# HKPolyU-UAV/FLVIS

Hardware: AMD Instinct MI355X
Metric: frames/sec/node (640×480 stereo+IMU) + ATE vs CPU ref, EuRoC MH_05 (higher is better)
Workload: dtype u8/f32 LK+GFTT, f64 geometry+BA

## Files before the change

### flvis_amd/csrc/frame_schedule.cpp

```cpp
#include <algorithm>
#include <chrono>
#include <cstring>
#include <thread>
#include <vector>

#include "pipeline_host.hpp"

using namespace flvis;

static void fill_pyr(Pipeline* pl, PyrSel& ps, uint8_t* const* l0, uint8_t* const* l1, const int* cur, int flip, int levels) {
  ps.levels = levels;
  for (int l = 0; l <= levels; l++) {
    ps.lvl[l] = ImgSel{{l0[l], l1 ? l1[l] : l0[l]}, cur, flip, nullptr};
    ps.w[l] = pl->lw[l];
    ps.h[l] = pl->lh[l];
    ps.pitch[l] = pl->lpitch[l];
    ps.stride[l] = pl->lstride[l];
    ps.bx[l] = pl->lbx;
    ps.by[l] = pl->lby;
  }
}

unsigned flvis::pyramid_levels(hipStream_t ds, bool bordered, ImgSel src0, int spitch0, size_t sstride0, bool ingest, bool level0_is_buffer,
                               const PyrSel& pyr, int S, const int* active) {
// ... 35 lines not shown
      if (f) border_left &= ~(1u << d);
    }
    l = d;
  }
  return border_left;
}

static void join_signal(Pipeline* pl, Lane* L, JoinId id, hipStream_t s) {
  Join& j = L->join[id];
  ++j.seq;
  if (pl->flag_joins) launch_store_flag(s, j.word, j.seq);
  else hipEventRecord(j.ev, s);
}
static void join_wait(Pipeline* pl, Lane* L, hipStream_t s, JoinId id) {
  const Join& j = L->join[id];
  if (pl->flag_joins) launch_wait_flag(s, j.word, 1, j.seq, L->d_progress + 2);
  else hipStreamWaitEvent(s, j.ev, 0);
}

namespace flvis {
struct LaunchJoins {
  Pipeline* pl;
  Lane* L;
  hipStream_t s;
  KJoin& kj;
  int n_wait = 0, sig_later = -1, post_later = -1;
  LaunchJoins(Pipeline* pl_, Lane* L_, hipStream_t s_, KJoin& kj_) : pl(pl_), L(L_), s(s_), kj(kj_) {}
  LaunchJoins(const LaunchJoins&) = delete;
  ~LaunchJoins() { end(); }
  bool fold_signal(JoinId id) {
    if (!pl->fold_joins) return false;
    Join& j = L->join[id];
    kj.sig = j.word;
    kj.sig_seq = ++j.seq;
    kj.sig_cnt = j.cnt;
    return true;
  }
  bool fold_wait(JoinId id) {
    if (!pl->fold_joins || n_wait == (int)(sizeof(kj.wait) / sizeof(kj.wait[0]))) return false;
    kj.wait[n_wait] = L->join[id].word;
    kj.wait_seq[n_wait++] = L->join[id].seq;
    kj.err = L->d_progress + 2;
    return true;
  }
  bool fold_post(JoinId id) {
    if (!pl->fold_joins) return false;
    kj.post = L->join[id].word;
    kj.post_seq = L->join[id].seq;
    kj.err = L->d_progress + 2;
    return true;
  }
  void signal(JoinId id) {
    if (!fold_signal(id)) sig_later = id;
  }
  void wait(JoinId id) {
    if (!fold_wait(id)) join_wait(pl, L, s, id);
  }
  void post(JoinId id) {
    if (!fold_post(id)) post_later = id;
  }
  void end() {
    kj = KJoin{};
    if (sig_later >= 0) join_signal(pl, L, (JoinId)sig_later, s);
    if (post_later >= 0) join_wait(pl, L, s, (JoinId)post_later);
    n_wait = 0, sig_later = post_later = -1;
  }
};
}

LmCloudRec flvis::lane_lmc(const Pipeline* pl, const Lane* L) {
  LmCloudRec r = pl->lmc;
  r.hdr += (size_t)L->s0 * LMC_HDR;
  r.ids += (size_t)L->s0 * r.cap;
  r.pts += (size_t)L->s0 * r.cap * 3;
  return r;
}
void flvis::local_map_work(Pipeline* pl, Lane* L, hipStream_t bs, int pairs, hipEvent_t prof_end) {
  if (pl->lmc.cap <= 0) {
    launch_ba_worker(bs, L->pipe);
    if (prof_end) hipEventRecord(prof_end, bs);
    return;
  }
  Pipe one = L->pipe;
  one.ba_drain = 1;
  const LmCloudRec r = lane_lmc(pl, L);
  for (int k = 0; k < pairs; k++) {
    launch_ba_worker(bs, one);
    if (prof_end && k == 0) hipEventRecord(prof_end, bs);
    launch_lm_cloud_append(bs, one, r);
  }
}

void flvis::launch_local_map(Pipeline* pl, Lane* L, JoinId at, bool signal, hipEvent_t* prof_begin_end) {
  const int bi = (L->idx * pl->nba_lane + (int)(L->ba_launches % pl->nba_lane)) % pl->nba;
  hipStream_t bs = pl->ba_stream[bi];
  if (prof_begin_end) {
    unsigned char& rec = L->prof18_rec[(size_t)pl->prof_step];
    if (rec) prof_begin_end = nullptr;
    else rec = 1;
  }
  if (signal) join_signal(pl, L, at, L->st);
  join_wait(pl, L, bs, at);
  const bool rec_on = pl->lmc.cap > 0;
  if (rec_on && L->ba_launches > 0) join_wait(pl, L, bs, J_BA(L->ba_launches - 1));
  if (prof_begin_end) hipEventRecord(prof_begin_end[0], bs);
  local_map_work(pl, L, bs, pl->ba_every + std::min(L->lmc_cmds, pl->ba_every), prof_begin_end ? prof_begin_end[1] : nullptr);
  L->lmc_cmds = 0;
  join_signal(pl, L, J_BA(L->ba_launches), bs);
  L->ba_launches++;
  L->ba_pending = false;
}

static void sync_streams(flvis_ctx* ctx) {
  hipStreamSynchronize(ctx->stream);
  Pipeline* pl = ctx->pipe;
  if (!pl) return;
  for (Lane* L : pl->lanes) {
    hipStreamSynchronize(L->st);
    hipStreamSynchronize(L->det_stream);
  }
  for (int k = 0; k < Pipeline::NBA; k++)
    if (pl->ba_stream[k]) hipStreamSynchronize(pl->ba_stream[k]);
}
void flvis::sync_all(flvis_ctx* ctx) {
  if (ctx->pipe)
    for (Lane* L : ctx->pipe->lanes)
      if (L->ba_pending) launch_local_map(ctx->pipe, L, J_FE, true, nullptr);
  sync_streams(ctx);
  Pipeline* pl = ctx->pipe;
  if (!pl) return;
  for (Lane* L : pl->lanes) {
    std::vector<unsigned> hd(L->S), tl(L->S);
    for (int guard = 0; guard < 64; guard++) {
      hipMemcpy(hd.data(), L->pipe.kfq_head, sizeof(unsigned) * L->S, hipMemcpyDeviceToHost);
      hipMemcpy(tl.data(), L->pipe.kfq_tail, sizeof(unsigned) * L->S, hipMemcpyDeviceToHost);
      bool pending = false;
      for (int i = 0; i < L->S; i++) pending = pending || hd[i] != tl[i];
      if (!pending) break;
      local_map_work(pl, L, pl->ba_stream[0], 1, nullptr);
      hipStreamSynchronize(pl->ba_stream[0]);
    }
  }
}

static long long lane_backpressure_depth(Pipeline* pl, Lane* L) {
  long long D = std::max(0, KFQ / 2 / pl->ba_every - 3);
  if (L->cmd_steps.empty()) return D;
  const long long window = (D + pl->nba_lane + 2) * pl->ba_every;
  std::vector<long long>& c = L->cmd_steps;
  c.erase(std::remove_if(c.begin(), c.end(), [&](long long f) { return L->frames_uploaded - f > window; }), c.end());
  return std::max(0LL, D - (long long)c.size());
}

void flvis::lane_backpressure_wait(Pipeline* pl, Lane* L, LaunchJoins* folded) {
  const long long D = lane_backpressure_depth(pl, L);
  for (int k = 0; k < pl->nba_lane; k++) {
    const long long j = L->ba_launches - 1 - D - k;
    if (j < 0 || L->ba_launches - j > BAQ) continue;
    if (folded) folded->wait(J_BA(j));
    else join_wait(pl, L, L->st, J_BA(j));
  }
}

namespace {

struct Frame {
  Pipeline* pl;
  Lane* L;
  Pipe& p;
  hipStream_t st, ds;
  int S, w, h;
  int with_local_map;
  long long frame_no;
  bool zerocopy;
  bool prof;
  hipEvent_t* pev;
  hipEvent_t* prof18;
  bool skipped, idle_step;
  bool eq, aligned, depth_cam, r_in_place;
  ImgSel in0, in1, l0cur;
  bool cmd_pending;
  bool first_processed;
  bool head_prepare;
  bool head_posts;
  bool merge_collect;
  void mark(int i, int end, hipStream_t s) const {
    if (prof && ((pl->prof_mask >> i) & 1ull)) hipEventRecord(pev[2 * i + end], s);
  }
  void pb(int i, hipStream_t s) const { mark(i, 0, s); }
  void pe(int i, hipStream_t s) const { mark(i, 1, s); }
  void stage_host_inputs(const uint8_t* d_img0, const uint8_t* d_img1, const double* h_times, const uint8_t* present);
  void stage_ingest_left(), stage_head(), stage_idle_tail(), stage_temporal_lk(), stage_collect_ransac_f(), stage_detection_fork();
  void stage_pnp_pose(), stage_new_landmarks(), stage_stereo_depth(), stage_frame_end();
  void local_map_tail(hipEvent_t* p18, bool timed), frame_end(bool backpressure);
  LKParams lk_params(int stats_at, int tc_mode, int order) const;
};

void Frame::stage_host_inputs(const uint8_t* d_img0, const uint8_t* d_img1, const double* h_times, const uint8_t* present) {
  frame_no = ++L->frames_uploaded;
  const int pslot = (int)((frame_no - 1) % Lane::PIN_RING);
  uint8_t* pin = (uint8_t*)L->pinned[pslot];
  if (pl->sync_each_frame) hipStreamSynchronize(st);
  const long long lead = std::min(std::min(pl->host_lead, pl->host_lead_cap), (int)Lane::PIN_RING - 1);
  if (frame_no > lead && *L->h_progress < frame_no - lead) {
    const auto tw = std::chrono::steady_clock::now();
    int polls = 0;
    while (*L->h_progress < frame_no - lead) {
      if ((++polls & 255) == 0 && hipStreamQuery(st) == hipSuccess && *L->h_progress < frame_no - lead) break;
      std::this_thread::sleep_for(std::chrono::microseconds(30));
    }
    pl->host_ms_wait += std::chrono::duration<double, std::milli>(std::chrono::steady_clock::now() - tw).count();
  }
  double* pt = (double*)pin;
  double* pi = pt + S;
  const uint8_t** ptab = (const uint8_t**)(pi + (size_t)S * IMU_MAX * 7);
  int* pn = (int*)(ptab + 2);
  int* ppres = (int*)((uint8_t*)pin + L->in_off_pres);
  int n_present = S;
  if (present) {
    n_present = 0;
    for (int s = 0; s < S; s++) n_present += (ppres[s] = present[s] ? 1 : 0);
  }
  const bool all_present = n_present == S, none_present = n_present == 0;
  memcpy(pt, h_times, sizeof(double) * S);
  for (int s = 0; s < S; s++)
    memcpy(pi + (size_t)s * IMU_MAX * 7, &L->h_imu[(size_t)s * IMU_MAX * 7], sizeof(double) * 7 * L->h_nimu[s]);
  ptab[0] = d_img0;
  ptab[1] = d_img1;
  memcpy(pn, L->h_nimu.data(), sizeof(int) * S);
  std::fill(L->h_nimu.begin(), L->h_nimu.end(), 0);
  cmd_pending = L->cmd_since_frame;
  L->cmd_since_frame = false;
  zerocopy = L->pinned_dev[pslot] != nullptr;
  L->h_tab[0] = d_img0, L->h_tab[1] = d_img1;
  p.in_img1 = d_img1;
  {
    uint8_t* din = zerocopy ? L->pinned_dev[pslot] : L->d_inputs;
    L->d_time = reinterpret_cast<double*>(din);
    p.imu_in = reinterpret_cast<double*>(din + L->in_off_imu);
    p.n_imu = reinterpret_cast<int*>(din + L->in_off_n);
    p.present = all_present ? nullptr : reinterpret_cast<const int*>(din + L->in_off_pres);
  }
  if (!zerocopy) hipMemcpyAsync(L->d_inputs, pin, L->input_bytes, hipMemcpyHostToDevice, st);
  prof = pl->prof_cap > 0 && pl->prof_step < pl->prof_cap;
  pev = prof ? &L->prof_ev[(size_t)pl->prof_step * (2 * PROF_STAGES)] : nullptr;
  prof18 = (prof && ((pl->prof_mask >> 18) & 1ull)) ? &pev[2 * 18] : nullptr;
  skipped = pl->frames_fed < (long long)pl->cfg.skip_first_n_imgs;
  idle_step = skipped || none_present;
  first_processed = pl->frames_fed == (long long)pl->cfg.skip_first_n_imgs;
  depth_cam = pl->cfg.cam_type == CAM_DEPTH;
  eq = pl->cfg.need_equal_hist != 0;
  aligned = (w & 15) == 0 && !(((uintptr_t)d_img0 | (depth_cam ? (uintptr_t)0 : (uintptr_t)d_img1)) & 15);
  r_in_place = !eq && aligned;
  in0 = img_plain(d_img0), in1 = img_plain(d_img1);
  l0cur = ImgSel{{L->pyr0[0][0], L->pyr0[1][0]}, p.img_slot, 0, nullptr};
  head_prepare = pl->head_prepare && !pl->feedback_used && !idle_step;
  merge_collect = (pl->chain_merge & 2) != 0;
}

void Frame::stage_ingest_left() {
  ImgSel l0in{{L->pyr0[0][0], L->pyr0[1][0]}, p.img_slot_in, 0, nullptr};
  if (pl->fold_joins && zerocopy && L->endf_valid && pl->chain_continuous) {
    join_wait(pl, L, ds, J_ENDF);
  } else {
    join_signal(pl, L, J_LM, st);
    join_wait(pl, L, ds, J_LM);
  }
  if (pl->up_event) hipStreamWaitEvent(ds, pl->up_event, 0);
  if (pl->up_flag) launch_wait_flag(ds, pl->up_flag, Pipeline::HostFeed::FLAG_WORDS, pl->up_seq, L->d_progress + 2);
  pb(1, ds);
  const int* pg = p.present;
  if (eq) launch_equalize_hist(ds, in0, l0in, w, h, w, pl->lpitch[0], (size_t)w * h, pl->lstride[0], S, L->eq_hist, L->eq_lut, pg);
  else if (!aligned) launch_copy_image_any(ds, in0, l0in, w, h, w, pl->lpitch[0], (size_t)w * h, pl->lstride[0], S, pg);
  pe(1, ds);
  pb(2, ds);
  PyrSel pyl;
  fill_pyr(pl, pyl, L->pyr0[0], L->pyr0[1], p.img_slot_in, 0, pl->levels);
  unsigned border_left = pyramid_levels(ds, pl->lbx != 0, in0, w, (size_t)w * h, !eq && aligned, true, pyl, S, pg);
  if (pl->levels == 0 && !eq && aligned) launch_copy_image(ds, in0, l0in, w, h, w, pl->lpitch[0], (size_t)w * h, pl->lstride[0], S, pg);
  if (border_left) launch_pyr_border(ds, pyl, S, pg, border_left);
  pe(2, ds);
  join_signal(pl, L, J_IMG, ds);
}

void Frame::stage_head() {
  pb(0, st);
  bool head_signals;
  {
    LaunchJoins j(pl, L, st, p.kj);
    head_signals = !pl->feedback_used && j.fold_signal(J_HEAD);
    head_posts = !idle_step && j.fold_post(J_IMG);
    if (head_prepare) launch_frame_head_prepare(st, p, L->d_time, L->d_progress, frame_no);
    else launch_frame_head(st, p, L->d_time, L->d_progress, frame_no);
  }
  if (pl->feedback_used) launch_apply_correction(st, p);
  pe(0, st);
  if (!head_signals) join_signal(pl, L, J_HEAD, st);
}

void Frame::local_map_tail(hipEvent_t* p18, bool timed) {
  if (with_local_map && (pl->frames_fed % pl->ba_every) == 0) {
    if (L->ba_pending) launch_local_map(pl, L, J_FE, true, nullptr);
    if (pl->defer_ba) L->ba_pending = true;
    else if (L->endf_valid) launch_local_map(pl, L, J_ENDF, false, p18);
    else launch_local_map(pl, L, J_FE, true, p18);
  } else if (!with_local_map) {
    if (cmd_pending) {
      if (L->ba_launches > 0) join_wait(pl, L, st, J_BA(L->ba_launches - 1));
      launch_kfq_drop(st, p);
    } else hipMemcpyAsync(p.kfq_head, p.kfq_tail, sizeof(unsigned) * S, hipMemcpyDeviceToDevice, st);
    if (timed) {
      pb(18, st);
      pe(18, st);
      L->prof18_rec[(size_t)pl->prof_step] = 1;
    }
  }
}

void Frame::frame_end(bool backpressure) {
  LaunchJoins j(pl, L, st, p.kj);
  if (backpressure) lane_backpressure_wait(pl, L, &j);
  pb(17, st);
  L->endf_valid = j.fold_signal(J_ENDF);
  launch_frame_end(st, p);
  j.end();
  pe(17, st);
  pe(19, st);
}

void Frame::stage_idle_tail() {
  frame_end(false);
  if (prof)
    for (int i = 1; i < PROF_STAGES; i++)
      if (i != 17 && i != 19) {
        pb(i, st);
        pe(i, st);
      }
  if (!skipped) local_map_tail(nullptr, false);
}

LKParams Frame::lk_params(int stats_at, int tc_mode, int order) const {
  LKParams prm{30, 1e-3 * 1e-3, 1e-4f, 1};
  if (pl->lk_stats) prm.stats = reinterpret_cast<unsigned long long*>(p.counters) + stats_at;
  if (pl->lk_stats) prm.stats_tc = reinterpret_cast<unsigned long long*>(p.counters) + 61;
  if (L->tc) {
    prm.tc = L->tc;
    prm.tc_mode = tc_mode;
    prm.tc_cap = p.tc_cap;
    prm.tc_stride = L->tc_stride;
    prm.tc_slot = p.lk_slot;
    prm.tc_tag = p.lk_tag;
  }
  prm.dbg_slot = (int)(pl->frames_fed & 7);
  prm.order = order;
  return prm;
}

void Frame::stage_temporal_lk() {
  if (first_processed && L->idx > 0) hipStreamWaitEvent(st, pl->lanes[L->idx - 1]->ev_stagger, 0);
  pb(3, st);
  if (!head_prepare) launch_track_prepare(st, p);
  pe(3, st);
  if (!head_posts) join_wait(pl, L, st, J_IMG);
  pb(4, st);
  PyrSel prev, next;
  fill_pyr(pl, prev, L->pyr0[0], L->pyr0[1], p.img_slot, 1, pl->levels_t);
  fill_pyr(pl, next, L->pyr0[0], L->pyr0[1], p.img_slot, 0, pl->levels_t);
  launch_lk_track(st, prev, next, p.prev_pts, p.next_pts, p.lk_status, p.lk_count, NMAX, S, lk_params(36, 2, 0), p.act_track, pl->max_pts, 1);
  pe(4, st);
}

void Frame::stage_collect_ransac_f() {
  pb(5, st);
  if (!merge_collect) launch_track_collect(st, p);
  pe(5, st);
  if (first_processed && pl->lanes.size() > 1) hipEventRecord(L->ev_stagger, st);
  pb(6, st);
  {
    LaunchJoins j(pl, L, st, p.kj);
    j.signal(J_LM);
    launch_ransac_f(st, p, merge_collect);
    pe(6, st);
  }
}

void Frame::stage_detection_fork() {
  join_wait(pl, L, ds, J_LM);
  join_wait(pl, L, ds, J_HEAD);
  launch_gftt(ds, l0cur, w, h, pl->lpitch[0], pl->lstride[0], S, L->gftt, nullptr, p.cam.gftt_ql, p.gftt_maxc, p.cam.gftt_num,
              (double)p.cam.gftt_dis, L->gftt_xy, L->gftt_n, 2 * p.cam.gftt_num, p.gftt_act,
              (prof && ((pl->prof_mask >> 10) & 7ull) == 7ull) ? &pev[2 * 10] : nullptr, false);
  {
    KJoin prep_kj{};
    LaunchJoins j(pl, L, ds, prep_kj);
    j.signal(J_GFTT);
    launch_feature_dem_prep(ds, l0cur, w, h, pl->lpitch[0], pl->lstride[0], S, p.cam.dem, L->gftt_xy, L->gftt_n, 2 * p.cam.gftt_num,
                            p.gftt_act, L->dem_sorted, L->dem_roff, &prep_kj);
  }
  join_wait(pl, L, ds, J_HEAD);
  if (!depth_cam) {
    if (eq) launch_equalize_hist(ds, in1, img_plain(L->pyr1[0]), w, h, w, pl->lpitch[0], (size_t)w * h, pl->lstride[0], S, L->eq_hist, L->eq_lut, p.act_img);
    else if (!aligned) launch_copy_image_any(ds, in1, img_plain(L->pyr1[0]), w, h, w, pl->lpitch[0], (size_t)w * h, pl->lstride[0], S, p.act_img);
    PyrSel pyr_r;
    fill_pyr(pl, pyr_r, L->pyr1, nullptr, nullptr, 0, pl->levels);
    unsigned border_left = pyramid_levels(ds, pl->lbx != 0, in1, w, (size_t)w * h, false, !r_in_place, pyr_r, S, p.act_img);
    if (border_left) launch_pyr_border(ds, pyr_r, S, p.act_img, border_left);
  }
  join_signal(pl, L, J_DET, ds);
}

void Frame::stage_pnp_pose() {
  pb(7, st);
  const bool ba_here = L->ba_pending;
  bool pnp_signals;
  {
    LaunchJoins j(pl, L, st, p.kj);
    pnp_signals = ba_here && j.fold_signal(J_FE);
    launch_ransac_pnp(st, p);
  }
  if (p.pnp_tail_cv) launch_pnp_tail_cv(st, p);
  pe(7, st);
  if (ba_here) launch_local_map(pl, L, J_FE, !pnp_signals, prof18);
  pb(8, st);
  launch_pose_lm(st, p);
  pe(8, st);
  pb(9, st);
  {
    LaunchJoins j(pl, L, st, p.kj);
    j.signal(J_LM);
    launch_reproj_filter(st, p);
    pe(9, st);
  }
  join_wait(pl, L, ds, J_LM);
  launch_vi_correction(ds, p);
}

void Frame::stage_new_landmarks() {
  {
    KJoin dem_kj{};
    LaunchJoins j(pl, L, st, dem_kj);
    j.wait(J_GFTT);
    pb(13, st);
    launch_feature_dem(st, w, h, S, p.cam.dem, L->dem_sorted, L->dem_roff, 2 * p.cam.gftt_num, p.det_mode, p.exist_xy, p.n_exist, NMAX,
                       p.new_xy, p.n_new, NEW_MAX, &dem_kj);
  }
  const bool merge_seeds = (pl->chain_merge & 1) != 0;
  bool an_signals, seeds_post;
  {
    LaunchJoins j(pl, L, st, p.kj);
    an_signals = j.fold_signal(J_LM);
    if (!merge_seeds) {
      launch_add_new(st, p);
      j.end();
    }
    pe(13, st);
    pb(14, st);
    seeds_post = j.fold_post(J_DET);
    if (merge_seeds) launch_add_new_seeds(st, p);
    else launch_depth_seeds(st, p);
  }
  pe(14, st);
  if (!an_signals) join_signal(pl, L, J_LM, st);
  join_wait(pl, L, ds, J_LM);
  launch_depth_triangulate(ds, p);
  join_signal(pl, L, J_TRI, ds);
  if (!seeds_post) join_wait(pl, L, st, J_DET);
}

void Frame::stage_stereo_depth() {
  pb(15, st);
  if (!depth_cam) {
    PyrSel prev, next;
    fill_pyr(pl, prev, L->pyr0[0], L->pyr0[1], p.img_slot, 0, pl->levels_s);
    fill_pyr(pl, next, L->pyr1, nullptr, nullptr, 0, pl->levels_s);
    next.lvl[0] = r_in_place ? in1 : img_plain(L->pyr1[0]);
    next.pitch[0] = r_in_place ? w : pl->lpitch[0];
    next.stride[0] = r_in_place ? (size_t)w * h : pl->lstride[0];
    if (r_in_place) next.bx[0] = next.by[0] = 0;
    launch_lk_track(st, prev, next, p.prev_pts, p.next_pts, p.lk_status, p.lk_count, NMAX, S, lk_params(48, 1, 1), p.det_mode, pl->max_pts, 2);
  }
  pe(15, st);
  LaunchJoins j(pl, L, st, p.kj);
  j.wait(J_TRI);
  pb(16, st);
  launch_depth_innovate(st, p);
  j.end();
  pe(16, st);
}

void Frame::stage_frame_end() {
  frame_end(with_local_map != 0);
  if (pl->kfl.cap > 0) kf_log_frame(pl, L, st, in1.b[0], depth_cam || r_in_place);
  local_map_tail(prof18, prof);
}

}

static void lane_frame(Pipeline* pl, Lane* L, const uint8_t* d_img0, const uint8_t* d_img1, const double* h_times, const uint8_t* present,
                       int with_local_map) {
  Frame f{pl, L, L->pipe, L->st, L->det_stream, L->S, pl->cfg.image_width, pl->cfg.image_height, with_local_map};
  f.stage_host_inputs(d_img0, d_img1, h_times, present);
  f.pb(19, f.st);
  if (!f.idle_step) f.stage_ingest_left();
  f.stage_head();
  if (f.idle_step) return f.stage_idle_tail();
  f.stage_temporal_lk();
  f.stage_collect_ransac_f();
  f.stage_detection_fork();
  f.stage_pnp_pose();
  f.stage_new_landmarks();
  f.stage_stereo_depth();
  f.stage_frame_end();
}

extern "C" {

int flvis_image_feed(flvis_ctx* ctx, const uint8_t* d_img0, const uint8_t* d_img1, const double* h_times,
                     flvis_frame_out* h_out, int with_local_map) {
  return flvis_image_feed_present(ctx, d_img0, d_img1, h_times, nullptr, h_out, with_local_map);
}

int flvis_image_feed_present(flvis_ctx* ctx, const uint8_t* d_img0, const uint8_t* d_img1, const double* h_times, const uint8_t* h_present,
                             flvis_frame_out* h_out, int with_local_map) {
  if (!ctx || !ctx->pipe || !d_img0 || !d_img1 || !h_times) return FLVIS_ERR_INVALID_ARG;
  Pipeline* pl = ctx->pipe;
  if (h_present) {
    bool all = true;
    for (int s = 0; s < pl->S && all; s++) all = h_present[s] != 0;
    if (all) h_present = nullptr;
  }
  hipSetDevice(ctx->device);
  const size_t img_px = (size_t)pl->cfg.image_width * pl->cfg.image_height;
  const size_t img1_bytes = img_px * (pl->cfg.cam_type == CAM_DEPTH ? 2 : 1);
  const bool multi = pl->lanes.size() > 1;
  const auto t_host0 = std::chrono::steady_clock::now();
  if (multi) hipEventRecord(pl->ev_in, ctx->stream);
  for (Lane* L : pl->lanes) {
    if (multi) hipStreamWaitEvent(L->st, pl->ev_in, 0);
    lane_frame(pl, L, d_img0 + (size_t)L->s0 * img_px, d_img1 + (size_t)L->s0 * img1_bytes, h_times + L->s0,
               h_present ? h_present + L->s0 : nullptr, with_local_map);
    if (multi) {
      hipEventRecord(L->ev_end[pl->frames_fed % Lane::HOLD_RING], L->st);
      const long long rel = pl->frames_fed - pl->input_hold;
      if (rel >= 0) hipStreamWaitEvent(ctx->stream, L->ev_end[rel % Lane::HOLD_RING], 0);
    }
  }
  pl->host_ms_total += std::chrono::duration<double, std::milli>(std::chrono::steady_clock::now() - t_host0).count();
  const bool prof = pl->prof_cap > 0 && pl->prof_step < pl->prof_cap;
  if (prof) pl->prof_step++;
  pl->frames_fed++;
  if (h_present) {
    for (int s = 0; s < pl->S; s++) pl->stream_frames += h_present[s] != 0;
  } else {
    pl->stream_frames += pl->S;
  }
  hipError_t e = hipGetLastError();
  if (e != hipSuccess) return ctx->hip_fail(e, "image_feed launch");
  if (h_out) {
    static_assert(sizeof(flvis_frame_out) == sizeof(FrameOut), "FrameOut layout");
    for (Lane* L : pl->lanes) {
      e = hipMemcpyAsync(h_out + L->s0, L->pipe.out, sizeof(FrameOut) * L->S, hipMemcpyDeviceToHost, L->st);
      if (e != hipSuccess) return ctx->hip_fail(e, "image_feed readback");
    }
    for (Lane* L : pl->lanes) {
      e = hipStreamSynchronize(L->st);
      if (e != hipSuccess) return ctx->hip_fail(e, "image_feed readback");
    }
  }
  return FLVIS_OK;
}


int flvis_imu_feed_all(flvis_ctx* ctx, const int* h_counts, const double* h_samples, int samples_per_stream) {
  if (!ctx || !ctx->pipe || !h_counts || !h_samples || samples_per_stream <= 0) return FLVIS_ERR_INVALID_ARG;
  Pipeline* pl = ctx->pipe;
  for (int s = 0; s < pl->S; s++) {
    int n = h_counts[s];
    if (n < 0 || n > samples_per_stream) return ctx->fail(FLVIS_ERR_INVALID_ARG, "imu_feed_all: bad count");
    int rc = flvis_imu_feed_flvis_frame(ctx, s, n, h_samples + (size_t)s * samples_per_stream * 7);
    if (rc) return rc;
  }
  return FLVIS_OK;
}

int flvis_run_steps(flvis_ctx* ctx, int n_steps, const flvis_step* steps, int with_local_map, double* h_call_ms) {
  return flvis_run_steps_present(ctx, n_steps, steps, nullptr, with_local_map, h_call_ms);
}

int flvis_run_steps_present(flvis_ctx* ctx, int n_steps, const flvis_step* steps, const uint8_t* h_present, int with_local_map,
                            double* h_call_ms) {
  if (!ctx || !ctx->pipe || n_steps < 0 || (n_steps > 0 && !steps)) return FLVIS_ERR_INVALID_ARG;
  for (int k = 0; k < n_steps; k++) {
    const flvis_step& f = steps[k];
    const auto t0 = std::chrono::steady_clock::now();
    if (f.h_imu_counts) {
      const int rc = flvis_imu_feed_all(ctx, f.h_imu_counts, f.h_imu_samples, f.imu_samples_per_stream);
      if (rc != FLVIS_OK) return rc;
    }
    ctx->pipe->defer_ba = k + 1 < n_steps;
    ctx->pipe->chain_continuous = k > 0;
    const int rc = flvis_image_feed_present(ctx, f.d_img0, f.d_img1, f.h_times, h_present ? h_present + (size_t)k * ctx->pipe->S : nullptr,
                                            nullptr, with_local_map);
    ctx->pipe->defer_ba = false;
    ctx->pipe->chain_continuous = false;
    if (rc != FLVIS_OK) return rc;
    if (h_call_ms) h_call_ms[k] = std::chrono::duration<double, std::milli>(std::chrono::steady_clock::now() - t0).count();
  }
  return FLVIS_OK;
}

}
```

### flvis_amd/csrc/img_kernels.hip

```cpp
#include <cstdlib>

#include "dev_common.hpp"
#include "dem_sort.hpp"
#include "eig_strip.hpp"
#include "img_kernels.hpp"

namespace flvis {

template <int TH, int TW, int TS>
__device__ __forceinline__ void load_tile_u8(const uint8_t* __restrict__ img, int w, int h, int pitch, int x0, int y0,
                                             uint8_t* tile, int bx = 0, int by = 0) {
  static_assert(TW % 4 == 0, "tile width must be a multiple of 4");
  constexpr int DW = TW / 4;
  if (x0 >= -bx && y0 >= -by && x0 + TW <= w + bx && y0 + TH <= h + by && blockDim.x == 256) {
    constexpr int N = TH * DW, T = (N + 255) / 256;
    const __attribute__((address_space(1))) uint8_t* const base =
        (const __attribute__((address_space(1))) uint8_t*)(img + (ptrdiff_t)y0 * pitch + x0);
    uint32_t v[T];
#pragma unroll
    for (int t = 0; t < T; t++) {
      const int i = (int)threadIdx.x + 256 * t;
      const int r = i / DW, c = i - r * DW;
      const bool on = 256 * (t + 1) <= N || i < N;
      v[t] = *(const __attribute__((address_space(1))) uint32_t*)(base + (on ? (size_t)r * pitch + 4 * c : 0));
    }
#pragma unroll
    for (int t = 0; t < T; t++) asm volatile("" : "+v"(v[t]));
#pragma unroll
    for (int t = 0; t < T; t++) {
      const int i = (int)threadIdx.x + 256 * t;
      const int r = i / DW, c = i - r * DW;
      if (256 * (t + 1) <= N || i < N) *reinterpret_cast<uint32_t*>(tile + r * TS + 4 * c) = v[t];
    }
    return;
  }
  for (int i = threadIdx.x; i < TH * DW; i += blockDim.x) {
    int r = i / DW, c = i - r * DW;
    int gy = reflect101c(y0 + r, h);
    int gx = x0 + 4 * c;
    const uint8_t* row = img + (size_t)gy * pitch;
    uint32_t v;
    if (gx >= 0 && gx + 3 < w) {
      v = *reinterpret_cast<const uint32_t*>(row + gx);
    } else {
      uint32_t b0 = row[reflect101c(gx, w)], b1 = row[reflect101c(gx + 1, w)], b2 = row[reflect101c(gx + 2, w)],
               b3 = row[reflect101c(gx + 3, w)];
      v = b0 | (b1 << 8) | (b2 << 16) | (b3 << 24);
    }
    *reinterpret_cast<uint32_t*>(tile + r * TS + 4 * c) = v;
  }
}

__global__ __launch_bounds__(256) void k_hist256(ImgSel src, int w, int h, int pitch, size_t sstride,
                                                 unsigned* __restrict__ hist, const int* __restrict__ active) {
  const int s = blockIdx.y;
  if (active && !active[s]) return;
  __shared__ unsigned lh[4][256];
  for (int i = threadIdx.x; i < 1024; i += 256) (&lh[0][0])[i] = 0;
  __syncthreads();
  const uint8_t* img = src.ptr(s, sstride);
  const int wv = threadIdx.x >> 6;
  const int dwords_per_row = w >> 2;
  const int total = dwords_per_row * h;
  for (int i = blockIdx.x * 256 + threadIdx.x; i < total; i += gridDim.x * 256) {
    const int y = i / dwords_per_row, x4 = i - y * dwords_per_row;
    uint32_t v = *reinterpret_cast<const uint32_t*>(img + (size_t)y * pitch + 4 * x4);
    atomicAdd(&lh[wv][v & 255], 1u);
    atomicAdd(&lh[wv][(v >> 8) & 255], 1u);
    atomicAdd(&lh[wv][(v >> 16) & 255], 1u);
    atomicAdd(&lh[wv][v >> 24], 1u);
  }
  __syncthreads();
  unsigned t = lh[0][threadIdx.x] + lh[1][threadIdx.x] + lh[2][threadIdx.x] + lh[3][threadIdx.x];
  if (t) atomicAdd(&hist[s * 256 + threadIdx.x], t);
}

__global__ __launch_bounds__(256) void k_equalize_lut(unsigned* __restrict__ hist, uint8_t* __restrict__ lut, int total,
                                                      const int* __restrict__ active) {
  const int s = blockIdx.x;
  if (active && !active[s]) return;
  __shared__ unsigned hs[256];
  __shared__ unsigned cs[256];
  __shared__ int first;
  const int t = threadIdx.x;
  hs[t] = hist[s * 256 + t];
  hist[s * 256 + t] = 0;
  if (t == 0) first = 256;
  __syncthreads();
  if (hs[t]) atomicMin(&first, t);
  cs[t] = hs[t];
  __syncthreads();
  for (int o = 1; o < 256; o <<= 1) {
    unsigned v = (t >= o) ? cs[t - o] : 0;
    __syncthreads();
    cs[t] += v;
    __syncthreads();
  }
  const int i0 = first;
  uint8_t out;
  if ((int)hs[i0] == total) {
    out = (uint8_t)i0;
  } else if (t <= i0) {
    out = 0;
  } else {
    float scale = (256 - 1.f) / (float)(total - (int)hs[i0]);
    int sum = (int)(cs[t] - cs[i0]);
    int v = __float2int_rn((float)sum * scale);
    out = (uint8_t)(v < 0 ? 0 : v > 255 ? 255 : v);
  }
  lut[s * 256 + t] = out;
}

__global__ __launch_bounds__(256) void k_lut_apply(ImgSel src, ImgSel dst, int w, int h, int spitch, int dpitch,
                                                   size_t sstride, size_t dstride, const uint8_t* __restrict__ lut,
                                                   const int* __restrict__ active) {
  const int s = blockIdx.y;
  if (active && !active[s]) return;
  __shared__ uint8_t l[256];
  l[threadIdx.x] = lut ? lut[s * 256 + threadIdx.x] : (uint8_t)threadIdx.x;
  __syncthreads();
  const uint8_t* in = src.ptr(s, sstride);
  uint8_t* out = const_cast<uint8_t*>(dst.ptr(s, dstride));
  const int dpr = w >> 2;
  const int total = dpr * h;
  for (int i = blockIdx.x * 256 + threadIdx.x; i < total; i += gridDim.x * 256) {
    const int y = i / dpr, x4 = i - y * dpr;
    uint32_t v = *reinterpret_cast<const uint32_t*>(in + (size_t)y * spitch + 4 * x4);
    uint32_t o = (uint32_t)l[v & 255] | ((uint32_t)l[(v >> 8) & 255] << 8) | ((uint32_t)l[(v >> 16) & 255] << 16) |
                 ((uint32_t)l[v >> 24] << 24);
    *reinterpret_cast<uint32_t*>(out + (size_t)y * dpitch + 4 * x4) = o;
  }
}

template <int CH>
__global__ __launch_bounds__(256) void k_bgr_to_gray(const uint8_t* __restrict__ src, uint8_t* __restrict__ dst, int quads) {
  const int i = blockIdx.x * 256 + threadIdx.x;
  if (i >= quads) return;
  const uint32_t* in = reinterpret_cast<const uint32_t*>(src) + (size_t)i * CH;
  uint32_t o = 0;
  if (CH == 4) {
#pragma unroll
    for (int k = 0; k < 4; k++) {
      const uint32_t v = in[k];
      const uint32_t y = ((v & 255u) * 1868u + ((v >> 8) & 255u) * 9617u + ((v >> 16) & 255u) * 4899u + (1u << 13)) >> 14;
      o |= y << (8 * k);
    }
  } else {
    const uint32_t a = in[0], b = in[1], c = in[2];
    const uint32_t px[4][3] = {{a & 255u, (a >> 8) & 255u, (a >> 16) & 255u},
                               {a >> 24, b & 255u, (b >> 8) & 255u},
                               {(b >> 16) & 255u, b >> 24, c & 255u},
                               {(c >> 8) & 255u, (c >> 16) & 255u, c >> 24}};
#pragma unroll
    for (int k = 0; k < 4; k++) o |= ((px[k][0] * 1868u + px[k][1] * 9617u + px[k][2] * 4899u + (1u << 13)) >> 14) << (8 * k);
  }
  reinterpret_cast<uint32_t*>(dst)[i] = o;
}
// ... 498 lines not shown
      out[2 * pos] = (float)x;
      out[2 * pos + 1] = (float)y;
      atomicOr(&bitmap[y * wpr + (x >> 5)], 1u << (x & 31));
    }
    accepted += __popcll(accmask);
    __builtin_amdgcn_wave_barrier();
    asm volatile("" ::: "memory");
  }
  ps.accepted = accepted;
}

__global__ __launch_bounds__(SORT_T) void k_gftt_pick(unsigned long long* __restrict__ keys, int* __restrict__ nkeys, int cap,
                                                      int w, int h, const int* __restrict__ max_corners_s, int max_corners,
                                                      double min_distance, float* __restrict__ out_xy,
                                                      int* __restrict__ out_n, int out_cap, const int* __restrict__ active,
                                                      unsigned* __restrict__ maxenc, const double* __restrict__ qual_s,
                                                      double quality) {
  const int s = blockIdx.x;
  if (active && !active[s]) return;
  extern __shared__ __attribute__((aligned(16))) unsigned char pick_smem[];
  unsigned long long* sk = reinterpret_cast<unsigned long long*>(pick_smem);
  int* hist = reinterpret_cast<int*>(sk + SORT_LDS);
  unsigned* bitmap = reinterpret_cast<unsigned*>(hist + PICK_BINS + 8);
  __shared__ PickState ps;
  __shared__ int s_lo, s_hi, s_m, s_full, s_fill;
  const int tid = threadIdx.x;
  const unsigned thr_ord = f32_ordered((float)((double)f32_unordered(maxenc[s]) * (qual_s ? qual_s[s] : quality)));
  __syncthreads();
  if (tid == 0) maxenc[s] = 0;
  int n = nkeys[s];
  if (n > cap) n = cap;
  const int maxc = max_corners_s ? max_corners_s[s] : max_corners;
  unsigned long long* K = keys + (size_t)s * cap;
  float* out = out_xy + (size_t)s * out_cap * 2;
  const bool use_dist = min_distance >= 1.0;
  const float md2 = (float)(min_distance * min_distance);
  int R = use_dist ? (int)__double2int_rn(min_distance) : 0;
  if (R > PICK_MAXR) R = PICK_MAXR;
  const int wpr = (w + 31) >> 5;
  for (int i = tid; i < wpr * h; i += SORT_T) bitmap[i] = 0;
  for (int i = tid; i <= PICK_BINS; i += SORT_T) hist[i] = 0;
  if (tid <= PICK_MAXR) {
    int cw = -1;
    if (tid <= R)
      for (int dx = 0; dx <= R; dx++) {
        float fdx = (float)dx, fdy = (float)tid;
        if (fdx * fdx + fdy * fdy < md2) cw = dx;
      }
    ps.chord[tid] = cw;
  }
  if (tid == 0) {
    ps.accepted = 0;
    s_full = 0;
  }
  __syncthreads();
  for (int i = tid; i < n; i += SORT_T) {
    const unsigned long long nk = ~K[i];
    if ((unsigned)(nk >> 32) > thr_ord) atomicAdd(&hist[(unsigned)(nk >> 52)], 1);
  }
  __syncthreads();
  {
    const int b0 = PICK_BINS - 4 * (tid + 1);
    const int c3 = hist[b0 + 3], c2 = hist[b0 + 2], c1 = hist[b0 + 1], c0 = hist[b0];
    int mysum = c0 + c1 + c2 + c3, inc = mysum;
    const int lane = tid & 63, wv = tid >> 6;
#pragma unroll
    for (int o = 1; o < 64; o <<= 1) {
      const int v = __shfl_up(inc, o, 64);
      if (lane >= o) inc += v;
    }
    __shared__ int wtot[SORT_T / 64];
    if (lane == 63) wtot[wv] = inc;
    __syncthreads();
    int before = inc - mysum;
    for (int k = 0; k < wv; k++) before += wtot[k];
    hist[b0 + 3] = before + c3;
    hist[b0 + 2] = before + c3 + c2;
    hist[b0 + 1] = before + c3 + c2 + c1;
    hist[b0] = before + mysum;
  }
  __syncthreads();
  int hi = PICK_BINS;
  bool sorted_all = false;
  while (true) {
    if (tid == 0) {
      int lo = hi, m = 0;
      if (!s_full && hi > 0) {
        int tier = SORT_LDS;
        if (hi == PICK_BINS && maxc > 0 && 3 * maxc < SORT_LDS) tier = 3 * maxc > 1024 ? 3 * maxc : 1024;
        const int basec = hist[hi];
        int a = 0, b = hi - 1;
        if (hist[hi - 1] - basec > SORT_LDS) {
          s_full = 1;
        } else {
          if (hist[hi - 1] - basec > tier) tier = SORT_LDS;
          while (a < b) {
            const int mid = (a + b) >> 1;
            if (hist[mid] - basec <= tier) b = mid;
            else a = mid + 1;
          }
          lo = a;
          m = hist[lo] - basec;
        }
      }
      s_lo = lo;
      s_hi = hi;
      s_m = m;
    }
    __syncthreads();
    if (s_full) break;
    const int lo = s_lo, m = s_m;
    if (lo == hi) break;
    if (tid == 0) s_fill = 0;
    __syncthreads();
    for (int i = tid; i < n; i += SORT_T) {
      const unsigned long long k = K[i];
      const int bin = (int)((~k) >> 52);
      if (bin >= lo && bin < hi && (unsigned)((~k) >> 32) > thr_ord) sk[atomicAdd(&s_fill, 1)] = k;
    }
    __syncthreads();
    sort_keys_lds(sk, m);
    if (tid < 64) pick_walk(sk, m, w, h, wpr, bitmap, maxc, md2, R, use_dist, out, out_cap, ps);
    __syncthreads();
    hi = lo;
    if ((maxc > 0 && ps.accepted >= maxc) || hi == 0) {
      sorted_all = true;
      break;
    }
  }
  if (!sorted_all && s_full) {
    for (int i = tid; i < wpr * h; i += SORT_T) bitmap[i] = 0;
    if (tid == 0) ps.accepted = 0;
    __syncthreads();
    sort_keys_global(K, n, cap, sk);
    __syncthreads();
    const int nv = hist[0];
    if (tid < 64) {
      for (int base = 0; base < nv && (maxc <= 0 || ps.accepted < maxc); base += SORT_LDS) {
        const int m = (nv - base) < SORT_LDS ? (nv - base) : SORT_LDS;
        pick_walk(K + base, m, w, h, wpr, bitmap, maxc, md2, R, use_dist, out, out_cap, ps);
      }
    }
    __syncthreads();
  }
  if (tid == 0) {
    int accepted = ps.accepted;
    if (maxc > 0 && accepted > maxc) accepted = maxc;
    if (accepted > out_cap) accepted = out_cap;
    out_n[s] = accepted;
    nkeys[s] = 0;
  }
}

constexpr int DEM_MAXC = 4096;
constexpr int DEM_MAXR = 192;
int dem_max_region_features() { return DEM_MAXR; }

__device__ __forceinline__ float dem_harris(const uint8_t* __restrict__ img, int pitch, float ptx, float pty) {
  int xx = (int)ptx, yy = (int)pty;
  const uint8_t* p = img + (size_t)yy * pitch + xx;
  int p0 = p[-pitch - 1], p1 = p[-pitch], p2 = p[-pitch + 1];
  int p3 = p[-1];
  int p5 = p[pitch + 1];
  int p6 = p[pitch - 1], p7 = p[pitch], p8 = p[pitch + 1];
  float IX = (float)((p0 + p3 + p6 - (p2 + p5 + p8)) / 3);
  float IY = (float)((p0 + p1 + p2 - (p6 + p7 + p8)) / 3);
  float X2 = IX * IX, Y2 = IY * IX, XY = IX * IX;
  return (X2 * Y2) - (XY * XY) - 0.05f * (X2 + Y2) * (X2 + Y2);
}

constexpr int DEM_T = 256;
constexpr int DEMP_T = 1024;
struct PackedArray {
  typedef int value_type;
  int* v;
  __device__ __forceinline__ int get(int i) const { return v[i]; }
  __device__ __forceinline__ void set(int i, int x) const { v[i] = x; }
  __device__ __forceinline__ bool before(int a, int b) const { return (a >> 16) < (b >> 16); }
};

__device__ __forceinline__ void k_feature_dem_prep_body(ImgSel src, int w, int h, int pitch, size_t sstride, DemParams prm,
                                                            const float* __restrict__ corners, const int* __restrict__ ncorners,
                                                            int corner_cap, const int* __restrict__ active, float* __restrict__ sorted_xy,
                                                            int* __restrict__ region_off) {
  const int s = blockIdx.x;
  if (active && !active[s]) return;
  const int tid = threadIdx.x, lane = tid & 63, wv = tid >> 6;
  extern __shared__ __attribute__((aligned(16))) unsigned char dem_smem[];
  const int cmax = ((corner_cap < DEM_MAXC ? corner_cap : DEM_MAXC) + 1) & ~1;
  float* cx = reinterpret_cast<float*>(dem_smem);
  float* cy = cx + cmax;
  float* cscore = cy + cmax;
  short* creg = reinterpret_cast<short*>(cscore + cmax);
  short* bucket = creg + cmax;
  __shared__ int rcount[16], roff[17];
  const uint8_t* img = src.ptr(s, sstride);
  int nc = ncorners[s];
  if (nc > corner_cap) nc = corner_cap;
  if (nc > DEM_MAXC) nc = DEM_MAXC;
  const float* C = corners + (size_t)s * corner_cap * 2;
  if (tid < 16) rcount[tid] = 0;
  __syncthreads();
  for (int i = tid; i < nc; i += DEMP_T) {
    float px = C[2 * i], py = C[2 * i + 1];
    int r = -1;
    float sc = 0.f;
    if (px >= 3 && px < (w - 3) && py >= 3 && py < (h - 3)) {
      r = (int)(4.f * floorf(py / (float)prm.regionHeight) + px / (float)prm.regionWidth);
      sc = dem_harris(img, pitch, px, py);
      atomicAdd(&rcount[r], 1);
    }
    cx[i] = px;
    cy[i] = py;
    cscore[i] = sc;
    creg[i] = (short)r;
  }
  __syncthreads();
  if (tid == 0) {
    int o = 0;
    for (int r = 0; r < 16; r++) {
      roff[r] = o;
      o += rcount[r];
    }
    roff[16] = o;
  }
  __syncthreads();
  for (int r = wv; r < 16; r += DEMP_T / 64) {
    int o = roff[r];
    for (int base = 0; base < nc; base += 64) {
      const int i = base + lane;
      const bool in = i < nc && creg[i] == r;
      const unsigned long long bq = __ballot(in);
      if (in) bucket[o + lane_prefix(bq)] = (short)i;
      o += __popcll(bq);
    }
  }
  __syncthreads();
  float* const SX = sorted_xy + (size_t)s * corner_cap * 2;
  __shared__ int rtie[16];
  __shared__ int sstack[16][3 * demsort::STACK];
  int* const ccls = reinterpret_cast<int*>(cx + 3 * cmax) + cmax;
  if (tid < 16) rtie[tid] = 0;
  __syncthreads();
  for (int j = tid; j < roff[16]; j += DEMP_T) {
    const int i = bucket[j];
    const int r = creg[i];
    const float sc = cscore[i];
    int greater = 0, earlier = 0;
    bool tie = false;
    for (int q = roff[r]; q < roff[r + 1]; q++) {
      const float sj = cscore[bucket[q]];
      greater += sj > sc;
      earlier += sj == sc && q < j;
      tie = tie || (sj == sc && q != j);
    }
    if (tie) rtie[r] = 1;
    ccls[j] = (greater << 16) | (j - roff[r]);
    const int pos = greater + earlier;
    SX[2 * (roff[r] + pos)] = cx[i];
    SX[2 * (roff[r] + pos) + 1] = cy[i];
  }
  __syncthreads();
  if (wv < 16 && rtie[wv] && roff[wv + 1] - roff[wv] > demsort::THRESHOLD) {
    const int r0 = roff[wv], n = roff[wv + 1] - r0;
    if (lane == 0) demsort::quicksort_phase(PackedArray{ccls + r0}, n, sstack[wv]);
    __builtin_amdgcn_wave_barrier();
    asm volatile("s_waitcnt lgkmcnt(0)" ::: "memory");
    for (int e = lane; e < n; e += 64) {
      const int key = ccls[r0 + e], cls = key >> 16;
      int earlier = 0;
      for (int q = 0; q < e; q++) earlier += (ccls[r0 + q] >> 16) == cls;
      const int i = bucket[r0 + (key & 0xffff)];
      SX[2 * (r0 + cls + earlier)] = cx[i];
      SX[2 * (r0 + cls + earlier) + 1] = cy[i];
    }
  }
  if (tid < 17) region_off[(size_t)s * 17 + tid] = roff[tid];
}
__global__ __launch_bounds__(DEMP_T) void k_feature_dem_prep(ImgSel src, int w, int h, int pitch, size_t sstride, DemParams prm,
                                                            const float* __restrict__ corners, const int* __restrict__ ncorners,
                                                            int corner_cap, const int* __restrict__ active, float* __restrict__ sorted_xy,
                                                            int* __restrict__ region_off, KJoin kj) {
  kj_wait(kj);
  k_feature_dem_prep_body(src, w, h, pitch, sstride, prm, corners, ncorners, corner_cap, active, sorted_xy, region_off);
  kj_signal(kj);
}

__device__ __forceinline__ void k_feature_dem_body(int w, int h, DemParams prm, const float* __restrict__ sorted_xy,
                                                       const int* __restrict__ region_off, int corner_cap, const int* __restrict__ mode,
                                                       const double* __restrict__ exist_xy, const int* __restrict__ nexist,
                                                       int exist_cap, float* __restrict__ out_xy, int* __restrict__ out_n,
                                                       int out_cap) {
  const int s = blockIdx.x;
  const int md = mode ? mode[s] : 1;
  if (md == 0) return;
  const int tid = threadIdx.x, lane = tid & 63, wv = tid >> 6;
  extern __shared__ __attribute__((aligned(16))) unsigned char dem_smem[];
  const int cmax = ((corner_cap < DEM_MAXC ? corner_cap : DEM_MAXC) + 1) & ~1;
  float* cx = reinterpret_cast<float*>(dem_smem);
  float* cy = cx + cmax;
  __shared__ int roff[17];
  __shared__ float kx[16][DEM_MAXR], ky[16][DEM_MAXR];
  __shared__ int kcount[16], knew0[16], ooff[17], kover[16];
  __shared__ int wcnt[DEM_T / 64][16];
  if (tid < 17) roff[tid] = region_off[(size_t)s * 17 + tid];
  if (tid < 16) kcount[tid] = 0, kover[tid] = 0;
  __syncthreads();
  {
    const float* const SX = sorted_xy + (size_t)s * corner_cap * 2;
    const int tot = roff[16] < cmax ? roff[16] : cmax;
    for (int j = tid; j < tot; j += DEM_T) {
      cx[j] = SX[2 * j];
      cy[j] = SX[2 * j + 1];
    }
  }
  if (md == 2) {
    int ne = nexist[s];
    if (ne > exist_cap) ne = exist_cap;
    const double* E = exist_xy + (size_t)s * exist_cap * 2;
    for (int base = 0; base < ne; base += DEM_T) {
      const int i = base + tid;
      int r = -1;
      float px = 0.f, py = 0.f;
      if (i < ne) {
        px = (float)E[2 * i];
        py = (float)E[2 * i + 1];
        if (px >= 3 && px < (w - 3) && py >= 3 && py < (h - 3))
          r = (int)(4.f * floorf(py / (float)prm.regionHeight) + px / (float)prm.regionWidth);
      }
      int myrank = 0;
#pragma unroll
      for (int q = 0; q < 16; q++) {
        const unsigned long long bq = __ballot(r == q);
        if (lane == 0) wcnt[wv][q] = __popcll(bq);
        if (r == q) myrank = lane_prefix(bq);
      }
      __syncthreads();
      if (r >= 0) {
        int k = kcount[r] + myrank;
        for (int v = 0; v < wv; v++) k += wcnt[v][r];
        if (k < DEM_MAXR) {
          kx[r][k] = px;
          ky[r][k] = py;
        }
      }
      __syncthreads();
      if (tid < 16) {
        int k = kcount[tid];
        for (int v = 0; v < DEM_T / 64; v++) k += wcnt[v][tid];
        kcount[tid] = k < DEM_MAXR ? k : DEM_MAXR;
        if (k >= DEM_MAXR) kover[tid] = 1;
      }
      __syncthreads();
    }
  }
  __syncthreads();
  if (tid < 16) knew0[tid] = kcount[tid];
  __syncthreads();
  {
    const int r = tid >> 4, sub = tid & 15;
    const int bd = prm.boundary_dis;
    int kept = kcount[r];
    unsigned count = 0;
    const int j0 = roff[r], j1 = roff[r + 1];
    if (md == 2 && kover[r]) {
      int ne = nexist[s];
      if (ne > exist_cap) ne = exist_cap;
      const double* E = exist_xy + (size_t)s * exist_cap * 2;
      int found = 0;
      for (int j = j0; j < j1 && !found; j++) {
        const float px = (float)__float2int_rn(cx[j]), py = (float)__float2int_rn(cy[j]);
        int bad = 0;
        for (int i = sub; i < ne; i += 16) {
          const float ex = (float)E[2 * i], ey = (float)E[2 * i + 1];
          if (!(ex >= 3 && ex < (w - 3) && ey >= 3 && ey < (h - 3))) continue;
          if ((int)(4.f * floorf(ey / (float)prm.regionHeight) + ex / (float)prm.regionWidth) != r) continue;
          if (fabsf(px - ex) <= (float)bd || fabsf(py - ey) <= (float)bd) bad = 1;
        }
        bad = (int)((__ballot(bad != 0) >> (lane & 48)) & 0xFFFFull);
        if (!bad) {
          if (sub == 0) {
            kx[r][0] = px;
            ky[r][0] = py;
          }
          found = 1;
        }
      }
      if (sub == 0) {
        knew0[r] = 0;
        kcount[r] = found;
      }
    } else {
    for (int j = j0; j < j1; j++) {
      float px = cx[j], py = cy[j];
      if (md == 2) {
        px = (float)__float2int_rn(px);
        py = (float)__float2int_rn(py);
      }
      int bad = 0;
      for (int k = sub; k < kept; k += 16) {
        float dis_x = fabsf(px - kx[r][k]);
        float dis_y = fabsf(py - ky[r][k]);
        if (dis_x <= (float)bd || dis_y <= (float)bd) bad = 1;
      }
      bad = (int)((__ballot(bad != 0) >> (lane & 48)) & 0xFFFFull);
      if (!bad) {
        if (kept < DEM_MAXR && sub == 0) {
          kx[r][kept] = px;
          ky[r][kept] = py;
        }
        kept++;
        count++;
        __builtin_amdgcn_wave_barrier();
        asm volatile("" ::: "memory");
        if (md == 1) {
          if (count >= prm.max_region_feature_num) break;
        } else {
          if ((unsigned)kept >= prm.max_region_feature_num) break;
        }
      }
    }
    if (sub == 0) kcount[r] = kept < DEM_MAXR ? kept : DEM_MAXR;
    }
  }
  __syncthreads();
  if (tid == 0) {
    int o = 0;
    for (int r = 0; r < 16; r++) {
      ooff[r] = o;
      o += kcount[r] - knew0[r];
    }
    ooff[16] = o;
    out_n[s] = o < out_cap ? o : out_cap;
  }
  __syncthreads();
  {
    float* O = out_xy + (size_t)s * out_cap * 2;
    const int r = tid >> 4, sub = tid & 15;
    for (int k = knew0[r] + sub; k < kcount[r]; k += 16) {
      const int o = ooff[r] + (k - knew0[r]);
      if (o < out_cap) {
        O[2 * o] = kx[r][k];
        O[2 * o + 1] = ky[r][k];
      }
    }
  }
}
__global__ __launch_bounds__(DEM_T) void k_feature_dem(int w, int h, DemParams prm, const float* __restrict__ sorted_xy,
                                                       const int* __restrict__ region_off, int corner_cap, const int* __restrict__ mode,
                                                       const double* __restrict__ exist_xy, const int* __restrict__ nexist,
                                                       int exist_cap, float* __restrict__ out_xy, int* __restrict__ out_n,
                                                       int out_cap, KJoin kj) {
  kj_wait(kj);
  k_feature_dem_body(w, h, prm, sorted_xy, region_off, corner_cap, mode, exist_xy, nexist, exist_cap, out_xy, out_n, out_cap);
  kj_signal(kj);
}

static inline int div_up(int a, int b) { return (a + b - 1) / b; }

void launch_equalize_hist(hipStream_t st, ImgSel src, ImgSel dst, int w, int h, int spitch, int dpitch, size_t sstride,
                          size_t dstride, int S, unsigned* hist, uint8_t* lut, const int* active) {
  int blocks = div_up((w / 4) * h, 256 * 8);
  if (blocks > 64) blocks = 64;
  hipLaunchKernelGGL(k_hist256, dim3(blocks, S), dim3(256), 0, st, src, w, h, spitch, sstride, hist, active);
  hipLaunchKernelGGL(k_equalize_lut, dim3(S), dim3(256), 0, st, hist, lut, w * h, active);
  int ablocks = div_up((w / 4) * h, 256 * 4);
  hipLaunchKernelGGL(k_lut_apply, dim3(ablocks, S), dim3(256), 0, st, src, dst, w, h, spitch, dpitch, sstride, dstride,
                     (const uint8_t*)lut, active);
}

void launch_bgr_to_gray(hipStream_t st, const uint8_t* src, int channels, uint8_t* dst, size_t npixels) {
  const int quads = (int)(npixels / 4);
  if (channels == 4)
    hipLaunchKernelGGL(k_bgr_to_gray<4>, dim3(div_up(quads, 256)), dim3(256), 0, st, src, dst, quads);
  else
    hipLaunchKernelGGL(k_bgr_to_gray<3>, dim3(div_up(quads, 256)), dim3(256), 0, st, src, dst, quads);
}

void launch_copy_image(hipStream_t st, ImgSel src, ImgSel dst, int w, int h, int spitch, int dpitch, size_t sstride,
                       size_t dstride, int S, const int* active) {
  const bool a16 = !src.ind && (w % 16) == 0 && (spitch % 16) == 0 && (dpitch % 16) == 0 && (sstride % 16) == 0 && (dstride % 16) == 0 &&
                   ((uintptr_t)src.b[0] % 16) == 0 && ((uintptr_t)src.b[1] % 16) == 0 && ((uintptr_t)dst.b[0] % 16) == 0 &&
                   ((uintptr_t)dst.b[1] % 16) == 0;
  if (a16) {
    hipLaunchKernelGGL(k_copy_image16, dim3(div_up((w / 16) * h, 256 * 2), S), dim3(256), 0, st, src, dst, w / 16, h, spitch,
                       dpitch, sstride, dstride, active);
    return;
  }
  int ablocks = div_up((w / 4) * h, 256 * 4);
  hipLaunchKernelGGL(k_lut_apply, dim3(ablocks, S), dim3(256), 0, st, src, dst, w, h, spitch, dpitch, sstride, dstride,
                     (const uint8_t*)nullptr, active);
}

void launch_copy_image_any(hipStream_t st, ImgSel src, ImgSel dst, int w, int h, int spitch, int dpitch, size_t sstride,
                           size_t dstride, int S, const int* active) {
  hipLaunchKernelGGL(k_copy_image_any, dim3(div_up((dpitch / 4) * h, 256 * 4), S), dim3(256), 0, st, src, dst, w, h, spitch, dpitch,
                     sstride, dstride, active);
}

bool pyr_border_fusable(int w, int h, int bx, int by) { return bx < w && by < h; }

void launch_pyr_down(hipStream_t st, ImgSel src, int sw, int sh, int spitch, size_t sstride, ImgSel dst, int dpitch,
                     size_t dstride, int S, const int* active, int bx, int by, int sbx, int sby) {
  int dw = (sw + 1) / 2, dh = (sh + 1) / 2;
  hipLaunchKernelGGL(k_pyr_down, dim3(div_up(dw, PD_TW), div_up(dh, PD_TH), S), dim3(256), 0, st, src, sw, sh, spitch,
                     sstride, dst, dpitch, dstride, active, bx, by, sbx, sby);
}

void launch_pyr_down_ingest(hipStream_t st, ImgSel src, int sw, int sh, int spitch, size_t sstride, ImgSel dst0, int d0pitch,
                            size_t d0stride, ImgSel dst, int dpitch, size_t dstride, int S, const int* active, int bx, int by) {
  int dw = (sw + 1) / 2, dh = (sh + 1) / 2;
  hipLaunchKernelGGL(k_pyr_down_ingest, dim3(div_up(dw, PD_TW), div_up(dh, PD_TH), S), dim3(256), 0, st, src, sw, sh, spitch,
                     sstride, dst0, d0pitch, d0stride, dst, dpitch, dstride, active, bx, by);
}

void launch_pyr_border(hipStream_t st, const PyrSel& pyr, int S, const int* active, unsigned level_mask) {
  bool any = false;
  for (int l = 0; l <= pyr.levels; l++) any = any || (((level_mask >> l) & 1u) && (pyr.bx[l] > 0 || pyr.by[l] > 0));
  if (!any) return;
  hipLaunchKernelGGL(k_pyr_border, dim3(8, pyr.levels + 1, S), dim3(256), 0, st, pyr, active, level_mask);
}
void launch_corner_response(hipStream_t st, int variant, int rows, ImgSel src, int w, int h, int pitch, size_t sstride, int S, unsigned* maxenc,
                            unsigned long long* keys, int* nkeys, int cap, const int* active) {
  dim3 grid(div_up(w, EG_TW), div_up(h, EG_TH), S);
  if (variant == 2)
    launch_eig_walk(st, src, w, h, pitch, sstride, S, maxenc, keys, nkeys, cap, active, rows);
  else if (variant == 1)
    hipLaunchKernelGGL(k_eig_cand_strip, grid, dim3(256), 0, st, src, w, h, pitch, sstride, maxenc, keys, nkeys, cap, active);
  else
    hipLaunchKernelGGL(k_eig_cand, grid, dim3(256), 0, st, src, w, h, pitch, sstride, maxenc, keys, nkeys, cap, active);
}

void launch_gftt(hipStream_t st, ImgSel src, int w, int h, int pitch, size_t sstride, int S, GfttScratch sc,
                 const double* qual_s, double quality, const int* maxc_s, int max_corners, double min_distance,
                 float* out_xy, int* out_n, int out_cap, const int* active, hipEvent_t* ev, bool reset_counters) {
  if (reset_counters) {
    hipMemsetAsync(sc.maxenc, 0, sizeof(unsigned) * S, st);
    hipMemsetAsync(sc.nkeys, 0, sizeof(int) * S, st);
  }
  if (ev) hipEventRecord(ev[0], st);
  static const int variant_rows = [] {
    const char* e = getenv("FLVIS_EIG_WALK");
    if (!e) return 60;
    if (atoi(e) > 0) return atoi(e);
    e = getenv("FLVIS_EIG_STRIP");
    return (e && atoi(e) != 0) ? -2 : -1;
  }();
  launch_corner_response(st, variant_rows > 0 ? 2 : (variant_rows == -2 ? 1 : 0), variant_rows, src, w, h, pitch, sstride, S, sc.maxenc, sc.keys,
                         sc.nkeys, sc.cap, active);
  if (ev) hipEventRecord(ev[1], st), hipEventRecord(ev[2], st), hipEventRecord(ev[3], st), hipEventRecord(ev[4], st);
  const size_t lds = sizeof(unsigned long long) * SORT_LDS + sizeof(int) * (PICK_BINS + 8) +
                     (size_t)((w + 31) / 32) * h * sizeof(unsigned);
  hipLaunchKernelGGL(k_gftt_pick, dim3(S), dim3(SORT_T), lds, st, sc.keys, sc.nkeys, sc.cap, w, h, maxc_s, max_corners,
                     min_distance, out_xy, out_n, out_cap, active, sc.maxenc, qual_s, quality);
  if (ev) hipEventRecord(ev[5], st);
}

void launch_feature_dem_prep(hipStream_t st, ImgSel src, int w, int h, int pitch, size_t sstride, int S, DemParams prm,
                             const float* corners, const int* ncorners, int corner_cap, const int* active, float* sorted_xy,
                             int* region_off, const KJoin* kj) {
  const int cmax = ((corner_cap < DEM_MAXC ? corner_cap : DEM_MAXC) + 1) & ~1;
  hipLaunchKernelGGL(k_feature_dem_prep, dim3(S), dim3(DEMP_T), (size_t)cmax * 20, st, src, w, h, pitch, sstride, prm, corners, ncorners,
                     corner_cap, active, sorted_xy, region_off, kj ? *kj : KJoin{});
}
void launch_feature_dem(hipStream_t st, int w, int h, int S, DemParams prm, const float* sorted_xy, const int* region_off,
                        int corner_cap, const int* mode, const double* exist_xy, const int* nexist, int exist_cap, float* out_xy,
                        int* out_n, int out_cap, const KJoin* kj) {
  const int cmax = ((corner_cap < DEM_MAXC ? corner_cap : DEM_MAXC) + 1) & ~1;
  hipLaunchKernelGGL(k_feature_dem, dim3(S), dim3(DEM_T), (size_t)cmax * 8, st, w, h, prm, sorted_xy, region_off, corner_cap, mode,
                     exist_xy, nexist, exist_cap, out_xy, out_n, out_cap, kj ? *kj : KJoin{});
}

hipError_t img_kernels_init() {
  hipError_t e = hipFuncSetAttribute((const void*)k_feature_dem_prep, hipFuncAttributeMaxDynamicSharedMemorySize, DEM_MAXC * 20);
  if (e != hipSuccess) return e;
  return hipFuncSetAttribute((const void*)k_gftt_pick, hipFuncAttributeMaxDynamicSharedMemorySize, 150 * 1024);
}

}
```

### flvis_amd/csrc/pipeline.cpp

```cpp
#include <algorithm>
#include <chrono>
#include <cmath>
#include <cstddef>
#include <cstdio>
#include <cstdlib>
#include <cstring>
#include <thread>
#include <limits>
#include <vector>

#include "pipeline_host.hpp"

using namespace flvis;

static const char* kStageNames[PROF_STAGES] = {
    "imu_feed+frame_begin", "ingest(equalize)", "pyr_down(left)", "track_prepare", "lk_track(temporal)", "track_collect",
    "ransac_f", "ransac_pnp", "track_post+pose_lm", "reproj_filter", "gftt:eig_cand", "gftt:(merged)", "gftt:pick",
    "feature_dem+add_new", "depth_prepare", "lk_track(stereo)", "depth_innovate", "frame_end",
    "ba_worker(launch)", "frame(chain)"};

namespace {

int lk_levels(int w, int h, int win, int max_level) {
  int level = 0;
// ... 311 lines not shown
  p.tc_cap = 0;
  p.tc = nullptr;
  p.tc_stride = 0;
  L->tc = nullptr;
  {
    const bool on = pl->lk_tcache && pl->cfg.cam_type != CAM_DEPTH && pl->levels_s == pl->levels_t;
    if (ok && on) {
      const int cap = std::min(NMAX, (pl->max_pts + 63) / 64 * 64);
      L->tc_stride = lk_tc_slot_dwords(pl->levels_t);
      const size_t n = (size_t)S * cap * L->tc_stride;
      L->tc = dalloc<uint32_t>(L->allocs, n, false);
      if (L->tc) {
        hipMemset(L->tc, 0xff, n * sizeof(uint32_t));
        p.tc_cap = cap;
        p.tc = L->tc;
        p.tc_stride = L->tc_stride;
      } else {
        (void)hipGetLastError();
      }
    }
  }
  const int cap = gftt_key_cap(w, h);
  L->gftt.cap = cap;
  ok = ok && ((L->gftt.maxenc = dalloc<unsigned>(L->allocs, S)) != nullptr);
  ok = ok && ((L->gftt.nkeys = dalloc<int>(L->allocs, S)) != nullptr);
  ok = ok && ((L->gftt.keys = dalloc<unsigned long long>(L->allocs, (size_t)cap * S, false)) != nullptr);
  ok = ok && ((L->gftt_xy = dalloc<float>(L->allocs, (size_t)S * 2 * c.gftt_num * 2)) != nullptr);
  ok = ok && ((L->gftt_n = dalloc<int>(L->allocs, S)) != nullptr);
  ok = ok && ((L->dem_sorted = dalloc<float>(L->allocs, (size_t)S * 2 * c.gftt_num * 2)) != nullptr);
  ok = ok && ((L->dem_roff = dalloc<int>(L->allocs, (size_t)S * 17)) != nullptr);
  ok = ok && ((L->eq_hist = dalloc<unsigned>(L->allocs, (size_t)S * 256)) != nullptr);
  ok = ok && ((L->eq_lut = dalloc<uint8_t>(L->allocs, (size_t)S * 256)) != nullptr);
  ok = ok && ((L->d_join = dalloc<long long>(L->allocs, (size_t)JOIN_IDS * 8)) != nullptr);
  ok = ok && ((L->d_join_cnt = dalloc<unsigned>(L->allocs, (size_t)JOIN_IDS)) != nullptr);
  if (!ok) return false;
  for (int id = 0; id < JOIN_IDS; id++) L->join[id].word = L->d_join + 8 * id, L->join[id].cnt = L->d_join_cnt + id;
  for (int b = 0; b < S; b += RESET_LIST) {
    ResetList rl{};
    rl.n = std::min(RESET_LIST, S - b);
    for (int i = 0; i < rl.n; i++) rl.s[i] = b + i, rl.mode[i] = RS_TRACKER | RS_CREATE;
    launch_stream_reset(nullptr, p, rl, nullptr);
  }
  std::vector<unsigned long long> hseed(S);
  for (int s = 0; s < S; s++) hseed[s] = seed_base + (unsigned long long)(s0 + s);
  hipMemcpy(seeds, hseed.data(), sizeof(unsigned long long) * S, hipMemcpyHostToDevice);
  hipMemcpy(rig, pl->rigs.data() + s0, sizeof(RigParams) * S, hipMemcpyHostToDevice);
  L->cmd_frame.assign(S, -1);
  L->h_imu.assign((size_t)S * IMU_MAX * 7, 0.0);
  L->h_nimu.assign(S, 0);
  L->imu_read.assign(S, 0);
  for (int k = 0; k < Lane::PIN_RING; k++)
    if (hipHostMalloc(&L->pinned[k], L->input_bytes, hipHostMallocMapped) != hipSuccess) return false;
  for (int k = 0; k < Lane::PIN_RING; k++) {
    void* dv = nullptr;
    if (hipHostGetDevicePointer(&dv, L->pinned[k], 0) != hipSuccess) {
      (void)hipGetLastError();
      dv = nullptr;
    }
    L->pinned_dev[k] = (uint8_t*)dv;
  }
  {
    void* hp = nullptr;
    void* dp = nullptr;
    if (hipHostMalloc(&hp, 64, hipHostMallocMapped | hipHostMallocCoherent) != hipSuccess || hipHostGetDevicePointer(&dp, hp, 0) != hipSuccess) return false;
    L->h_progress = (volatile long long*)hp;
    L->d_progress = (long long*)dp;
    for (int k = 0; k < 8; k++) L->h_progress[k] = 0;
    L->pipe.ba_ovf_word = L->d_progress + 4;
  }
  if (own_stream) {
    if (hipStreamCreateWithFlags(&L->st, hipStreamNonBlocking) != hipSuccess) return false;
    L->own_st = true;
  } else {
    L->st = ctx->stream;
  }
  bool evok = hipStreamCreateWithFlags(&L->det_stream, hipStreamNonBlocking) == hipSuccess;
  for (int id = 0; id < JOIN_IDS && evok; id++) evok = hipEventCreateWithFlags(&L->join[id].ev, pl->ev_flags) == hipSuccess;
  evok = evok && hipEventCreateWithFlags(&L->ev_stagger, pl->ev_flags) == hipSuccess;
  for (hipEvent_t& e : L->ev_end) evok = evok && hipEventCreateWithFlags(&e, pl->ev_flags) == hipSuccess;
  return evok;
}

extern "C" {

}

static int check_cfg(flvis_ctx* ctx, const flvis_cfg* cfg, const std::string& pre) {
  const int w = cfg->image_width, h = cfg->image_height;
  if (w < 64 || h < 64) return ctx->fail(FLVIS_ERR_CONFIG, pre + "image must be at least 64 x 64");
  if (cfg->need_equal_hist && (w & 15)) return ctx->fail(FLVIS_ERR_CONFIG, pre + "equalizeHist rigs need an image width that is a multiple of 16");
  if (cfg->feature_para[5] > 64.0) return ctx->fail(FLVIS_ERR_CAPACITY, pre + "feature_para6 (GFTT minDistance) > 64 is not supported");
  if (cfg->window_size > BA_WMAX) return ctx->fail(FLVIS_ERR_CAPACITY, pre + "window_size exceeds the LDS-resident solver (16)");
  if (!ba_lds_admits(ba_lds_bytes_env(), cfg->window_size)) {
    char msg[192];
    snprintf(msg, sizeof msg, "FLVIS_BA_LDS_KB=%d is below the %d KB the local-map solver needs for window_size %d", ba_lds_bytes_env() / 1024,
             ba_lds_min_bytes(cfg->window_size) / 1024, cfg->window_size);
    return ctx->fail(FLVIS_ERR_CONFIG, pre + msg);
  }
  if (16 * (int)cfg->feature_para[0] > 512) return ctx->fail(FLVIS_ERR_CAPACITY, pre + "feature_para1 (landmarks per region) must be <= 32: the pose LM holds 512 edges");
  if ((int)cfg->feature_para[3] * 2 > 4096) return ctx->fail(FLVIS_ERR_CAPACITY, pre + "feature_para4 (gftt_num) must be <= 2048");
  if ((size_t)((w + 31) / 32) * h * 4 > 96 * 1024) return ctx->fail(FLVIS_ERR_CAPACITY, pre + "image too large for the GFTT LDS bitmap");
  if (cfg->cam_type == CAM_DEPTH && !(cfg->depth_factor > 0)) return ctx->fail(FLVIS_ERR_CONFIG, pre + "depth mode needs depth_factor > 0");
  return FLVIS_OK;
}

static const char* batch_field_mismatch(const flvis_cfg& ref, const flvis_cfg& c) {
  if (c.type_of_vi != ref.type_of_vi) return "type_of_vi";
  if (c.cam_type != ref.cam_type) return "cam_type";
  if (c.imu_type != ref.imu_type) return "imu_type";
  if (c.image_width != ref.image_width) return "image_width";
  if (c.image_height != ref.image_height) return "image_height";
  static const char* const fp[6] = {"feature_para[0]", "feature_para[1]", "feature_para[2]", "feature_para[3]", "feature_para[4]", "feature_para[5]"};
  for (int i = 0; i < 6; i++)
    if (memcmp(&c.feature_para[i], &ref.feature_para[i], sizeof(double))) return fp[i];
  if (c.window_size != ref.window_size) return "window_size";
  if (c.skip_first_n_imgs != ref.skip_first_n_imgs) return "skip_first_n_imgs";
  if (c.need_equal_hist != ref.need_equal_hist) return "need_equal_hist";
  return nullptr;
}

static int check_stream_cfgs(flvis_ctx* ctx, const flvis_cfg& ref, int n, const flvis_cfg* cfgs, const int* streams, const char* what) {
  for (int i = 0; i < n; i++) {
    const int s = streams ? streams[i] : i;
    const std::string pre = std::string(what) + ": stream " + std::to_string(s) + ": ";
    const int rc = check_cfg(ctx, &cfgs[i], pre);
    if (rc != FLVIS_OK) return rc;
    if (const char* f = batch_field_mismatch(ref, cfgs[i]))
      return ctx->fail(FLVIS_ERR_CONFIG, pre + "batch-wide field " + f + " differs from the tracker's (stream 0)");
  }
  return FLVIS_OK;
}

static bool env_is(const char* name, int v) {
  const char* e = getenv(name);
  return e && atoi(e) == v;
}
static void read_knobs(Pipeline* pl) {
  const char* j = getenv("FLVIS_JOIN");
  pl->flag_joins = !(j && !strcmp(j, "event"));
  if (!j) {
    const char* cc = getenv("ROCPROF_COUNTER_COLLECTION");
    if (cc && cc[0] && strcmp(cc, "0") && strcmp(cc, "False") && strcmp(cc, "false")) pl->flag_joins = false;
  }
  pl->fold_joins = pl->flag_joins && !env_is("FLVIS_JOIN_FOLD", 0);
  if (const char* e = getenv("FLVIS_LANES")) {
    const int v = atoi(e);
    if (v >= 1 && v <= 16) pl->n_lanes_req = v;
  }
  pl->lk_border = !env_is("FLVIS_LK_BORDER", 0);
  pl->lk_tcache = !env_is("FLVIS_LK_TCACHE", 0);
  pl->head_prepare = !env_is("FLVIS_HEAD_PREPARE", 0);
  if (const char* e = getenv("FLVIS_HOST_LEAD")) pl->host_lead = std::max(1, std::min(atoi(e), (int)Lane::PIN_RING));
  if (const char* e = getenv("FLVIS_SYNC_EACH_FRAME")) pl->sync_each_frame = atoi(e) != 0;
  if (const char* e = getenv("FLVIS_CHAIN_MERGE")) pl->chain_merge = atoi(e) & 3;
  if (const char* e = getenv("FLVIS_BA_EVERY")) {
    const int v = atoi(e);
    if (v >= 1 && v <= KFQ / 4) pl->ba_every = v;
  }
  pl->kf_check = env_is("FLVIS_KF_CHECK", 1);
  if (const char* e = getenv("FLVIS_PNP_TAIL")) pl->pnp_tail_cv = !strcmp(e, "cv");
  if (const char* e = getenv("FLVIS_H2D_MODE")) pl->hf.mode = atoi(e) == 1 ? 1 : 2;
  if (const char* e = getenv("FLVIS_PROF_EVENT_SCOPE")) pl->prof_scope = !strcmp(e, "agent") ? hipEventReleaseToDevice : 0u;
}

static int tracker_create_impl(flvis_ctx* ctx, const flvis_cfg* cfgs, int n_cfgs, int n_streams, uint64_t seed_base, int traj_capacity) {
  const flvis_cfg* cfg = &cfgs[0];
  const int w = cfg->image_width, h = cfg->image_height;
  hipSetDevice(ctx->device);
  Pipeline* pl = new Pipeline();
  ctx->pipe = pl;
  read_knobs(pl);
  const int S = n_streams;
  pl->S = S;
  pl->cfg = *cfg;
  pl->cfgs.resize(S);
  pl->rigs.resize(S);
  for (int k = 0; k < S; k++) {
    pl->cfgs[k] = cfgs[n_cfgs == 1 ? 0 : k];
    if (k > 0 && n_cfgs == 1) pl->rigs[k] = pl->rigs[0];
    else rig_from_cfg(pl->cfgs[k], pl->rigs[k]);
  }
  pl->max_pts = std::min(NMAX, 16 * (int)cfg->feature_para[0]);
  pl->levels_t = lk_levels(w, h, 31, 10);
  pl->levels_s = lk_levels(w, h, 31, 5);
  pl->levels = std::max(pl->levels_t, pl->levels_s);
  if (pl->levels >= LK_MAX_LEVELS) pl->levels = LK_MAX_LEVELS - 1;
  pl->lbx = pl->lk_border ? LK_BORDER_X : 0;
  pl->lby = pl->lk_border ? LK_BORDER_Y : 0;
  int lw = w, lh = h;
  for (int l = 0; l <= pl->levels; l++) {
    pl->lw[l] = lw;
    pl->lh[l] = lh;
    pl->lpitch[l] = align_up(lw, 16) + 2 * pl->lbx;
    pl->lstride[l] = (size_t)pl->lpitch[l] * (lh + 2 * pl->lby) + 64;
    pl->lstride[l] = (pl->lstride[l] + 63) / 64 * 64;
    lw = (lw + 1) / 2;
    lh = (lh + 1) / 2;
  }
  int n_lanes = std::min(pl->n_lanes_req, S);
  pl->lane_size = (S + n_lanes - 1) / n_lanes;
  n_lanes = (S + pl->lane_size - 1) / pl->lane_size;
  pl->nba_lane = std::max(1, std::min(pl->nba_lane, Pipeline::NBA / n_lanes));
  pl->nba = std::min(Pipeline::NBA, pl->nba_lane * n_lanes);
  bool ok = true;
  for (int k = 0; k < n_lanes && ok; k++) {
    Lane* L = new Lane();
    L->idx = k;
    pl->lanes.push_back(L);
    const int s0 = k * pl->lane_size;
    ok = lane_create(ctx, pl, L, s0, std::min(pl->lane_size, S - s0), seed_base, traj_capacity, n_lanes > 1);
  }
  int prio_least = 0, prio_greatest = 0;
  hipDeviceGetStreamPriorityRange(&prio_least, &prio_greatest);
  for (int k = 0; k < pl->nba && ok; k++)
    ok = hipStreamCreateWithPriority(&pl->ba_stream[k], hipStreamNonBlocking, prio_least) == hipSuccess;
  ok = ok && hipEventCreateWithFlags(&pl->ev_in, pl->ev_flags) == hipSuccess;
  if (!ok) {
    flvis_pipeline_destroy_internal(ctx);
    (void)hipGetLastError();
    return ctx->fail(FLVIS_ERR_HIP, "tracker_create: device / pinned allocation or stream creation failed");
  }
  if (ba_kernels_init() != hipSuccess || track_kernels_init() != hipSuccess) {
    (void)hipGetLastError();
    flvis_pipeline_destroy_internal(ctx);
    return ctx->fail(FLVIS_ERR_HIP, "tracker_create: cannot reserve LDS for the BA kernel");
  }
  hipDeviceSynchronize();
  return FLVIS_OK;
}

extern "C" {

int flvis_tracker_create(flvis_ctx* ctx, const flvis_cfg* cfg, int n_streams, uint64_t seed_base, int traj_capacity) {
  if (!ctx || !cfg || n_streams <= 0) return FLVIS_ERR_INVALID_ARG;
  if (ctx->pipe) flvis_pipeline_destroy_internal(ctx);
  const int rc = check_cfg(ctx, cfg, "");
  if (rc != FLVIS_OK) return rc;
  return tracker_create_impl(ctx, cfg, 1, n_streams, seed_base, traj_capacity);
}

int flvis_tracker_create_rigs(flvis_ctx* ctx, const flvis_cfg* cfgs, int n_streams, uint64_t seed_base, int traj_capacity) {
  if (!ctx || !cfgs || n_streams <= 0) return FLVIS_ERR_INVALID_ARG;
  const int rc = check_stream_cfgs(ctx, cfgs[0], n_streams, cfgs, nullptr, "tracker_create_rigs");
  if (rc != FLVIS_OK) return rc;
  if (ctx->pipe) flvis_pipeline_destroy_internal(ctx);
  return tracker_create_impl(ctx, cfgs, n_streams, n_streams, seed_base, traj_capacity);
}

int flvis_get_stream_cfg(flvis_ctx* ctx, int stream, flvis_cfg* out) {
  if (!ctx || !out) return FLVIS_ERR_INVALID_ARG;
  Pipeline* pl = ctx->pipe;
  if (!pl) return ctx->fail(FLVIS_ERR_INVALID_ARG, "get_stream_cfg: no tracker (flvis_tracker_create)");
  if (stream < 0 || stream >= pl->S) return ctx->fail(FLVIS_ERR_INVALID_ARG, "get_stream_cfg: stream out of range");
  *out = pl->cfgs[stream];
  return FLVIS_OK;
}

static int lane_flush_imu(flvis_ctx* ctx, Lane& L) {
  hipError_t e = hipStreamSynchronize(L.st);
  L.pipe.imu_in = reinterpret_cast<double*>(L.d_inputs + L.in_off_imu);
  L.pipe.n_imu = reinterpret_cast<int*>(L.d_inputs + L.in_off_n);
  if (e == hipSuccess) e = hipMemcpy(L.pipe.imu_in, L.h_imu.data(), sizeof(double) * L.h_imu.size(), hipMemcpyHostToDevice);
  if (e == hipSuccess) e = hipMemcpy(L.pipe.n_imu, L.h_nimu.data(), sizeof(int) * L.S, hipMemcpyHostToDevice);
  if (e != hipSuccess) return ctx->hip_fail(e, "imu_feed (flush)");
  launch_imu_feed(L.st, L.pipe);
  e = hipStreamSynchronize(L.st);
  if (e != hipSuccess) return ctx->hip_fail(e, "imu_feed (flush)");
  std::fill(L.h_nimu.begin(), L.h_nimu.end(), 0);
  return FLVIS_OK;
}

int flvis_imu_feed_flvis_frame(flvis_ctx* ctx, int stream, int n, const double* samples7) {
  if (!ctx || !ctx->pipe || !samples7) return FLVIS_ERR_INVALID_ARG;
  Pipeline* pl = ctx->pipe;
  if (stream < 0 || stream >= pl->S || n < 0) return ctx->fail(FLVIS_ERR_INVALID_ARG, "imu_feed: bad stream");
  int ls;
  Lane& L = pl->lane_of(stream, ls);
  while (n > 0) {
    int& cnt = L.h_nimu[ls];
    if (cnt == IMU_MAX) {
      hipSetDevice(ctx->device);
      const int rc = lane_flush_imu(ctx, L);
      if (rc != FLVIS_OK) return rc;
    }
    const int m = std::min(n, IMU_MAX - L.h_nimu[ls]);
    memcpy(&L.h_imu[((size_t)ls * IMU_MAX + L.h_nimu[ls]) * 7], samples7, sizeof(double) * 7 * m);
    L.h_nimu[ls] += m;
    samples7 += 7 * (size_t)m;
    n -= m;
  }
  return FLVIS_OK;
}

int flvis_imu_feed(flvis_ctx* ctx, int stream, double t, const double* a, const double* g) {
  if (!ctx || !ctx->pipe || !a || !g) return FLVIS_ERR_INVALID_ARG;
  double s[7];
  s[0] = t;
  if (ctx->pipe->cfg.imu_type == 3) return ctx->fail(FLVIS_ERR_CONFIG, "imu_feed: this rig has no IMU (type_of_vi 4: imu_type NONE)");
  switch (ctx->pipe->cfg.imu_type) {
    case 0:
      s[1] = -a[2]; s[2] = a[0]; s[3] = a[1];
      s[4] = g[2]; s[5] = -g[0]; s[6] = -g[1];
      break;
    case 1:
      s[1] = -a[2]; s[2] = a[1]; s[3] = -a[0];
      s[4] = g[2]; s[5] = -g[1]; s[6] = g[0];
      break;
// ... 859 lines not shown
```

### flvis_amd/csrc/pipeline_host.hpp

```cpp
#pragma once
#include <vector>

#include "../../include/flvis_hip.h"
#include "ctx.hpp"
#include "kf_log.hpp"
#include "lm_cloud.hpp"
#include "track_kernels.hpp"

namespace flvis {

constexpr int PROF_STAGES = 20;

constexpr int BAQ = 64;
enum JoinId {
  J_IMG,
  J_DET,
  J_GFTT,
  J_FE,
  J_LM,
  J_TRI,
  J_HEAD,
  J_ENDF,
  J_BA0,
  JOIN_IDS = J_BA0 + BAQ
};
inline JoinId J_BA(long long launch) { return (JoinId)(J_BA0 + (int)(launch % BAQ)); }
struct Join {
  hipEvent_t ev = nullptr;
  long long* word = nullptr;
  unsigned* cnt = nullptr;
  long long seq = 0;
};

struct Lane {
  int s0 = 0, S = 0;
  Pipe pipe;
  hipStream_t st = nullptr;
  bool own_st = false;
  uint8_t* pyr0[2][LK_MAX_LEVELS] = {};
  uint8_t* pyr1[LK_MAX_LEVELS] = {};
  uint32_t* tc = nullptr;
  int tc_stride = 0;
  GfttScratch gftt;
  float* gftt_xy = nullptr;
  float* dem_sorted = nullptr;
  int* dem_roff = nullptr;
  int* gftt_n = nullptr;
  unsigned* eq_hist = nullptr;
  uint8_t* eq_lut = nullptr;
  uint8_t* d_inputs = nullptr;
  double* d_time = nullptr;
  const uint8_t** d_tab = nullptr;
  size_t input_bytes = 0;
  std::vector<double> h_imu;
  std::vector<int> h_nimu;
  std::vector<long long> imu_read;
  static constexpr int PIN_RING = 4;
  void* pinned[PIN_RING] = {};
  uint8_t* pinned_dev[PIN_RING] = {};
  const uint8_t* h_tab[2] = {nullptr, nullptr};
  size_t in_off_imu = 0, in_off_tab = 0, in_off_n = 0, in_off_pres = 0;
  volatile long long* h_progress = nullptr;
  long long* d_progress = nullptr;
  long long frames_uploaded = 0;
  std::vector<void*> allocs;
  std::vector<hipEvent_t> prof_ev;
  std::vector<unsigned char> prof18_rec;
  hipStream_t det_stream = nullptr;
  Join join[JOIN_IDS];
  long long* d_join = nullptr;
  unsigned* d_join_cnt = nullptr;
  bool endf_valid = false;
  int idx = 0;
  static constexpr int HOLD_RING = 8;
  hipEvent_t ev_end[HOLD_RING] = {};
  hipEvent_t ev_stagger = nullptr;
  long long ba_launches = 0;
  bool ba_pending = false;
  std::vector<long long> cmd_frame;
  std::vector<long long> cmd_steps;
  int lmc_cmds = 0;
  bool cmd_since_frame = false;
  long long kfl_seq = 0;
};

struct Pipeline {
  int S = 0;
  flvis_cfg cfg;
  std::vector<flvis_cfg> cfgs;
  std::vector<RigParams> rigs;
  int lane_size = 0;
  std::vector<Lane*> lanes;
  int levels_t = 0, levels_s = 0, levels = 0;
  int lw[LK_MAX_LEVELS], lh[LK_MAX_LEVELS], lpitch[LK_MAX_LEVELS];
  size_t lstride[LK_MAX_LEVELS];
  int lbx = 0, lby = 0;
  int max_pts = 0;
  int n_lanes_req = 1;
  bool lk_border = true;
  bool lk_tcache = true;
  int chain_merge = 3;
  bool head_prepare = true;
  bool kf_check = false;
  bool pnp_tail_cv = false;
  unsigned prof_scope = 0;
  long long frames_fed = 0;
  long long stream_frames = 0;
  std::vector<void*> allocs;
  int prof_cap = 0, prof_step = 0;
  unsigned long long prof_mask = ~0ull;
  static constexpr int NBA = 8;
  int nba = 2;
  int nba_lane = 2;
  int host_lead = 3;
  int host_lead_cap = 4;
  int input_hold = 0;
  double host_ms_total = 0, host_ms_wait = 0;
  bool sync_each_frame = false;
  int ba_every = 1;
  bool lk_stats = false;
  hipStream_t ba_stream[NBA] = {};
  long long ba_rr = 0;
  hipEvent_t ev_in = nullptr;
  bool defer_ba = false;
  bool feedback_used = false;
  struct HostFeed {
    hipStream_t strm = nullptr;
    static constexpr int SLOTS = 3;
    uint8_t* raw[SLOTS][2] = {};
    uint8_t* gray[SLOTS][2] = {};
    int mode = 2;
    static constexpr int FLAG_WORDS = 4096, FLAG_RING = 4;
    long long* h_flag[FLAG_RING] = {};
    long long* d_flag = nullptr;
    long long slot_frame[SLOTS] = {0, 0, 0};
    long long last_call_frame = -1;
    size_t raw_bytes[2] = {}, gray_bytes = 0;
    hipEvent_t ev_done[2] = {}, ev_free[2] = {};
    long long n = 0;
    volatile long long* h_up = nullptr;
    long long* d_up = nullptr;
    std::vector<double> times;
    double ms_wait_uploads = 0, ms_issue = 0, ms_feed = 0;
    bool timing = false;
    hipEvent_t ev_t0[2] = {}, ev_t1[2] = {};
    bool timed[2] = {false, false};
    size_t timed_bytes[2] = {0, 0};
    double up_ms = 0, up_bytes = 0, up_calls = 0;
  } hf;
  hipEvent_t up_event = nullptr;
  const long long* up_flag = nullptr;
  long long up_seq = 0;
  static constexpr unsigned ev_flags = hipEventDisableTiming;
  bool flag_joins = false;
  bool fold_joins = false;
  bool chain_continuous = false;
  LmCloudRec lmc{};
  hipEvent_t lmc_ev = nullptr;
  KfLogRec kfl{};
  Lane& lane_of(int stream, int& local) {
    const int k = stream / lane_size;
    local = stream - k * lane_size;
    return *lanes[k];
  }
};

template <typename T>
T* dalloc(std::vector<void*>& allocs, size_t n, bool zero = true) {
  void* p = nullptr;
  if (hipMalloc(&p, n * sizeof(T)) != hipSuccess) return nullptr;
  if (zero) hipMemset(p, 0, n * sizeof(T));
  allocs.push_back(p);
  return (T*)p;
}

unsigned pyramid_levels(hipStream_t ds, bool bordered, ImgSel src0, int spitch0, size_t sstride0, bool ingest, bool level0_is_buffer,
                        const PyrSel& pyr, int S, const int* active);
void sync_all(flvis_ctx* ctx);
LmCloudRec lane_lmc(const Pipeline* pl, const Lane* L);
void local_map_work(Pipeline* pl, Lane* L, hipStream_t bs, int pairs, hipEvent_t prof_end);
void launch_local_map(Pipeline* pl, Lane* L, JoinId at, bool signal, hipEvent_t* prof_begin_end);
KfLogRec lane_kfl(const Pipeline* pl, const Lane* L);
void kf_log_frame(Pipeline* pl, Lane* L, hipStream_t st, const uint8_t* in1, bool in_place);
void kf_log_reset_stream(Pipeline* pl, Lane* L, int ls);
void kf_log_free(Pipeline* pl);
struct LaunchJoins;
void lane_backpressure_wait(Pipeline* pl, Lane* L, LaunchJoins* folded);

}
```

### flvis_amd/csrc/track_kernels.hip

```cpp
#include <vector>

#include "dev_common.hpp"
#include "dev_geom.hpp"
#include "epnp_core.hpp"
#include "track_kernels.hpp"
#include "cv_solvers.hpp"
#include "vi_motion.hpp"

namespace flvis {

FD Landmark* lm_ptr(const Pipe& p, int slot, int s) { return p.lm + ((size_t)slot * p.S + s) * NMAX; }

extern __shared__ __attribute__((aligned(16))) unsigned char pl_smem[];

FD int glibc_rand_next(StreamState& st) {
  int pos = st.rnd_pos;
  int a = st.rnd_r[(pos + 34 - 31) % 34], b = st.rnd_r[(pos + 34 - 3) % 34];
  int n = (int)((unsigned)a + (unsigned)b);
  st.rnd_r[pos] = n;
  st.rnd_pos = (pos + 1) % 34;
  return (int)(((unsigned)n) >> 1);
}

FD void track_fail(StreamState& st) {
  st.cont_fail++;
  st.cur ^= 1;
  if (st.cont_fail >= 2) {
    st.state = ST_TRACKFAIL;
    st.cont_fail = 0;
  }
  st.phase = PH_IDLE;
  st.ok = 0;
}

__device__ inline void imu_feed_dev(const Pipe& p, int s, const double* in) {
  StreamState& st = p.st[s];
  ViRing ring{p.vi + (size_t)s * VI_QUEUE, &st};
  int n = p.n_imu[s];
  if (n > IMU_MAX) n = IMU_MAX;
  double* const out = p.imu_out + (size_t)s * IMU_OUT_CAP * IMU_ROW;
  long long seen = st.imu_seen;
  const ViGain gain{{rig_of(p, s).vi_para[0]}};
  int i = 0;
  for (; i < n && !st.vi_initialized; i++, seen++)
    vi_imu_feed(gain, st, ring, in[7 * i], V3{in[7 * i + 1], in[7 * i + 2], in[7 * i + 3]},
                V3{in[7 * i + 4], in[7 * i + 5], in[7 * i + 6]}, out + (size_t)(seen % IMU_OUT_CAP) * IMU_ROW);
  if (i < n) {
    const V3 acc_bias = ld3(st.acc_bias), gyro_bias = ld3(st.gyro_bias);
    int head = st.vi_head, count = st.vi_count;
    MotionState prev = ring.back();
    Q4 kdq{st.kf_dq[0], st.kf_dq[1], st.kf_dq[2], st.kf_dq[3]};
    double kdt = st.kf_dt;
    V3 kdp = ld3(st.kf_dp), kdv = ld3(st.kf_dv);
    for (; i < n; i++, seen++) {
      MotionState cur;
      vi_propagate(gain, prev, in[7 * i], V3{in[7 * i + 1], in[7 * i + 2], in[7 * i + 3]},
                   V3{in[7 * i + 4], in[7 * i + 5], in[7 * i + 6]}, acc_bias, gyro_bias, cur, kdq, kdt, kdp, kdv);
      imu_row_store(out + (size_t)(seen % IMU_OUT_CAP) * IMU_ROW, cur.t, ms_q(cur), ld3(cur.pos), ld3(cur.vel));
      ring.base[(head + count) % VI_QUEUE] = cur;
      count++;
      if (count >= VI_QUEUE) {
        head = (head + 1) % VI_QUEUE;
        count--;
      }
      prev = cur;
    }
    st.vi_head = head;
    st.vi_count = count;
    st.kf_dq[0] = kdq.w, st.kf_dq[1] = kdq.x, st.kf_dq[2] = kdq.y, st.kf_dq[3] = kdq.z;
    st.kf_dt = kdt;
    st3(st.kf_dp, kdp);
    st3(st.kf_dv, kdv);
  }
  st.imu_seen = seen;
  p.n_imu[s] = 0;
}
__global__ __launch_bounds__(64) void k_imu_feed(Pipe p) {
  int s = blockIdx.x * blockDim.x + threadIdx.x;
  if (s >= p.S) return;
  imu_feed_dev(p, s, p.imu_in + (size_t)s * IMU_MAX * 7);
}

__device__ inline void pose_record_push(const Pipe& p, int s, StreamState& st, int frame_id, const double* T7, bool pop) {
  if (st.rec_count == POSE_REC) {
    st.rec_head = (st.rec_head + 1) % POSE_REC;
    st.rec_count--;
  }
  const int k = (st.rec_head + st.rec_count) % POSE_REC;
  p.rec_id[(size_t)s * POSE_REC + k] = frame_id;
  for (int j = 0; j < 7; j++) p.rec_T[((size_t)s * POSE_REC + k) * 7 + j] = T7[j];
  st.rec_count++;
  if (pop && st.rec_count >= 1000) {
    st.rec_head = (st.rec_head + 1) % POSE_REC;
    st.rec_count--;
  }
}

constexpr int AC_T = 256;
__global__ __launch_bounds__(AC_T) void k_apply_correction(Pipe p) {
  const int s = blockIdx.x;
  StreamState& st = p.st[s];
  CorrectionDev& c = p.corr_in[s];
  if (!c.valid || st.phase != PH_TRACK) return;
  __shared__ double s_old_inv[7], s_upd[7];
  __shared__ int s_idx;
  __shared__ long long s_ids[1024];
  const int tid = threadIdx.x;
  const int last = st.cur ^ 1;
  if (tid == 0) {
    const int corr_id = (int)c.frame_id;
    int idx = 0;
    for (int i = st.rec_count - 1; i >= 0; i--)
      if (p.rec_id[(size_t)s * POSE_REC + (st.rec_head + i) % POSE_REC] == corr_id) {
        idx = i;
        break;
      }
    s_idx = idx;
    const SE3d old = load_pose7(p.rec_T + ((size_t)s * POSE_REC + (st.rec_head + idx) % POSE_REC) * 7);
    store_pose7(s_old_inv, se3_inverse(old));
    for (int j = 0; j < 7; j++) s_upd[j] = c.T_c_w[j];
  }
  __syncthreads();
  const SE3d old_inv = load_pose7(s_old_inv), upd = load_pose7(s_upd);
  for (int i = s_idx + tid; i < st.rec_count; i += AC_T) {
    double* T = p.rec_T + ((size_t)s * POSE_REC + (st.rec_head + i) % POSE_REC) * 7;
    store_pose7(T, se3_mul(se3_mul(load_pose7(T), old_inv), upd));
  }
  if (tid == 0) store_pose7(st.T_c_w[last], se3_mul(se3_mul(load_pose7(st.T_c_w[last]), old_inv), upd));
  Landmark* lms = lm_ptr(p, last, s);
  const int n = st.n_lm[last];
  const int nc = min(c.lm_count, BA_LMAX);
  for (int c0 = 0; c0 < nc; c0 += 1024) {
    const int m = min(1024, nc - c0);
    __syncthreads();
    for (int i = tid; i < m; i += AC_T) s_ids[i] = (long long)(int)c.lm_id[c0 + i];
    __syncthreads();
    for (int j = tid; j < n; j += AC_T) {
      const long long id = lms[j].id;
      int hit = -1;
      for (int i = 0; i < m; i++)
        if (s_ids[i] == id) hit = i;
      if (hit >= 0)
        for (int k = 0; k < 3; k++) lms[j].p3w[k] = c.lm_3d[c0 + hit][k];
    }
  }
  const int no = min(c.lm_outlier_count, BA_EMAX);
  for (int c0 = 0; c0 < no; c0 += 1024) {
    const int m = min(1024, no - c0);
    __syncthreads();
    for (int i = tid; i < m; i += AC_T) s_ids[i] = (long long)(int)c.lm_outlier_id[c0 + i];
    __syncthreads();
    for (int j = tid; j < n; j += AC_T) {
      const long long id = lms[j].id;
      bool hit = false;
      for (int i = 0; i < m; i++) hit = hit || (s_ids[i] == id);
      if (hit) lms[j].inlier = 0;
    }
// ... 1374 lines not shown
}
__global__ void k_track_post(Pipe p) {
  int s = blockIdx.x * blockDim.x + threadIdx.x;
  if (s >= p.S) return;
  if (p.st[s].phase != PH_TRACK) return;
  track_post_dev(p, s);
}

constexpr int PL_T = 256;
constexpr int PL_ROW = 29;
constexpr int PL_NS = 28;
constexpr int PL_CH = 32;
constexpr int PL_EMAX = 512;
struct PoseLMShared {
  double pw[3][PL_EMAX];
  double zu[PL_EMAX], zv[PL_EMAX];
  unsigned char alive[PL_EMAX];
  short src[PL_EMAX];
  double terms[PL_T * PL_ROW];
  double tot[PL_NS];
  double part[PL_T / PL_CH][PL_NS];
  int n;
};
static_assert(sizeof(double) * PL_T * PL_ROW >= sizeof(long long) * PL_EMAX, "the id scratch must fit the terms buffer");

__device__ inline void pose_pass(const SE3d& T, PoseLMShared& sh, int n, bool want_H, double fx, double fy, double cx, double cy) {
  const int tid = threadIdx.x;
  double sum = 0;
  for (int c0 = 0; c0 < n; c0 += PL_T) {
    const int e = c0 + tid;
    double* row = sh.terms + tid * PL_ROW;
    const bool on = e < n && sh.alive[e];
    if (on) {
      double er[2], J[2][6];
      proj_edge(T, V3{sh.pw[0][e], sh.pw[1][e], sh.pw[2][e]}, sh.zu[e], sh.zv[e], fx, fy, cx, cy, er, want_H ? J : nullptr);
      const double c2 = er[0] * er[0] + er[1] * er[1];
      row[27] = huber_rho(c2);
      if (want_H) {
        const double w = huber_w(c2);
        const double o0 = -er[0] * w, o1 = -er[1] * w;
        int q = 0;
#pragma unroll
        for (int r = 0; r < 6; r++) {
          row[21 + r] = J[0][r] * o0 + J[1][r] * o1;
#pragma unroll
          for (int cc = r; cc < 6; cc++) row[q++] = (J[0][r] * w) * J[0][cc] + (J[1][r] * w) * J[1][cc];
        }
      }
    } else if (e < n) {
#pragma unroll
      for (int k = 0; k < PL_NS; k++) row[k] = 0.0;
    }
    __syncthreads();
    const int m = (n - c0 < PL_T) ? n - c0 : PL_T;
    const int nch = (m + PL_CH - 1) / PL_CH;
    {
      const int c = tid / PL_NS, col = tid - c * PL_NS;
      if (c < nch && (want_H || col == 27)) {
        const double* colp = sh.terms + col;
        const int k0 = c * PL_CH, k1 = k0 + PL_CH < m ? k0 + PL_CH : m;
        double ps = 0;
        int k = k0;
        for (; k + 8 <= k1; k += 8) {
          double v[8];
#pragma unroll
          for (int u = 0; u < 8; u++) v[u] = colp[(k + u) * PL_ROW];
#pragma unroll
          for (int u = 0; u < 8; u++) ps += v[u];
        }
        for (; k < k1; k++) ps += colp[k * PL_ROW];
        sh.part[c][col] = ps;
      }
    }
    __syncthreads();
    if (tid < PL_NS && (want_H || tid == 27))
      for (int c = 0; c < nch; c++) sum += sh.part[c][tid];
  }
  if (tid < PL_NS) sh.tot[tid] = sum;
  __syncthreads();
}

__device__ inline void pose_lm_optimize(SE3d& T, PoseLMShared& sh, int n, int iterations, double fx, double fy, double cx, double cy) {
  double lambda = -1, ni = 2;
  for (int iteration = 0; iteration < iterations; iteration++) {
    pose_pass(T, sh, n, true, fx, fy, cx, cy);
    double currentChi = sh.tot[27];
    double H[36], b[6];
    int q = 0;
#pragma unroll
    for (int r = 0; r < 6; r++) {
      b[r] = sh.tot[21 + r];
#pragma unroll
      for (int c = r; c < 6; c++) {
        H[6 * r + c] = sh.tot[q];
        H[6 * c + r] = sh.tot[q];
        q++;
      }
    }
    if (iteration == 0) {
      double maxDiag = 0;
#pragma unroll
      for (int j = 0; j < 6; j++) maxDiag = fmax(fabs(H[7 * j]), maxDiag);
      lambda = 1e-5 * maxDiag;
      ni = 2;
    }
    double rho = 0;
    int qmax = 0;
    bool lambda_bad = false;
    do {
      SE3d backup = T;
      double Hl[36], x[6];
#pragma unroll
      for (int k = 0; k < 36; k++) Hl[k] = H[k];
#pragma unroll
      for (int j = 0; j < 6; j++) {
        Hl[7 * j] += lambda;
        x[j] = 0;
      }
      bool ok2 = solve_spd6(Hl, b, x);
      if (ok2) T = g2o_mul(g2o_exp(x), T);
      __syncthreads();
      pose_pass(T, sh, n, false, fx, fy, cx, cy);
      double tempChi = sh.tot[27];
      if (!ok2) tempChi = 1.7976931348623157e308;
      rho = currentChi - tempChi;
      double scale = 0;
#pragma unroll
      for (int j = 0; j < 6; j++) scale += x[j] * (lambda * x[j] + b[j]);
      scale += 1e-3;
      rho /= scale;
      if (rho > 0 && isfinite(tempChi)) {
        double alpha = 1. - detm::det_powi((2 * rho - 1), 3);
        alpha = fmin(alpha, 2. / 3.);
        double scaleFactor = fmax(1. / 3., alpha);
        lambda *= scaleFactor;
        ni = 2;
        currentChi = tempChi;
      } else {
        lambda *= ni;
        ni *= 2;
        T = backup;
        if (!isfinite(lambda)) {
          lambda_bad = true;
          break;
        }
      }
      qmax++;
    } while (rho < 0 && qmax < 10);
    __syncthreads();
    if (qmax == 10 || rho == 0 || lambda_bad) break;
  }
}

__global__ __launch_bounds__(PL_T) void k_pose_lm(Pipe p) {
  const int s = blockIdx.x;
  CRig& rg = rig_of(p, s);
  StreamState& st = p.st[s];
  if (st.phase != PH_TRACK) return;
  const int tid = threadIdx.x, lane = tid & 63;
  const int cur = st.cur;
  Landmark* lms = lm_ptr(p, cur, s);
  const int nl = st.n_lm[cur];
  PoseLMShared& sh = *reinterpret_cast<PoseLMShared*>(pl_smem);
  long long* ids = reinterpret_cast<long long*>(sh.terms);
#ifdef FLVIS_RANSAC_PROF
  long long tlast_ = (long long)wall_clock64();
#endif
  __shared__ int s_go;
  __syncthreads();
  if (tid == 64) s_go = track_post_dev(p, s) ? 1 : 0;
  if (tid < 64) {
    int n = 0;
    for (int base = 0; base < nl; base += 64) {
      const int i = base + lane;
      const bool sel = i < nl && lms[i].has3d && lms[i].inlier;
      const unsigned long long bm = __ballot(sel);
      if (sel) {
        const int k = n + lane_prefix(bm);
        if (k < PL_EMAX) {
          ids[k] = lms[i].id;
          sh.src[k] = (short)i;
        }
      }
      n += __popcll(bm);
    }
    if (lane == 0) sh.n = n < PL_EMAX ? n : PL_EMAX;
  }
  __syncthreads();
  RPROF(48, 0);
  if (!s_go) return;
  const int n = sh.n;
  bool ok = n >= 10;
  if (ok) {
    for (int k = tid; k < n; k += PL_T) {
      const long long id = ids[k];
      int rank = 0;
      for (int j = 0; j < n; j++) rank += ids[j] < id;
      const Landmark& lm = lms[sh.src[k]];
      sh.pw[0][rank] = lm.p3w[0];
      sh.pw[1][rank] = lm.p3w[1];
      sh.pw[2][rank] = lm.p3w[2];
      sh.zu[rank] = lm.p2u[0];
      sh.zv[rank] = lm.p2u[1];
      sh.alive[rank] = 1;
    }
    __syncthreads();
    const double fx = rg.fx, fy = rg.fy, cx = rg.cx, cy = rg.cy;
    SE3d T0 = load_pose7(st.T_c_w[cur]);
    if (tid == 0) store_pose7(st.dbg_T_pre, T0);
    SE3d T = g2o_from_mat(q_to_mat(T0.q), T0.t);
    RPROF(48, 1);
    pose_lm_optimize(T, sh, n, 2, fx, fy, cx, cy);
    RPROF(48, 2);
    __shared__ int s_alive[PL_T / 64];
    int alive = 0;
    for (int base = 0; base < n; base += PL_T) {
      const int e = base + tid;
      bool keep = false;
      if (e < n) {
        double er[2];
        proj_edge(T, V3{sh.pw[0][e], sh.pw[1][e], sh.pw[2][e]}, sh.zu[e], sh.zv[e], fx, fy, cx, cy, er, nullptr);
        keep = !(er[0] * er[0] + er[1] * er[1] > 3.0);
        if (!keep) sh.alive[e] = 0;
      }
      int tot;
      block_rank<PL_T / 64>(keep, s_alive, tot);
      alive += tot;
    }
    __syncthreads();
    RPROF(48, 3);
    if (alive < 10) {
      ok = false;
    } else {
      pose_lm_optimize(T, sh, n, 2, fx, fy, cx, cy);
      RPROF(48, 4);
      if (tid == 0) {
        store_pose7(st.T_c_w[cur], se3_from_mat(q_to_mat(T.q), T.t));
        store_pose7(st.dbg_T_lm, load_pose7(st.T_c_w[cur]));
      }
    }
  }
  if (!ok && tid == 0) track_fail(st);
#ifdef FLVIS_RANSAC_PROF
  if (tid == 0 && p.counters) atomicAdd((unsigned long long*)&p.counters[48 + 7], 1ull);
#endif
}

__global__ __launch_bounds__(PL_T) void k_pose_lm_sets(const double* __restrict__ lm3d, const double* __restrict__ lm2d,
                                                       const long long* __restrict__ lm_id, const int* __restrict__ count, int cap,
                                                       const double* __restrict__ K4, int k_stride, double* __restrict__ pose7,
                                                       unsigned char* __restrict__ okflag) {
  const int b = blockIdx.x, tid = threadIdx.x;
  PoseLMShared& sh = *reinterpret_cast<PoseLMShared*>(pl_smem);
  long long* ids = reinterpret_cast<long long*>(sh.terms);
  int n = count[b];
  n = n < 0 ? 0 : (n > cap ? cap : n);
  bool ok = n >= 10;
  if (ok) {
    const long long* const gid = lm_id + (size_t)b * cap;
    const double* const P = lm3d + (size_t)b * cap * 3;
    const double* const Z = lm2d + (size_t)b * cap * 2;
    for (int k = tid; k < n; k += PL_T) ids[k] = gid[k];
    __syncthreads();
    for (int k = tid; k < n; k += PL_T) {
      const long long id = ids[k];
      int rank = 0;
      for (int j = 0; j < n; j++) rank += (ids[j] < id) || (ids[j] == id && j < k);
      sh.pw[0][rank] = P[3 * k];
      sh.pw[1][rank] = P[3 * k + 1];
      sh.pw[2][rank] = P[3 * k + 2];
      sh.zu[rank] = Z[2 * k];
      sh.zv[rank] = Z[2 * k + 1];
      sh.alive[rank] = 1;
    }
    __syncthreads();
    const double* const k4 = K4 + (size_t)k_stride * b;
    const double fx = k4[0], fy = k4[1], cx = k4[2], cy = k4[3];
    const SE3d T0 = load_pose7(pose7 + 7 * b);
    SE3d T = g2o_from_mat(q_to_mat(T0.q), T0.t);
    pose_lm_optimize(T, sh, n, 2, fx, fy, cx, cy);
    __shared__ int s_alive[PL_T / 64];
    int alive = 0;
    for (int base = 0; base < n; base += PL_T) {
      const int e = base + tid;
      bool keep = false;
      if (e < n) {
        double er[2];
        proj_edge(T, V3{sh.pw[0][e], sh.pw[1][e], sh.pw[2][e]}, sh.zu[e], sh.zv[e], fx, fy, cx, cy, er, nullptr);
        keep = !(er[0] * er[0] + er[1] * er[1] > 3.0);
        if (!keep) sh.alive[e] = 0;
      }
      int tot;
      block_rank<PL_T / 64>(keep, s_alive, tot);
      alive += tot;
    }
    __syncthreads();
    if (alive < 10) {
      ok = false;
    } else {
      pose_lm_optimize(T, sh, n, 2, fx, fy, cx, cy);
      if (tid == 0) store_pose7(pose7 + 7 * b, se3_from_mat(q_to_mat(T.q), T.t));
    }
  }
  if (tid == 0) okflag[b] = ok ? 1 : 0;
}

__device__ __forceinline__ void k_reproj_filter_body(const Pipe& p) {
  const int s = blockIdx.x;
  CRig& rg = rig_of(p, s);
  StreamState& st = p.st[s];
  if (st.phase != PH_TRACK) return;
  const int i = threadIdx.x;
  const int cur = st.cur;
  Landmark* lms = lm_ptr(p, cur, s);
  const int n = st.n_lm[cur];
  __shared__ double valid[NMAX];
  __shared__ double sh_thr;
  __shared__ int s_cnt[NMAX / 64];
  const SE3d T = load_pose7(st.T_c_w[cur]);
  Landmark lm;
  double d = 0;
  bool v = false;
  if (i < n) {
    lm = lms[i];
    V3 pc = se3_act(T, V3{lm.p3w[0], lm.p3w[1], lm.p3w[2]});
    double u = rg.fx * pc.x / pc.z + rg.cx, vv = rg.fy * pc.y / pc.z + rg.cy;
    double ex = lm.p2u[0] - u, ey = lm.p2u[1] - vv;
    d = sqrt(ex * ex + ey * ey);
    v = d < 3.0;
  }
  int nv;
  const int vr = block_rank<NMAX / 64>(v, s_cnt, nv);
  if (v) valid[vr] = d;
  if (i == 0 && nv == 0) sh_thr = 3.0;
  __syncthreads();
  if (i == 0) {
    double sum = 0;
    for (int k = 0; k < nv; k++) sum += valid[k];
    st.reproj_err = sum / (double)nv;
  }
  if (i < nv) {
    const int target = nv / 2;
    const double vi = valid[i];
    int less = 0, eq = 0;
    for (int j = 0; j < nv; j++) {
      const double vj = valid[j];
      less += vj < vi;
      eq += vj == vi;
    }
    if (less <= target && target < less + eq) sh_thr = 1.5 * vi;
  }
  __syncthreads();
  double sh = sh_thr;
  if (sh >= 3.0) sh = 3.0;
  const bool keep = i < n && !(d > sh);
  int kept;
  const int k = block_rank<NMAX / 64>(keep, s_cnt, kept);
  if (keep) {
    lm.inlier = 1;
    lms[k] = lm;
    double* ex = p.exist_xy + ((size_t)s * NMAX + k) * 2;
    ex[0] = lm.p2d[0];
    ex[1] = lm.p2d[1];
  }
  if (i == 0) {
    st.n_lm[cur] = kept;
    st.orig_size = kept;
    p.n_exist[s] = kept;
    p.det_mode[s] = 2;
    p.det_maxc[s] = p.cam.gftt_num;
    st.vi_corr_due = st.has_imu ? 1 : 0;
  }
}
__global__ __launch_bounds__(NMAX) void k_reproj_filter(Pipe p) {
  kj_wait(p.kj);
  k_reproj_filter_body(p);
  kj_signal(p.kj);
}
__global__ void k_vi_correction(Pipe p) {
  const int s = blockIdx.x * blockDim.x + threadIdx.x;
  if (s >= p.S) return;
  StreamState& st = p.st[s];
  if (!st.vi_corr_due) return;
  st.vi_corr_due = 0;
  const int cur = st.cur;
  ViRing ring{p.vi + (size_t)s * VI_QUEUE, &st};
  vi_correction_from_vision(rig_of(p, s), st, ring, st.frame_time[cur], load_pose7(st.T_c_w[cur]), st.frame_time[cur ^ 1],
                            load_pose7(st.T_c_w[cur ^ 1]));
}

template <int T>
__device__ __forceinline__ void k_add_new_body(const Pipe& p) {
  const int s = blockIdx.x;
  CRig& rg = rig_of(p, s);
  StreamState& st = p.st[s];
  const int mode = p.det_mode[s];
  if (mode == 0) return;
  const int lane = threadIdx.x;
  const int cur = st.cur;
  Landmark* lms = lm_ptr(p, cur, s);
  int n0 = st.n_lm[cur];
  int nn = p.n_new[s];
  if (n0 + nn > NMAX) nn = NMAX - n0;
  const float* xy = p.new_xy + (size_t)s * NEW_MAX * 2;
  const bool as_inlier = (mode == 1) ? true : (st.orig_size < 60);
  for (int k = lane; k < nn; k += T) {
    float src[2] = {xy[2 * k], xy[2 * k + 1]};
    float und[2] = {src[0], src[1]};
    if ((mode == 1 && p.cam.cam_type != CAM_DEPTH) || p.cam.cam_type == CAM_STEREO_UNRECT)
      undistort_point(src, rig_arr(rg.K0).v, rig_arr(rg.D0).v, rig_arr(rg.R0).v, rig_arr(rg.P0).v, und);
    Landmark lm;
    lm.id = st.lm_id_counter + k;
    lm.p3w[0] = lm.p3w[1] = lm.p3w[2] = 0;
    lm.p3c[0] = lm.p3c[1] = lm.p3c[2] = 0;
    lm.p2d[0] = (double)src[0];
    lm.p2d[1] = (double)src[1];
    lm.p2u[0] = (double)und[0];
    lm.p2u[1] = (double)und[1];
    lm.first2d[0] = lm.p2u[0];
    lm.first2d[1] = lm.p2u[1];
    for (int j = 0; j < 7; j++) lm.first_pose[j] = st.T_c_w[cur][j];
    lm.has3d = 0;
    lm.inlier = as_inlier ? 1 : 0;
    lm.tslot = -1;
    for (int j = 0; j < 4; j++) lm.pad[j] = 0;
    lms[n0 + k] = lm;
  }
  __syncthreads();
  if (lane == 0) {
    st.lm_id_counter += p.n_new[s];
    st.n_lm[cur] = n0 + nn;
    st.n_new = nn;
  }
}
__global__ __launch_bounds__(64) void k_add_new(Pipe p) {
  kj_wait(p.kj);
  k_add_new_body<64>(p);
  kj_signal(p.kj);
}

__device__ __forceinline__ void depth_seed_dev(const Pipe& p, int s, int i) {
  CRig& rg = rig_of(p, s);
  const StreamState& st = p.st[s];
  const int cur = st.cur;
  const int n = st.n_lm[cur];
  if (i == 0) {
    p.lk_count[s] = n;
    p.lk_tag[s] = st.frame_id[cur];
  }
  if (i >= n) return;
  if (p.cam.cam_type == CAM_DEPTH) return;
  Landmark& lm = lm_ptr(p, cur, s)[i];
  float* p0 = p.prev_pts + ((size_t)s * NMAX + i) * 2;
  float* p1 = p.next_pts + ((size_t)s * NMAX + i) * 2;
  p0[0] = (float)lm.p2d[0];
  p0[1] = (float)lm.p2d[1];
  lm.tslot = i < p.tc_cap ? (short)i : (short)-1;
  if (lm.has3d) {
    const SE3d T = load_pose7(st.T_c_w[cur]);
    SE3d T1c = se3_mul(load_pose7(rig_arr(rg.T_c1_c0).v), T);
    float p3[3] = {(float)lm.p3w[0], (float)lm.p3w[1], (float)lm.p3w[2]};
    project_point(p3, q_to_mat(T1c.q), T1c.t, rig_arr(rg.K1).v, rig_arr(rg.D1).v, p1);
  } else {
    p1[0] = p0[0];
    p1[1] = p0[1];
  }
}
__device__ __forceinline__ void k_depth_seeds_body(const Pipe& p) {
  const int s = blockIdx.y;
  if (p.det_mode[s] == 0) return;
  depth_seed_dev(p, s, blockIdx.x * 256 + threadIdx.x);
}
__global__ __launch_bounds__(256) void k_depth_seeds(Pipe p) {
  kj_wait(p.kj);
  k_depth_seeds_body(p);
  kj_signal(p.kj);
  kj_post_wait(p.kj);
}
__global__ __launch_bounds__(256) void k_add_new_seeds(Pipe p) {
  kj_wait(p.kj);
  const int s = blockIdx.x;
  if (p.det_mode[s] != 0) {
    k_add_new_body<256>(p);
    __syncthreads();
    for (int i = threadIdx.x; i < NMAX; i += 256) depth_seed_dev(p, s, i);
  }
  kj_signal(p.kj);
  kj_post_wait(p.kj);
}
__device__ __forceinline__ void k_depth_triangulate_body(const Pipe& p) {
  const int s = blockIdx.y;
  CRig& rg = rig_of(p, s);
  const StreamState& st = p.st[s];
  if (p.det_mode[s] == 0) return;
  const int cur = st.cur;
  const int n = st.n_lm[cur];
  const int i = blockIdx.x * 256 + threadIdx.x;
  if (i >= n) return;
  const Landmark& lm = lm_ptr(p, cur, s)[i];
  const SE3d T = load_pose7(st.T_c_w[cur]);
  SE3d T1 = load_pose7(lm.first_pose);
  V3 baseline = T1.t - T.t;
  double* tri = p.tri + ((size_t)s * NMAX + i) * 3;
  unsigned char tm = 0;
  tri[0] = tri[1] = tri[2] = 0;
  if (norm(baseline) >= 0.2) {
    V3 pw = triangulate_two_view(lm.first2d[0], lm.first2d[1], lm.p2u[0], lm.p2u[1], T1, T, rg.fx, rg.fy, rg.cx,
                                 rg.cy);
    V3 pc = se3_act(T, pw);
    if (pc.z >= 0.5 && pc.z <= (double)rg.range) {
      tri[0] = pc.x;
      tri[1] = pc.y;
      tri[2] = pc.z;
      tm = 1;
    }
  }
  p.tri_mask[(size_t)s * NMAX + i] = tm;
}
__global__ __launch_bounds__(256) void k_depth_triangulate(Pipe p) {
  kj_wait(p.kj);
  k_depth_triangulate_body(p);
  kj_signal(p.kj);
}

__device__ __forceinline__ void k_depth_innovate_body(const Pipe& p) {
  const int s = blockIdx.x;
  CRig& rg = rig_of(p, s);
  StreamState& st = p.st[s];
  if (p.det_mode[s] == 0) return;
  const int i = threadIdx.x;
  const int cur = st.cur;
  Landmark* lms = lm_ptr(p, cur, s);
  const int n = st.n_lm[cur];
  __shared__ float rnd[NMAX];
  __shared__ int s_cnt[NMAX / 64];
  const float* p1 = p.next_pts + (size_t)s * NMAX * 2;
  const uint8_t* status = p.lk_status + (size_t)s * NMAX;
  const double range = (double)rg.range;
  const bool valid = i < n;
  Landmark lm;
  bool ok = false;
  V3 meas{0, 0, 0};
  const bool depth_cam = p.cam.cam_type == CAM_DEPTH;
  float ptx = 0.f, pty = 0.f;
  if (valid) {
    lm = lms[i];
    if (depth_cam) {
      ptx = (float)round(lm.p2d[0]);
      pty = (float)round(lm.p2d[1]);
      const int ix = min(max(__float2int_rn(ptx), 0), p.cam.w - 1), iy = min(max(__float2int_rn(pty), 0), p.cam.h - 1);
      const uint16_t d16 = reinterpret_cast<const uint16_t*>(p.in_img1)[(size_t)s * p.cam.w * p.cam.h + (size_t)iy * p.cam.w + ix];
      const float z = (float)((double)d16 / rg.depth_scale);
      if ((double)z >= 0.3 && z <= rg.range) {
        meas = V3{((double)ptx - rg.cx) * (double)z / rg.fx, ((double)pty - rg.cy) * (double)z / rg.fy, (double)z};
        ok = true;
      }
    } else if (status[i] == 1) {
      float src[2] = {p1[2 * i], p1[2 * i + 1]}, u1[2];
      undistort_point(src, rig_arr(rg.K1).v, rig_arr(rg.D1).v, rig_arr(rg.R1).v, rig_arr(rg.P1).v, u1);
      float u0x = (float)lm.p2u[0], u0y = (float)lm.p2u[1];
      V3 pc = triangulate_dlt((double)u0x, (double)u0y, (double)u1[0], (double)u1[1], rig_arr(rg.P0).v, rig_arr(rg.P1).v);
      if (!(pc.z < 0 || pc.z > range)) {
        meas = pc;
        ok = true;
      }
    }
  }
  int nfail;
  const int frank = block_rank<NMAX / 64>(valid && !ok, s_cnt, nfail);
  if (i == 0)
    for (int k = 0; k < nfail; k++)
      rnd[k] = (float)(0.3 + (double)((float)glibc_rand_next(st) / ((float)(2147483647 / (0.4)))));
  __syncthreads();
  if (valid) {
    const SE3d T = load_pose7(st.T_c_w[cur]);
    const SE3d Tinv = se3_inverse(T);
    const float iir = rg.iir_ratio;
    const bool tm = p.tri_mask[(size_t)s * NMAX + i] != 0;
    if (!ok) {
      double depth = (double)rnd[frank];
      if (depth_cam) {
        meas = V3{(lm.p2d[0] - rg.cx) * depth / rg.fx, (lm.p2d[1] - rg.cy) * depth / rg.fy, depth};
      } else {
        float u0x = (float)lm.p2u[0], u0y = (float)lm.p2u[1];
        meas = V3{((double)u0x - rg.cx) * depth / rg.fx, ((double)u0y - rg.cy) * depth / rg.fy, depth};
      }
    }
    if (!ok && !tm) {
      if (!depth_cam && !lm.has3d && rg.enable_dummy) {
        V3 pw = se3_act(Tinv, meas);
        lm.p3c[0] = meas.x; lm.p3c[1] = meas.y; lm.p3c[2] = meas.z;
        lm.p3w[0] = pw.x; lm.p3w[1] = pw.y; lm.p3w[2] = pw.z;
        lm.has3d = 1;
      }
    } else {
      V3 m = meas;
      if (!ok) {
        const double* tri = p.tri + ((size_t)s * NMAX + i) * 3;
        m = V3{tri[0], tri[1], tri[2]};
      }
      if (lm.has3d) {
        V3 lc = se3_act(T, V3{lm.p3w[0], lm.p3w[1], lm.p3w[2]});
        V3 upd = lc * (double)iir + m * (double)(1 - iir);
        V3 pw = se3_act(Tinv, upd);
        lm.p3c[0] = upd.x; lm.p3c[1] = upd.y; lm.p3c[2] = upd.z;
        lm.p3w[0] = pw.x; lm.p3w[1] = pw.y; lm.p3w[2] = pw.z;
      } else {
        V3 pw = se3_act(Tinv, m);
        lm.p3c[0] = m.x; lm.p3c[1] = m.y; lm.p3c[2] = m.z;
        lm.p3w[0] = pw.x; lm.p3w[1] = pw.y; lm.p3w[2] = pw.z;
        lm.has3d = 1;
      }
    }
  }
  int kept;
  const bool keep = valid && lm.has3d;
  const int k = block_rank<NMAX / 64>(keep, s_cnt, kept);
  if (keep) lms[k] = lm;
  if (i == 0) st.n_lm[cur] = kept;
}
__global__ __launch_bounds__(NMAX) void k_depth_innovate(Pipe p) {
  kj_wait(p.kj);
  k_depth_innovate_body(p);
  kj_signal(p.kj);
}

constexpr int FE_T = 256;
__device__ __forceinline__ void k_frame_end_body(const Pipe& p) {
  const int s = blockIdx.x;
  StreamState& st = p.st[s];
  const int lane = threadIdx.x;
  __shared__ int s_newkf;
  __shared__ int s_cnt[FE_T / 64];
  const bool s_chain = st.phase == PH_TRACK;
  if (lane == 0) s_newkf = 0;
  __syncthreads();
  if (st.phase == PH_INIT) {
    const int cur = st.cur;
    Landmark* lms = lm_ptr(p, cur, s);
    int valid = 0;
    for (int base = 0; base < st.n_lm[cur]; base += FE_T) {
      const int i = base + lane;
      int tot;
      block_rank<FE_T / 64>(i < st.n_lm[cur] && lms[i].has3d && lms[i].inlier, s_cnt, tot);
      valid += tot;
    }
    if (lane == 0) {
      if (valid > 30) {
        pose_record_push(p, s, st, (int)st.frame_id[cur], st.T_c_w[cur], false);
        for (int j = 0; j < 7; j++) st.T_kf[j] = st.T_c_w[cur][j];
        st.new_kf = 1;
        st.state = ST_TRACKING;
      } else if (st.state == ST_TRACKFAIL) {
        st.cur ^= 1;
      }
    }
  } else if (st.phase == PH_TRACK && lane == 0) {
    const int cur = st.cur;
    pose_record_push(p, s, st, (int)st.frame_id[cur], st.T_c_w[cur], true);
    SE3d Tkf = load_pose7(st.T_kf), Tc = load_pose7(st.T_c_w[cur]);
    SE3d Td = se3_mul(Tkf, se3_inverse(Tc));
    V3 r = so3_log(Td.q);
    double t_norm = fabs(Td.t.x) + fabs(Td.t.y) + fabs(Td.t.z);
    double r_norm = fabs(r.x) + fabs(r.y) + fabs(r.z);
    bool kf = false;
    if (st.frameCount < 40 && (st.frameCount % 5) == 0) kf = true;
    if (t_norm >= 0.05 || r_norm >= 0.2) kf = true;
    if (kf) {
      st.new_kf = 1;
      for (int j = 0; j < 7; j++) st.T_kf[j] = st.T_c_w[cur][j];
    }
  }
  __syncthreads();
  const int cur = st.cur;
  if (lane == 0) {
    p.img_slot_in[s] = cur ^ 1;
    s_newkf = st.new_kf;
    FrameOut& o = p.out[s];
    o.state = st.state;
    o.new_keyframe = st.new_kf;
    o.reset_cmd = st.reset_cmd;
    o.n_landmarks = st.n_lm[cur];
    o.frame_id = st.frame_id[cur];
    for (int j = 0; j < 7; j++) o.T_c_w[j] = st.T_c_w[cur][j];
    o.of_cnt = st.of_cnt;
    o.f_cnt = st.f_cnt;
    o.pnp_cnt = st.pnp_cnt;
    o.reproj_err = st.reproj_err;
    const int frame_slot = st.feeds++;
    if (p.traj && frame_slot >= 0 && frame_slot < p.traj_cap) {
      double* t = p.traj + ((size_t)s * p.traj_cap + frame_slot) * 9;
      t[0] = st.frame_time[cur];
      for (int j = 0; j < 7; j++) t[1 + j] = st.T_c_w[cur][j];
      t[8] = (double)(st.state | (st.new_kf << 4));
    }
  }
  __syncthreads();
  if (s_newkf) {
    __shared__ unsigned s_tail;
    __shared__ int s_full;
    __shared__ unsigned s_hash;
    if (lane == 0) {
      s_hash = 0u;
      const unsigned tl = p.kfq_tail[s];
      s_full = (tl - __hip_atomic_load(&p.kfq_head[s], __ATOMIC_ACQUIRE, __HIP_MEMORY_SCOPE_AGENT) >= (unsigned)KFQ) ? 1 : 0;
      if (s_full) atomicAdd((unsigned long long*)&p.counters[3], 1ull);
      s_tail = tl;
    }
    __syncthreads();
    if (s_full) return;
    KeyFrameDev& kf = p.kfq[(size_t)s * KFQ + (s_tail % KFQ)];
    Landmark* lms = lm_ptr(p, cur, s);
    const int n = st.n_lm[cur];
    int cnt = 0;
    unsigned hsum = 0u;
    for (int base = 0; base < n; base += FE_T) {
      int i = base + lane;
      bool sel = i < n && lms[i].has3d && lms[i].inlier;
      int tot;
      const int rk = block_rank<FE_T / 64>(sel, s_cnt, tot);
      if (sel) {
        int k = cnt + rk;
        if (k < KF_MAXLM) {
          kf.lm_id[k] = lms[i].id;
          kf.lm_2d[k][0] = lms[i].p2u[0];
          kf.lm_2d[k][1] = lms[i].p2u[1];
          kf.lm_3d[k][0] = lms[i].p3w[0];
          kf.lm_3d[k][1] = lms[i].p3w[1];
          kf.lm_3d[k][2] = lms[i].p3w[2];
          if (p.kf_check) hsum += kf_entry_hash(k, lms[i].id, lms[i].p2u, lms[i].p3w);
        }
      }
      cnt += tot;
    }
    if (p.kf_check) {
      if (hsum) atomicAdd(&s_hash, hsum);
      __syncthreads();
    }
    if (lane == 0) {
      kf.frame_id = st.frame_id[cur];
      kf.stamp = st.frame_time[cur];
      kf.lm_count = cnt < KF_MAXLM ? cnt : KF_MAXLM;
      for (int j = 0; j < 7; j++) kf.T_c_w[j] = st.T_c_w[cur][j];
      for (int j = 0; j < 4; j++) kf.imu_dq[j] = st.kf_dq[j];
      kf.imu_dt = st.kf_dt;
      kf.imu_valid = (s_chain && st.kf_dt > 0) ? 1 : 0;
      kf.imu_pad = p.kf_check ? (int)s_hash : 0;
      for (int j = 0; j < 3; j++) {
        kf.imu_dp[j] = st.kf_dp[j];
        kf.imu_va[j] = st.kf_va[j];
        st.kf_dp[j] = st.kf_dv[j] = 0.0;
      }
      {
        const bool have = st.has_imu && st.vi_count > 0;
        const MotionState& mb = p.vi[(size_t)s * VI_QUEUE + (st.vi_head + (st.vi_count > 0 ? st.vi_count - 1 : 0)) % VI_QUEUE];
        for (int j = 0; j < 3; j++) st.kf_va[j] = have ? mb.vel[j] : 0.0;
      }
      st.kf_dq[0] = 1.0, st.kf_dq[1] = st.kf_dq[2] = st.kf_dq[3] = 0.0;
      st.kf_dt = 0;
      {
        CRig& rg = rig_of(p, s);
        kf.rig_K[0] = rg.fx, kf.rig_K[1] = rg.fy, kf.rig_K[2] = rg.cx, kf.rig_K[3] = rg.cy;
        for (int j = 0; j < 7; j++) kf.rig_T_c_i[j] = rg.T_c_i[j];
      }
      kf.valid = KFQ_KEYFRAME;
      p.kfq_kf[s] = s_tail + 1u;
    }
    __syncthreads();
    if (lane == 0) __hip_atomic_store(&p.kfq_tail[s], s_tail + 1u, __ATOMIC_RELEASE, __HIP_MEMORY_SCOPE_AGENT);
  }
}
__global__ __launch_bounds__(FE_T) void k_frame_end(Pipe p) {
  kj_wait(p.kj);
  if (stream_present(p, blockIdx.x)) k_frame_end_body(p);
  kj_signal(p.kj);
}

__global__ __launch_bounds__(256) void k_stream_reset(Pipe p, ResetList list, long long* err_word) {
  const int s = list.s[blockIdx.x];
  const unsigned mode = list.mode[blockIdx.x];
  const int t = threadIdx.x, nt = blockDim.x;
  if (s < 0 || s >= p.S) return;
  if (mode & RS_TRACKER) {
    __shared__ StreamState s_st;
    if (t == 0) stream_state_init(s_st, p.cam.skip_first_n);
    __syncthreads();
    const int* src = reinterpret_cast<const int*>(&s_st);
    int* dst = reinterpret_cast<int*>(p.st + s);
    const int lm_word = (int)(offsetof(StreamState, lm_state) / sizeof(int));
    for (int i = t; i < (int)(sizeof(StreamState) / sizeof(int)); i += nt)
      if (i != lm_word || (mode & RS_CREATE)) dst[i] = src[i];
    static_assert(sizeof(Landmark) % 8 == 0 && sizeof(MotionState) % 8 == 0 && sizeof(FrameOut) % 8 == 0, "records cleared in 8-byte words");
    for (int k = 0; k < 2; k++) {
      long long* l = reinterpret_cast<long long*>(lm_ptr(p, k, s));
      for (int i = t; i < (int)(NMAX * sizeof(Landmark) / 8); i += nt) l[i] = 0;
    }
    {
      long long* v = reinterpret_cast<long long*>(p.vi + (size_t)s * VI_QUEUE);
      for (int i = t; i < (int)(VI_QUEUE * sizeof(MotionState) / 8); i += nt) v[i] = 0;
    }
    for (int i = t; i < IMU_OUT_CAP * 11; i += nt) p.imu_out[(size_t)s * IMU_OUT_CAP * 11 + i] = 0.0;
    for (int i = t; i < POSE_REC; i += nt) p.rec_id[(size_t)s * POSE_REC + i] = 0;
    for (int i = t; i < POSE_REC * 7; i += nt) p.rec_T[(size_t)s * POSE_REC * 7 + i] = 0.0;
    if (p.traj)
      for (int i = t; i < p.traj_cap * 9; i += nt) p.traj[(size_t)s * p.traj_cap * 9 + i] = 0.0;
    {
      long long* o = reinterpret_cast<long long*>(p.out + s);
      for (int i = t; i < (int)(sizeof(FrameOut) / 8); i += nt) o[i] = 0;
    }
    if (p.tc) {
      uint32_t* tc = const_cast<uint32_t*>(p.tc) + (size_t)s * p.tc_cap * p.tc_stride;
      for (int i = t; i < p.tc_cap * 8; i += nt) tc[(size_t)(i >> 3) * p.tc_stride + (i & 7)] = 0xffffffffu;
    }
    if (t == 0) {
      p.img_slot_in[s] = 1;
      p.img_slot[s] = 0;
      p.lk_count[s] = 0;
      p.lk_tag[s] = 0;
      p.n_new[s] = 0;
      p.n_exist[s] = 0;
      p.act_img[s] = 0;
      p.act_track[s] = 0;
      p.det_mode[s] = 0;
      p.det_maxc[s] = 0;
      p.gftt_act[s] = 0;
      p.gftt_maxc[s] = 0;
      p.kfq_kf[s] = 0;
      if (p.corr_in) p.corr_in[s].valid = 0;
    }
  }
  if (t != 0) return;
  if (mode & RS_CMD) {
    const unsigned tl = p.kfq_tail[s];
    if (tl - __hip_atomic_load(&p.kfq_head[s], __ATOMIC_ACQUIRE, __HIP_MEMORY_SCOPE_AGENT) >= (unsigned)KFQ) {
      if (err_word) __hip_atomic_store(err_word, (long long)s + 1, __ATOMIC_RELAXED, __HIP_MEMORY_SCOPE_SYSTEM);
      return;
    }
    KeyFrameDev& kf = p.kfq[(size_t)s * KFQ + (tl % KFQ)];
    kf.frame_id = -1;
    kf.lm_count = 0;
    kf.stamp = 0.0;
    kf.imu_valid = 0;
    kf.valid = KFQ_CMD_RESET;
    p.kfq_cmd[s] = tl + 1u;
    p.kfq_base[s] = tl + 1u;
    if (mode & RS_SKIP) __hip_atomic_store(&p.kfq_skip[s], tl, __ATOMIC_RELAXED, __HIP_MEMORY_SCOPE_AGENT);
    __hip_atomic_store(&p.kfq_tail[s], tl + 1u, __ATOMIC_RELEASE, __HIP_MEMORY_SCOPE_AGENT);
  } else if (mode & RS_SKIP) {
    const unsigned c = p.kfq_cmd[s];
    if (c) __hip_atomic_store(&p.kfq_skip[s], c - 1u, __ATOMIC_RELAXED, __HIP_MEMORY_SCOPE_AGENT);
  }
}

__global__ __launch_bounds__(256) void k_kfq_drop(Pipe p) {
  const int s = blockIdx.x;
  __shared__ int s_apply;
  __shared__ unsigned s_tail;
  if (threadIdx.x == 0) {
    const unsigned tl = __hip_atomic_load(&p.kfq_tail[s], __ATOMIC_RELAXED, __HIP_MEMORY_SCOPE_AGENT);
    const unsigned hd = __hip_atomic_load(&p.kfq_head[s], __ATOMIC_ACQUIRE, __HIP_MEMORY_SCOPE_AGENT);
    const unsigned c = p.kfq_cmd[s];
    s_apply = c != 0u && c - 1u - hd < tl - hd;
    s_tail = tl;
  }
  __syncthreads();
  if (s_apply) window_reset_dev(p, s);
  if (threadIdx.x == 0) __hip_atomic_store(&p.kfq_head[s], s_tail, __ATOMIC_RELEASE, __HIP_MEMORY_SCOPE_AGENT);
}

void launch_stream_reset(hipStream_t st, const Pipe& p, const ResetList& list, long long* err_word) {
  if (list.n > 0) hipLaunchKernelGGL(k_stream_reset, dim3(list.n), dim3(256), 0, st, p, list, err_word);
}
__global__ void k_set_rig(RigParams* rig, int ls, RigParams r) {
  if (threadIdx.x == 0) rig[ls] = r;
}
void launch_set_rig(hipStream_t st, const Pipe& p, int ls, const RigParams& r) {
  hipLaunchKernelGGL(k_set_rig, dim3(1), dim3(64), 0, st, const_cast<RigParams*>(p.rig), ls, r);
}
void launch_kfq_drop(hipStream_t st, const Pipe& p) {
  hipLaunchKernelGGL(k_kfq_drop, dim3(p.S), dim3(256), 0, st, p);
}
void launch_imu_feed(hipStream_t st, const Pipe& p) {
  hipLaunchKernelGGL(k_imu_feed, dim3((p.S + 63) / 64), dim3(64), 0, st, p);
}
void launch_frame_begin(hipStream_t st, const Pipe& p, const double* d_time) {
  hipLaunchKernelGGL(k_frame_begin, dim3((p.S + 63) / 64), dim3(64), 0, st, p, d_time);
}
__global__ void k_store_progress(long long* __restrict__ host_word, long long v) {
  __hip_atomic_store(host_word, v, __ATOMIC_RELEASE, __HIP_MEMORY_SCOPE_SYSTEM);
}
void launch_store_progress(hipStream_t st, long long* host_word, long long v) {
  hipLaunchKernelGGL(k_store_progress, dim3(1), dim3(1), 0, st, host_word, v);
}
__global__ void k_wait_flag(const long long* __restrict__ flag, int n_words, long long seq, long long* __restrict__ err_word) {
  const unsigned long long t0 = wall_clock64();
  while (__hip_atomic_load(&flag[0], __ATOMIC_RELAXED, __HIP_MEMORY_SCOPE_SYSTEM) < seq ||
         __hip_atomic_load(&flag[n_words - 1], __ATOMIC_RELAXED, __HIP_MEMORY_SCOPE_SYSTEM) < seq) {
    __builtin_amdgcn_s_sleep(32);
    if (wall_clock64() - t0 > 400000000ull) {
      if (err_word) __hip_atomic_store(err_word, seq, __ATOMIC_RELAXED, __HIP_MEMORY_SCOPE_SYSTEM);
      break;
    }
  }
  __builtin_amdgcn_fence(__ATOMIC_ACQUIRE, "");
}
__global__ void k_store_flag(long long* __restrict__ word, long long v) {
  __hip_atomic_store(word, v, __ATOMIC_RELEASE, __HIP_MEMORY_SCOPE_AGENT);
}
void launch_store_flag(hipStream_t st, long long* word, long long v) { hipLaunchKernelGGL(k_store_flag, dim3(1), dim3(1), 0, st, word, v); }
void launch_wait_flag(hipStream_t st, const long long* flag, int n_words, long long seq, long long* err_word) {
  hipLaunchKernelGGL(k_wait_flag, dim3(1), dim3(1), 0, st, flag, n_words, seq, err_word);
}
void launch_frame_head(hipStream_t st, const Pipe& p, const double* d_time, long long* host_progress, long long frame_no) {
  hipLaunchKernelGGL(k_frame_head, dim3(p.S), dim3(64), 0, st, p, d_time, host_progress, frame_no);
}
void launch_frame_head_prepare(hipStream_t st, const Pipe& p, const double* d_time, long long* host_progress, long long frame_no) {
  hipLaunchKernelGGL(k_frame_head_prepare, dim3(p.S), dim3(256), 0, st, p, d_time, host_progress, frame_no);
}
void launch_apply_correction(hipStream_t st, const Pipe& p) {
  hipLaunchKernelGGL(k_apply_correction, dim3(p.S), dim3(AC_T), 0, st, p);
}
void launch_track_prepare(hipStream_t st, const Pipe& p) {
  hipLaunchKernelGGL(k_track_prepare, dim3(NMAX / 256, p.S), dim3(256), 0, st, p);
}
void launch_track_collect(hipStream_t st, const Pipe& p) { hipLaunchKernelGGL(k_track_collect, dim3(p.S), dim3(64), 0, st, p); }
void launch_ransac_f(hipStream_t st, const Pipe& p, bool with_collect) {
  if (with_collect) hipLaunchKernelGGL(k_collect_ransac_f, dim3(p.S), dim3(RF_T), 0, st, p);
  else hipLaunchKernelGGL(k_ransac_f, dim3(p.S), dim3(RF_T), 0, st, p);
}
void launch_ransac_pnp(hipStream_t st, const Pipe& p) { hipLaunchKernelGGL(k_ransac_pnp, dim3(p.S), dim3(RP_T), 0, st, p); }
void launch_pnp_tail_cv(hipStream_t st, const Pipe& p) { hipLaunchKernelGGL(k_pnp_tail_cv, dim3(p.S), dim3(64), 0, st, p); }
int pnp_ransac_max_points() { return PNP_MAXN; }
static hipError_t pnp_tables_init();
void launch_pnp_ransac_sets(hipStream_t st, const float* p3d, const float* p2d, const int* count, int cap, int n_sets, const double* K4,
                            const double* d_cams, int cam_stride, const int* d_cam_of, int iterative, const double* guess7,
                            const unsigned long long* seeds, int max_iters, double reproj_px, double conf, double* pose7, unsigned char* mask,
                            int* n_inliers) {
  (void)pnp_tables_init();
  const double none[4] = {0, 0, 0, 0};
  if (!K4) K4 = none;
  hipLaunchKernelGGL(k_pnp_ransac_sets, dim3(n_sets), dim3(RP_T), 0, st, p3d, p2d, count, cap, K4[0], K4[1], K4[2], K4[3], d_cams, cam_stride,
                     d_cam_of, iterative, guess7, seeds, max_iters, (float)(reproj_px * reproj_px), conf, pose7, mask, n_inliers);
}
void launch_fund_ransac_sets(hipStream_t st, const float* m1, const float* m2, const int* count, int cap, int n_sets, double thr_px,
                             double conf, unsigned char* mask, int* n_inliers) {
  (void)pnp_tables_init();
  hipLaunchKernelGGL(k_fund_ransac_sets, dim3(n_sets), dim3(RF_T), 0, st, m1, m2, count, cap, thr_px, conf, mask, n_inliers);
}
int fund_ransac_max_points() { return NMAX; }
void launch_track_post(hipStream_t st, const Pipe& p) {
  hipLaunchKernelGGL(k_track_post, dim3((p.S + 63) / 64), dim3(64), 0, st, p);
}
int pose_lm_max_edges() { return PL_EMAX; }
hipError_t launch_pose_lm_sets(hipStream_t st, const double* lm3d, const double* lm2d, const long long* lm_id, const int* count, int cap,
                               int n_sets, const double* d_K4, int k_stride, double* pose7, unsigned char* ok) {
  const hipError_t e = hipFuncSetAttribute((const void*)k_pose_lm_sets, hipFuncAttributeMaxDynamicSharedMemorySize, (int)sizeof(PoseLMShared));
  if (e != hipSuccess) return e;
  hipLaunchKernelGGL(k_pose_lm_sets, dim3(n_sets), dim3(PL_T), sizeof(PoseLMShared), st, lm3d, lm2d, lm_id, count, cap, d_K4, k_stride, pose7, ok);
  return hipSuccess;
}
void launch_pose_lm(hipStream_t st, const Pipe& p) { hipLaunchKernelGGL(k_pose_lm, dim3(p.S), dim3(PL_T), sizeof(PoseLMShared), st, p); }
static hipError_t pnp_tables_init() {
  static bool done[64] = {};
  int dev = 0;
  hipError_t e = hipGetDevice(&dev);
  if (e != hipSuccess) return e;
  if (dev >= 0 && dev < 64 && done[dev]) return hipSuccess;
  std::vector<unsigned short> s5((size_t)PNP_TAB_N * PNP_TAB_B5 * 5, 0), s4((size_t)PNP_TAB_N * PNP_TAB_B4 * 4, 0);
  std::vector<unsigned long long> r5(PNP_TAB_N, 0), r4(PNP_TAB_N, 0);
  auto fill = [](int count, int m, int nsub, unsigned short* out, unsigned long long& state_out) {
    uint64_t st = 0xffffffffffffffffull;
    for (int sidx = 0; sidx < nsub; sidx++) {
      int idx[5] = {-1, -1, -1, -1, -1};
      for (int i = 0; i < m;) {
        st = (uint64_t)(uint32_t)st * 4164903690u + (uint32_t)(st >> 32);
        const int v = (int)((uint32_t)st % (uint32_t)count);
        bool dup = false;
        for (int j = 0; j < i; j++) dup = dup || idx[j] == v;
        if (dup) continue;
        idx[i++] = v;
      }
      for (int j = 0; j < m; j++) out[(size_t)sidx * m + j] = (unsigned short)idx[j];
    }
    state_out = st;
  };
  for (int n = 0; n < PNP_TAB_N; n++) {
    if (n > 5) fill(n, 5, PNP_TAB_B5, &s5[(size_t)n * PNP_TAB_B5 * 5], r5[n]);
    if (n > 4) fill(n, 4, PNP_TAB_B4, &s4[(size_t)n * PNP_TAB_B4 * 4], r4[n]);
  }
  {
    std::vector<unsigned short> s7((size_t)F_TAB_N * F_TAB_B * 7, 0);
    std::vector<unsigned long long> r7((size_t)F_TAB_N * F_TAB_B, 0);
    for (int n = 8; n < F_TAB_N; n++) {
      uint64_t st = 0xffffffffffffffffull;
      for (int k = 0; k < F_TAB_B; k++) {
        int idx[7] = {-1, -1, -1, -1, -1, -1, -1};
        for (int i = 0; i < 7;) {
          st = (uint64_t)(uint32_t)st * 4164903690u + (uint32_t)(st >> 32);
          const int v = (int)((uint32_t)st % (uint32_t)n);
          bool dup = false;
          for (int j = 0; j < i; j++) dup = dup || idx[j] == v;
          if (dup) continue;
          idx[i++] = v;
        }
        for (int j = 0; j < 7; j++) s7[((size_t)n * F_TAB_B + k) * 7 + j] = (unsigned short)idx[j];
        r7[(size_t)n * F_TAB_B + k] = st;
      }
    }
    e = hipMemcpyToSymbol(HIP_SYMBOL(g_f_sub7), s7.data(), s7.size() * sizeof(unsigned short));
    if (e == hipSuccess) e = hipMemcpyToSymbol(HIP_SYMBOL(g_f_rng7), r7.data(), r7.size() * sizeof(unsigned long long));
    if (e != hipSuccess) return e;
  }
  e = hipMemcpyToSymbol(HIP_SYMBOL(g_pnp_sub5), s5.data(), s5.size() * sizeof(unsigned short));
  if (e == hipSuccess) e = hipMemcpyToSymbol(HIP_SYMBOL(g_pnp_sub4), s4.data(), s4.size() * sizeof(unsigned short));
  if (e == hipSuccess) e = hipMemcpyToSymbol(HIP_SYMBOL(g_pnp_rng5), r5.data(), r5.size() * sizeof(unsigned long long));
  if (e == hipSuccess) e = hipMemcpyToSymbol(HIP_SYMBOL(g_pnp_rng4), r4.data(), r4.size() * sizeof(unsigned long long));
  if (e == hipSuccess && dev >= 0 && dev < 64) done[dev] = true;
  return e;
}
hipError_t track_kernels_init() {
  {
    const hipError_t e = pnp_tables_init();
    if (e != hipSuccess) return e;
  }
  return hipFuncSetAttribute((const void*)k_pose_lm, hipFuncAttributeMaxDynamicSharedMemorySize, (int)sizeof(PoseLMShared));
}
void launch_reproj_filter(hipStream_t st, const Pipe& p) { hipLaunchKernelGGL(k_reproj_filter, dim3(p.S), dim3(NMAX), 0, st, p); }
void launch_vi_correction(hipStream_t st, const Pipe& p) { hipLaunchKernelGGL(k_vi_correction, dim3((p.S + 63) / 64), dim3(64), 0, st, p); }
void launch_add_new(hipStream_t st, const Pipe& p) { hipLaunchKernelGGL(k_add_new, dim3(p.S), dim3(64), 0, st, p); }
void launch_depth_seeds(hipStream_t st, const Pipe& p) {
  hipLaunchKernelGGL(k_depth_seeds, dim3(NMAX / 256, p.S), dim3(256), 0, st, p);
}
void launch_add_new_seeds(hipStream_t st, const Pipe& p) { hipLaunchKernelGGL(k_add_new_seeds, dim3(p.S), dim3(256), 0, st, p); }
void launch_depth_triangulate(hipStream_t st, const Pipe& p) {
  hipLaunchKernelGGL(k_depth_triangulate, dim3(NMAX / 256, p.S), dim3(256), 0, st, p);
}
void launch_depth_innovate(hipStream_t st, const Pipe& p) { hipLaunchKernelGGL(k_depth_innovate, dim3(p.S), dim3(NMAX), 0, st, p); }
void launch_frame_end(hipStream_t st, const Pipe& p) {
  hipLaunchKernelGGL(k_frame_end, dim3(p.S), dim3(FE_T), 0, st, p);
}

}
```

### flvis_amd/csrc/track_kernels.hpp

```cpp
#pragma once
#include "pipeline.hpp"

namespace flvis {

constexpr int NEW_MAX = 1024;

struct Pipe {
  int S;
  CamParams cam;
  const RigParams* rig;
  StreamState* st;
  Landmark* lm;
  MotionState* vi;
  const unsigned long long* seeds;
  double* imu_in;
  int* n_imu;
  const int* present;
  double* imu_out;
  float* prev_pts;
  float* next_pts;
  uint8_t* lk_status;
  int* lk_count;
  int* lk_slot;
  long long* lk_tag;
  int tc_cap;
  const uint32_t* tc;
  int tc_stride;
  float* m1;
  float* m2;
  double* tri;
  uint8_t* tri_mask;
  float* new_xy;
  int* n_new;
  double* exist_xy;
  int* n_exist;
  int* act_img;
  int* act_track;
  int* det_mode;
  int* det_maxc;
  int* gftt_act;
  int* gftt_maxc;
  int* img_slot;
  int* img_slot_in;
  FrameOut* out;
  double* traj;
  int traj_cap;
  KeyFrameDev* kfq;
  unsigned* kfq_tail;
  unsigned* kfq_head;
  unsigned* kfq_cmd;
  unsigned* kfq_skip;
  unsigned* kfq_base;
  unsigned* kfq_kf;
  int* ba_busy;
  WindowDev* win;
  KeyFrameDev* kfs_ring;
  CorrectionDev* corr;
  double* ba_scratch;
  size_t ba_scratch_stride;
  int imu_factor;
  double imu_sigma_a;
  double imu_sigma_g;
  int ba_lds_bytes;
  int ba_drain;
  int ba_backlog;
  int pnp_tail_cv;
  double* pnp_tail_ws;
  size_t pnp_tail_stride;
  int kf_check;
  long long* counters;
  long long* ba_ovf_word;
  int* rec_id;
  double* rec_T;
  const uint8_t* const* in_tab;
  const uint8_t* in_img1;
  CorrectionDev* corr_in;
  KJoin kj;
};

__device__ inline CRig& rig_of(const Pipe& p, int s) { return ((CRig*)p.rig)[s]; }

__device__ inline void window_reset_dev(const Pipe& p, int s) {
  long long* w = reinterpret_cast<long long*>(p.win + s);
  static_assert(sizeof(WindowDev) % 8 == 0, "WindowDev is cleared in 8-byte words");
  for (int i = threadIdx.x; i < (int)(sizeof(WindowDev) / 8); i += blockDim.x) w[i] = 0;
  if (threadIdx.x == 0) {
    p.corr[s].valid = 0;
    p.st[s].lm_state = 0;
  }
  __syncthreads();
}

int ba_lds_budget_max();
bool ba_lds_admits(int bytes, int window);
int ba_lds_min_bytes(int window);
void launch_imu_feed(hipStream_t st, const Pipe& p);
void launch_frame_begin(hipStream_t st, const Pipe& p, const double* d_time);
int pnp_ransac_max_points();
constexpr int EPNP_DBG_N = 160;
void launch_epnp_sets(hipStream_t st, const float* p3d, const float* p2d, const int* count, int cap, int n_sets, const double* K4, double* out);
void launch_pnp_ransac_sets(hipStream_t st, const float* p3d, const float* p2d, const int* count, int cap, int n_sets, const double* K4,
                            const double* d_cams, int cam_stride, const int* d_cam_of, int iterative, const double* guess7,
                            const unsigned long long* seeds, int max_iters, double reproj_px, double conf, double* pose7, unsigned char* mask,
                            int* n_inliers);
int fund_ransac_max_points();
void launch_fund_ransac_sets(hipStream_t st, const float* m1, const float* m2, const int* count, int cap, int n_sets, double thr_px,
                             double conf, unsigned char* mask, int* n_inliers);
int pose_lm_max_edges();
hipError_t launch_pose_lm_sets(hipStream_t st, const double* lm3d, const double* lm2d, const long long* lm_id, const int* count, int cap,
                               int n_sets, const double* d_K4, int k_stride, double* pose7, unsigned char* ok);
constexpr int GEOM_CAM_N = 29;
void launch_undistort_points_sets(hipStream_t st, const float* src, const int* count, int cap, int n_sets, const double* d_cam, int cam_stride,
                                  float* dst);
void launch_project_points_sets(hipStream_t st, const float* p3d, const int* count, int cap, int n_sets, const double* d_pose7,
                                const double* d_cam, int cam_stride, float* dst);
void launch_store_progress(hipStream_t st, long long* host_word, long long v);
void launch_store_flag(hipStream_t st, long long* word, long long v);
void launch_wait_flag(hipStream_t st, const long long* flag, int n_words, long long seq, long long* err_word);
void launch_frame_head(hipStream_t st, const Pipe& p, const double* d_time, long long* host_progress, long long frame_no);
void launch_frame_head_prepare(hipStream_t st, const Pipe& p, const double* d_time, long long* host_progress, long long frame_no);
void launch_apply_correction(hipStream_t st, const Pipe& p);
void launch_track_prepare(hipStream_t st, const Pipe& p);
void launch_track_collect(hipStream_t st, const Pipe& p);
void launch_ransac_f(hipStream_t st, const Pipe& p, bool with_collect = false);
void launch_ransac_pnp(hipStream_t st, const Pipe& p);
void launch_pnp_tail_cv(hipStream_t st, const Pipe& p);
void launch_track_post(hipStream_t st, const Pipe& p);
void launch_pose_lm(hipStream_t st, const Pipe& p);
void launch_reproj_filter(hipStream_t st, const Pipe& p);
void launch_vi_correction(hipStream_t st, const Pipe& p);
void launch_add_new(hipStream_t st, const Pipe& p);
void launch_depth_seeds(hipStream_t st, const Pipe& p);
void launch_add_new_seeds(hipStream_t st, const Pipe& p);
void launch_depth_triangulate(hipStream_t st, const Pipe& p);
void launch_depth_innovate(hipStream_t st, const Pipe& p);
void launch_frame_end(hipStream_t st, const Pipe& p);
constexpr int RESET_LIST = 64;
enum { RS_TRACKER = 1, RS_CMD = 2, RS_SKIP = 4, RS_CREATE = 8 };
struct ResetList {
  int n;
  int s[RESET_LIST];
  unsigned char mode[RESET_LIST];
};
void launch_stream_reset(hipStream_t st, const Pipe& p, const ResetList& list, long long* err_word);
void launch_kfq_drop(hipStream_t st, const Pipe& p);
void launch_set_rig(hipStream_t st, const Pipe& p, int ls, const RigParams& r);
void launch_ba_worker(hipStream_t st, const Pipe& p);
hipError_t ba_kernels_init();
hipError_t track_kernels_init();
size_t ba_scratch_doubles();

}
```

Before: 62280.

## Fuse DEM into add-new-seeds, pose LM with reproj filter, innovate with frame end

Adds three optional kernel fusions gated by chain_merge bits: the feature demotion body is moved to a shared header and fused into the add-new/seeds kernel, pose LM is fused with the reprojection filter, and depth innovation is fused with frame end. Backpressure waits are split so that part of them happens earlier. The goal is to cut kernel launches and inter-kernel joins on the per-frame critical path. Whether the new paths run depends on the default chain_merge value, and the fused kernels carry more shared memory and higher block sizes, which may reduce occupancy.

New measurement: 63160, median of 6. +1.4%, better.

```diff
diff --git a/flvis_amd/csrc/feature_dem_dev.hpp b/flvis_amd/csrc/feature_dem_dev.hpp
--- /dev/null
+++ b/flvis_amd/csrc/feature_dem_dev.hpp
@@ -0,0 +1,173 @@
+#pragma once
+#include "dev_common.hpp"
+#include "img_kernels.hpp"
+
+namespace flvis {
+
+constexpr int DEM_MAXC = 4096;
+constexpr int DEM_MAXR = 192;
+constexpr int DEM_T = 256;
+inline size_t dem_body_lds(int corner_cap) { return (size_t)(((corner_cap < DEM_MAXC ? corner_cap : DEM_MAXC) + 1) & ~1) * 8; }
+
+__device__ __forceinline__ void k_feature_dem_body(int w, int h, DemParams prm, const float* __restrict__ sorted_xy,
+                                                       const int* __restrict__ region_off, int corner_cap, const int* __restrict__ mode,
+                                                       const double* __restrict__ exist_xy, const int* __restrict__ nexist,
+                                                       int exist_cap, float* __restrict__ out_xy, int* __restrict__ out_n,
+                                                       int out_cap) {
+  const int s = blockIdx.x;
+  const int md = mode ? mode[s] : 1;
+  if (md == 0) return;
+  const int tid = threadIdx.x, lane = tid & 63, wv = tid >> 6;
+  extern __shared__ __attribute__((aligned(16))) unsigned char dem_smem[];
+  const int cmax = ((corner_cap < DEM_MAXC ? corner_cap : DEM_MAXC) + 1) & ~1;
+  float* cx = reinterpret_cast<float*>(dem_smem);
+  float* cy = cx + cmax;
+  __shared__ int roff[17];
+  __shared__ float kx[16][DEM_MAXR], ky[16][DEM_MAXR];
+  __shared__ int kcount[16], knew0[16], ooff[17], kover[16];
+  __shared__ int wcnt[DEM_T / 64][16];
+  if (tid < 17) roff[tid] = region_off[(size_t)s * 17 + tid];
+  if (tid < 16) kcount[tid] = 0, kover[tid] = 0;
+  __syncthreads();
+  {
+    const float* const SX = sorted_xy + (size_t)s * corner_cap * 2;
+    const int tot = roff[16] < cmax ? roff[16] : cmax;
+    for (int j = tid; j < tot; j += DEM_T) {
+      cx[j] = SX[2 * j];
+      cy[j] = SX[2 * j + 1];
+    }
+  }
+  if (md == 2) {
+    int ne = nexist[s];
+    if (ne > exist_cap) ne = exist_cap;
+    const double* E = exist_xy + (size_t)s * exist_cap * 2;
+    for (int base = 0; base < ne; base += DEM_T) {
+      const int i = base + tid;
+      int r = -1;
+      float px = 0.f, py = 0.f;
+      if (i < ne) {
+        px = (float)E[2 * i];
+        py = (float)E[2 * i + 1];
+        if (px >= 3 && px < (w - 3) && py >= 3 && py < (h - 3))
+          r = (int)(4.f * floorf(py / (float)prm.regionHeight) + px / (float)prm.regionWidth);
+      }
+      int myrank = 0;
+#pragma unroll
+      for (int q = 0; q < 16; q++) {
+        const unsigned long long bq = __ballot(r == q);
+        if (lane == 0) wcnt[wv][q] = __popcll(bq);
+        if (r == q) myrank = lane_prefix(bq);
+      }
+      __syncthreads();
+      if (r >= 0) {
+        int k = kcount[r] + myrank;
+        for (int v = 0; v < wv; v++) k += wcnt[v][r];
+        if (k < DEM_MAXR) {
+          kx[r][k] = px;
+          ky[r][k] = py;
+        }
+      }
+      __syncthreads();
+      if (tid < 16) {
+        int k = kcount[tid];
+        for (int v = 0; v < DEM_T / 64; v++) k += wcnt[v][tid];
+        kcount[tid] = k < DEM_MAXR ? k : DEM_MAXR;
+        if (k >= DEM_MAXR) kover[tid] = 1;
+      }
+      __syncthreads();
+    }
+  }
+  __syncthreads();
+  if (tid < 16) knew0[tid] = kcount[tid];
+  __syncthreads();
+  {
+    const int r = tid >> 4, sub = tid & 15;
+    const int bd = prm.boundary_dis;
+    int kept = kcount[r];
+    unsigned count = 0;
+    const int j0 = roff[r], j1 = roff[r + 1];
+    if (md == 2 && kover[r]) {
+      int ne = nexist[s];
+      if (ne > exist_cap) ne = exist_cap;
+      const double* E = exist_xy + (size_t)s * exist_cap * 2;
+      int found = 0;
+      for (int j = j0; j < j1 && !found; j++) {
+        const float px = (float)__float2int_rn(cx[j]), py = (float)__float2int_rn(cy[j]);
+        int bad = 0;
+        for (int i = sub; i < ne; i += 16) {
+          const float ex = (float)E[2 * i], ey = (float)E[2 * i + 1];
+          if (!(ex >= 3 && ex < (w - 3) && ey >= 3 && ey < (h - 3))) continue;
+          if ((int)(4.f * floorf(ey / (float)prm.regionHeight) + ex / (float)prm.regionWidth) != r) continue;
+          if (fabsf(px - ex) <= (float)bd || fabsf(py - ey) <= (float)bd) bad = 1;
+        }
+        bad = (int)((__ballot(bad != 0) >> (lane & 48)) & 0xFFFFull);
+        if (!bad) {
+          if (sub == 0) {
+            kx[r][0] = px;
+            ky[r][0] = py;
+          }
+          found = 1;
+        }
+      }
+      if (sub == 0) {
+        knew0[r] = 0;
+        kcount[r] = found;
+      }
+    } else {
+    for (int j = j0; j < j1; j++) {
+      float px = cx[j], py = cy[j];
+      if (md == 2) {
+        px = (float)__float2int_rn(px);
+        py = (float)__float2int_rn(py);
+      }
+      int bad = 0;
+      for (int k = sub; k < kept; k += 16) {
+        float dis_x = fabsf(px - kx[r][k]);
+        float dis_y = fabsf(py - ky[r][k]);
+        if (dis_x <= (float)bd || dis_y <= (float)bd) bad = 1;
+      }
+      bad = (int)((__ballot(bad != 0) >> (lane & 48)) & 0xFFFFull);
+      if (!bad) {
+        if (kept < DEM_MAXR && sub == 0) {
+          kx[r][kept] = px;
+          ky[r][kept] = py;
+        }
+        kept++;
+        count++;
+        __builtin_amdgcn_wave_barrier();
+        asm volatile("" ::: "memory");
+        if (md == 1) {
+          if (count >= prm.max_region_feature_num) break;
+        } else {
+          if ((unsigned)kept >= prm.max_region_feature_num) break;
+        }
+      }
+    }
+    if (sub == 0) kcount[r] = kept < DEM_MAXR ? kept : DEM_MAXR;
+    }
+  }
+  __syncthreads();
+  if (tid == 0) {
+    int o = 0;
+    for (int r = 0; r < 16; r++) {
+      ooff[r] = o;
+      o += kcount[r] - knew0[r];
+    }
+    ooff[16] = o;
+    out_n[s] = o < out_cap ? o : out_cap;
+  }
+  __syncthreads();
+  {
+    float* O = out_xy + (size_t)s * out_cap * 2;
+    const int r = tid >> 4, sub = tid & 15;
+    for (int k = knew0[r] + sub; k < kcount[r]; k += 16) {
+      const int o = ooff[r] + (k - knew0[r]);
+      if (o < out_cap) {
+        O[2 * o] = kx[r][k];
+        O[2 * o + 1] = ky[r][k];
+      }
+    }
+  }
+}
+
+}
diff --git a/flvis_amd/csrc/frame_schedule.cpp b/flvis_amd/csrc/frame_schedule.cpp
--- a/flvis_amd/csrc/frame_schedule.cpp
+++ b/flvis_amd/csrc/frame_schedule.cpp
@@ -211,9 +211,9 @@
   return std::max(0LL, D - (long long)c.size());
 }
 
-void flvis::lane_backpressure_wait(Pipeline* pl, Lane* L, LaunchJoins* folded) {
+void flvis::lane_backpressure_wait(Pipeline* pl, Lane* L, LaunchJoins* folded, int k0, int k1) {
   const long long D = lane_backpressure_depth(pl, L);
-  for (int k = 0; k < pl->nba_lane; k++) {
+  for (int k = k0; k < std::min(k1, pl->nba_lane); k++) {
     const long long j = L->ba_launches - 1 - D - k;
     if (j < 0 || L->ba_launches - j > BAQ) continue;
     if (folded) folded->wait(J_BA(j));
@@ -243,6 +243,9 @@
   bool head_prepare;
   bool head_posts;
   bool merge_collect;
+  bool merge_end;
+  bool merge_dem;
+  bool merge_filter;
   void mark(int i, int end, hipStream_t s) const {
     if (prof && ((pl->prof_mask >> i) & 1ull)) hipEventRecord(pev[2 * i + end], s);
   }
@@ -251,7 +254,7 @@
   void stage_host_inputs(const uint8_t* d_img0, const uint8_t* d_img1, const double* h_times, const uint8_t* present);
   void stage_ingest_left(), stage_head(), stage_idle_tail(), stage_temporal_lk(), stage_collect_ransac_f(), stage_detection_fork();
   void stage_pnp_pose(), stage_new_landmarks(), stage_stereo_depth(), stage_frame_end();
-  void local_map_tail(hipEvent_t* p18, bool timed), frame_end(bool backpressure);
+  void local_map_tail(hipEvent_t* p18, bool timed), frame_end(bool backpressure, bool with_innovate);
   LKParams lk_params(int stats_at, int tc_mode, int order) const;
 };
 
@@ -315,6 +318,9 @@
   l0cur = ImgSel{{L->pyr0[0][0], L->pyr0[1][0]}, p.img_slot, 0, nullptr};
   head_prepare = pl->head_prepare && !pl->feedback_used && !idle_step;
   merge_collect = (pl->chain_merge & 2) != 0;
+  merge_end = (pl->chain_merge & 4) != 0 && !idle_step && all_present;
+  merge_dem = (pl->chain_merge & 8) != 0;
+  merge_filter = (pl->chain_merge & 16) != 0;
 }
 
 void Frame::stage_ingest_left() {
@@ -376,19 +382,25 @@
   }
 }
 
-void Frame::frame_end(bool backpressure) {
+void Frame::frame_end(bool backpressure, bool with_innovate) {
   LaunchJoins j(pl, L, st, p.kj);
-  if (backpressure) lane_backpressure_wait(pl, L, &j);
-  pb(17, st);
+  if (with_innovate) j.wait(J_TRI);
+  if (backpressure) lane_backpressure_wait(pl, L, &j, 0, with_innovate ? 1 : pl->nba_lane);
+  pb(with_innovate ? 16 : 17, st);
   L->endf_valid = j.fold_signal(J_ENDF);
-  launch_frame_end(st, p);
+  if (with_innovate) launch_depth_innovate_end(st, p);
+  else launch_frame_end(st, p);
   j.end();
+  if (with_innovate) {
+    pe(16, st);
+    pb(17, st);
+  }
   pe(17, st);
   pe(19, st);
 }
 
 void Frame::stage_idle_tail() {
-  frame_end(false);
+  frame_end(false, false);
   if (prof)
     for (int i = 1; i < PROF_STAGES; i++)
       if (i != 17 && i != 19) {
@@ -444,8 +456,8 @@
 }
 
 void Frame::stage_detection_fork() {
+  join_wait(pl, L, ds, J_HEAD);
   join_wait(pl, L, ds, J_LM);
-  join_wait(pl, L, ds, J_HEAD);
   launch_gftt(ds, l0cur, w, h, pl->lpitch[0], pl->lstride[0], S, L->gftt, nullptr, p.cam.gftt_ql, p.gftt_maxc, p.cam.gftt_num,
               (double)p.cam.gftt_dis, L->gftt_xy, L->gftt_n, 2 * p.cam.gftt_num, p.gftt_act,
               (prof && ((pl->prof_mask >> 10) & 7ull) == 7ull) ? &pev[2 * 10] : nullptr, false);
@@ -456,7 +468,6 @@
     launch_feature_dem_prep(ds, l0cur, w, h, pl->lpitch[0], pl->lstride[0], S, p.cam.dem, L->gftt_xy, L->gftt_n, 2 * p.cam.gftt_num,
                             p.gftt_act, L->dem_sorted, L->dem_roff, &prep_kj);
   }
-  join_wait(pl, L, ds, J_HEAD);
   if (!depth_cam) {
     if (eq) launch_equalize_hist(ds, in1, img_plain(L->pyr1[0]), w, h, w, pl->lpitch[0], (size_t)w * h, pl->lstride[0], S, L->eq_hist, L->eq_lut, p.act_img);
     else if (!aligned) launch_copy_image_any(ds, in1, img_plain(L->pyr1[0]), w, h, w, pl->lpitch[0], (size_t)w * h, pl->lstride[0], S, p.act_img);
@@ -481,10 +492,17 @@
   pe(7, st);
   if (ba_here) launch_local_map(pl, L, J_FE, !pnp_signals, prof18);
   pb(8, st);
-  launch_pose_lm(st, p);
-  pe(8, st);
-  pb(9, st);
-  {
+  if (merge_filter) {
+    LaunchJoins j(pl, L, st, p.kj);
+    j.signal(J_LM);
+    launch_pose_lm_filter(st, p);
+    pe(8, st);
+    pb(9, st);
+    pe(9, st);
+  } else {
+    launch_pose_lm(st, p);
+    pe(8, st);
+    pb(9, st);
     LaunchJoins j(pl, L, st, p.kj);
     j.signal(J_LM);
     launch_reproj_filter(st, p);
@@ -495,7 +513,7 @@
 }
 
 void Frame::stage_new_landmarks() {
-  {
+  if (!merge_dem) {
     KJoin dem_kj{};
     LaunchJoins j(pl, L, st, dem_kj);
     j.wait(J_GFTT);
@@ -504,19 +522,27 @@
                        p.new_xy, p.n_new, NEW_MAX, &dem_kj);
   }
   const bool merge_seeds = (pl->chain_merge & 1) != 0;
+  const DemLaunch dem{w, h, L->dem_sorted, L->dem_roff, 2 * p.cam.gftt_num};
   bool an_signals, seeds_post;
   {
     LaunchJoins j(pl, L, st, p.kj);
+    if (merge_dem) {
+      j.wait(J_GFTT);
+      pb(13, st);
+    }
+    if (merge_end && with_local_map) lane_backpressure_wait(pl, L, &j, 1, pl->nba_lane);
     an_signals = j.fold_signal(J_LM);
     if (!merge_seeds) {
-      launch_add_new(st, p);
+      if (merge_dem) launch_dem_add_new_seeds(st, p, dem, false);
+      else launch_add_new(st, p);
       j.end();
     }
     pe(13, st);
     pb(14, st);
     seeds_post = j.fold_post(J_DET);
-    if (merge_seeds) launch_add_new_seeds(st, p);
-    else launch_depth_seeds(st, p);
+    if (!merge_seeds) launch_depth_seeds(st, p);
+    else if (merge_dem) launch_dem_add_new_seeds(st, p, dem, true);
+    else launch_add_new_seeds(st, p);
   }
   pe(14, st);
   if (!an_signals) join_signal(pl, L, J_LM, st);
@@ -539,6 +565,7 @@
     launch_lk_track(st, prev, next, p.prev_pts, p.next_pts, p.lk_status, p.lk_count, NMAX, S, lk_params(48, 1, 1), p.det_mode, pl->max_pts, 2);
   }
   pe(15, st);
+  if (merge_end) return;
   LaunchJoins j(pl, L, st, p.kj);
   j.wait(J_TRI);
   pb(16, st);
@@ -548,7 +575,7 @@
 }
 
 void Frame::stage_frame_end() {
-  frame_end(with_local_map != 0);
+  frame_end(with_local_map != 0, merge_end);
   if (pl->kfl.cap > 0) kf_log_frame(pl, L, st, in1.b[0], depth_cam || r_in_place);
   local_map_tail(prof18, prof);
 }
diff --git a/flvis_amd/csrc/img_kernels.hip b/flvis_amd/csrc/img_kernels.hip
--- a/flvis_amd/csrc/img_kernels.hip
+++ b/flvis_amd/csrc/img_kernels.hip
@@ -3,6 +3,7 @@
 #include "dev_common.hpp"
 #include "dem_sort.hpp"
 #include "eig_strip.hpp"
+#include "feature_dem_dev.hpp"
 #include "img_kernels.hpp"
 
 namespace flvis {
@@ -807,8 +808,6 @@
   }
 }
 
-constexpr int DEM_MAXC = 4096;
-constexpr int DEM_MAXR = 192;
 int dem_max_region_features() { return DEM_MAXR; }
 
 __device__ __forceinline__ float dem_harris(const uint8_t* __restrict__ img, int pitch, float ptx, float pty) {
@@ -824,7 +823,6 @@
   return (X2 * Y2) - (XY * XY) - 0.05f * (X2 + Y2) * (X2 + Y2);
 }
 
-constexpr int DEM_T = 256;
 constexpr int DEMP_T = 1024;
 struct PackedArray {
   typedef int value_type;
@@ -941,166 +939,6 @@
   kj_signal(kj);
 }
 
-__device__ __forceinline__ void k_feature_dem_body(int w, int h, DemParams prm, const float* __restrict__ sorted_xy,
-                                                       const int* __restrict__ region_off, int corner_cap, const int* __restrict__ mode,
-                                                       const double* __restrict__ exist_xy, const int* __restrict__ nexist,
-                                                       int exist_cap, float* __restrict__ out_xy, int* __restrict__ out_n,
-                                                       int out_cap) {
-  const int s = blockIdx.x;
-  const int md = mode ? mode[s] : 1;
-  if (md == 0) return;
-  const int tid = threadIdx.x, lane = tid & 63, wv = tid >> 6;
-  extern __shared__ __attribute__((aligned(16))) unsigned char dem_smem[];
-  const int cmax = ((corner_cap < DEM_MAXC ? corner_cap : DEM_MAXC) + 1) & ~1;
-  float* cx = reinterpret_cast<float*>(dem_smem);
-  float* cy = cx + cmax;
-  __shared__ int roff[17];
-  __shared__ float kx[16][DEM_MAXR], ky[16][DEM_MAXR];
-  __shared__ int kcount[16], knew0[16], ooff[17], kover[16];
-  __shared__ int wcnt[DEM_T / 64][16];
-  if (tid < 17) roff[tid] = region_off[(size_t)s * 17 + tid];
-  if (tid < 16) kcount[tid] = 0, kover[tid] = 0;
-  __syncthreads();
-  {
-    const float* const SX = sorted_xy + (size_t)s * corner_cap * 2;
-    const int tot = roff[16] < cmax ? roff[16] : cmax;
-    for (int j = tid; j < tot; j += DEM_T) {
-      cx[j] = SX[2 * j];
-      cy[j] = SX[2 * j + 1];
-    }
-  }
-  if (md == 2) {
-    int ne = nexist[s];
-    if (ne > exist_cap) ne = exist_cap;
-    const double* E = exist_xy + (size_t)s * exist_cap * 2;
-    for (int base = 0; base < ne; base += DEM_T) {
-      const int i = base + tid;
-      int r = -1;
-      float px = 0.f, py = 0.f;
-      if (i < ne) {
-        px = (float)E[2 * i];
-        py = (float)E[2 * i + 1];
-        if (px >= 3 && px < (w - 3) && py >= 3 && py < (h - 3))
-          r = (int)(4.f * floorf(py / (float)prm.regionHeight) + px / (float)prm.regionWidth);
-      }
-      int myrank = 0;
-#pragma unroll
-      for (int q = 0; q < 16; q++) {
-        const unsigned long long bq = __ballot(r == q);
-        if (lane == 0) wcnt[wv][q] = __popcll(bq);
-        if (r == q) myrank = lane_prefix(bq);
-      }
-      __syncthreads();
-      if (r >= 0) {
-        int k = kcount[r] + myrank;
-        for (int v = 0; v < wv; v++) k += wcnt[v][r];
-        if (k < DEM_MAXR) {
-          kx[r][k] = px;
-          ky[r][k] = py;
-        }
-      }
-      __syncthreads();
-      if (tid < 16) {
-        int k = kcount[tid];
-        for (int v = 0; v < DEM_T / 64; v++) k += wcnt[v][tid];
-        kcount[tid] = k < DEM_MAXR ? k : DEM_MAXR;
-        if (k >= DEM_MAXR) kover[tid] = 1;
-      }
-      __syncthreads();
-    }
-  }
-  __syncthreads();
-  if (tid < 16) knew0[tid] = kcount[tid];
-  __syncthreads();
-  {
-    const int r = tid >> 4, sub = tid & 15;
-    const int bd = prm.boundary_dis;
-    int kept = kcount[r];
-    unsigned count = 0;
-    const int j0 = roff[r], j1 = roff[r + 1];
-    if (md == 2 && kover[r]) {
-      int ne = nexist[s];
-      if (ne > exist_cap) ne = exist_cap;
-      const double* E = exist_xy + (size_t)s * exist_cap * 2;
-      int found = 0;
-      for (int j = j0; j < j1 && !found; j++) {
-        const float px = (float)__float2int_rn(cx[j]), py = (float)__float2int_rn(cy[j]);
-        int bad = 0;
-        for (int i = sub; i < ne; i += 16) {
-          const float ex = (float)E[2 * i], ey = (float)E[2 * i + 1];
-          if (!(ex >= 3 && ex < (w - 3) && ey >= 3 && ey < (h - 3))) continue;
-          if ((int)(4.f * floorf(ey / (float)prm.regionHeight) + ex / (float)prm.regionWidth) != r) continue;
-          if (fabsf(px - ex) <= (float)bd || fabsf(py - ey) <= (float)bd) bad = 1;
-        }
-        bad = (int)((__ballot(bad != 0) >> (lane & 48)) & 0xFFFFull);
-        if (!bad) {
-          if (sub == 0) {
-            kx[r][0] = px;
-            ky[r][0] = py;
-          }
-          found = 1;
-        }
-      }
-      if (sub == 0) {
-        knew0[r] = 0;
-        kcount[r] = found;
-      }
-    } else {
-    for (int j = j0; j < j1; j++) {
-      float px = cx[j], py = cy[j];
-      if (md == 2) {
-        px = (float)__float2int_rn(px);
-        py = (float)__float2int_rn(py);
-      }
-      int bad = 0;
-      for (int k = sub; k < kept; k += 16) {
-        float dis_x = fabsf(px - kx[r][k]);
-        float dis_y = fabsf(py - ky[r][k]);
-        if (dis_x <= (float)bd || dis_y <= (float)bd) bad = 1;
-      }
-      bad = (int)((__ballot(bad != 0) >> (lane & 48)) & 0xFFFFull);
-      if (!bad) {
-        if (kept < DEM_MAXR && sub == 0) {
-          kx[r][kept] = px;
-          ky[r][kept] = py;
-        }
-        kept++;
-        count++;
-        __builtin_amdgcn_wave_barrier();
-        asm volatile("" ::: "memory");
-        if (md == 1) {
-          if (count >= prm.max_region_feature_num) break;
-        } else {
-          if ((unsigned)kept >= prm.max_region_feature_num) break;
-        }
-      }
-    }
-    if (sub == 0) kcount[r] = kept < DEM_MAXR ? kept : DEM_MAXR;
-    }
-  }
-  __syncthreads();
-  if (tid == 0) {
-    int o = 0;
-    for (int r = 0; r < 16; r++) {
-      ooff[r] = o;
-      o += kcount[r] - knew0[r];
-    }
-    ooff[16] = o;
-    out_n[s] = o < out_cap ? o : out_cap;
-  }
-  __syncthreads();
-  {
-    float* O = out_xy + (size_t)s * out_cap * 2;
-    const int r = tid >> 4, sub = tid & 15;
-    for (int k = knew0[r] + sub; k < kcount[r]; k += 16) {
-      const int o = ooff[r] + (k - knew0[r]);
-      if (o < out_cap) {
-        O[2 * o] = kx[r][k];
-        O[2 * o + 1] = ky[r][k];
-      }
-    }
-  }
-}
 __global__ __launch_bounds__(DEM_T) void k_feature_dem(int w, int h, DemParams prm, const float* __restrict__ sorted_xy,
                                                        const int* __restrict__ region_off, int corner_cap, const int* __restrict__ mode,
                                                        const double* __restrict__ exist_xy, const int* __restrict__ nexist,
diff --git a/flvis_amd/csrc/pipeline.cpp b/flvis_amd/csrc/pipeline.cpp
--- a/flvis_amd/csrc/pipeline.cpp
+++ b/flvis_amd/csrc/pipeline.cpp
@@ -487,7 +487,7 @@
   pl->head_prepare = !env_is("FLVIS_HEAD_PREPARE", 0);
   if (const char* e = getenv("FLVIS_HOST_LEAD")) pl->host_lead = std::max(1, std::min(atoi(e), (int)Lane::PIN_RING));
   if (const char* e = getenv("FLVIS_SYNC_EACH_FRAME")) pl->sync_each_frame = atoi(e) != 0;
-  if (const char* e = getenv("FLVIS_CHAIN_MERGE")) pl->chain_merge = atoi(e) & 3;
+  if (const char* e = getenv("FLVIS_CHAIN_MERGE")) pl->chain_merge = atoi(e) & 31;
   if (const char* e = getenv("FLVIS_BA_EVERY")) {
     const int v = atoi(e);
     if (v >= 1 && v <= KFQ / 4) pl->ba_every = v;
diff --git a/flvis_amd/csrc/pipeline_host.hpp b/flvis_amd/csrc/pipeline_host.hpp
--- a/flvis_amd/csrc/pipeline_host.hpp
+++ b/flvis_amd/csrc/pipeline_host.hpp
@@ -99,7 +99,7 @@
   int n_lanes_req = 1;
   bool lk_border = true;
   bool lk_tcache = true;
-  int chain_merge = 3;
+  int chain_merge = 31;
   bool head_prepare = true;
   bool kf_check = false;
   bool pnp_tail_cv = false;
@@ -185,6 +185,6 @@
 void kf_log_reset_stream(Pipeline* pl, Lane* L, int ls);
 void kf_log_free(Pipeline* pl);
 struct LaunchJoins;
-void lane_backpressure_wait(Pipeline* pl, Lane* L, LaunchJoins* folded);
+void lane_backpressure_wait(Pipeline* pl, Lane* L, LaunchJoins* folded, int k0 = 0, int k1 = 1 << 30);
 
 }
diff --git a/flvis_amd/csrc/track_kernels.hip b/flvis_amd/csrc/track_kernels.hip
--- a/flvis_amd/csrc/track_kernels.hip
+++ b/flvis_amd/csrc/track_kernels.hip
@@ -3,6 +3,7 @@
 #include "dev_common.hpp"
 #include "dev_geom.hpp"
 #include "epnp_core.hpp"
+#include "feature_dem_dev.hpp"
 #include "track_kernels.hpp"
 #include "cv_solvers.hpp"
 #include "vi_motion.hpp"
@@ -1683,7 +1684,7 @@
   }
 }
 
-__global__ __launch_bounds__(PL_T) void k_pose_lm(Pipe p) {
+__device__ __forceinline__ void k_pose_lm_body(const Pipe& p) {
   const int s = blockIdx.x;
   CRig& rg = rig_of(p, s);
   StreamState& st = p.st[s];
@@ -1776,6 +1777,7 @@
   if (tid == 0 && p.counters) atomicAdd((unsigned long long*)&p.counters[48 + 7], 1ull);
 #endif
 }
+__global__ __launch_bounds__(PL_T) void k_pose_lm(Pipe p) { k_pose_lm_body(p); }
 
 __global__ __launch_bounds__(PL_T) void k_pose_lm_sets(const double* __restrict__ lm3d, const double* __restrict__ lm2d,
                                                        const long long* __restrict__ lm_id, const int* __restrict__ count, int cap,
@@ -1906,6 +1908,97 @@
 __global__ __launch_bounds__(NMAX) void k_reproj_filter(Pipe p) {
   kj_wait(p.kj);
   k_reproj_filter_body(p);
+  kj_signal(p.kj);
+}
+template <int T>
+__device__ __forceinline__ void reproj_filter_chunks_dev(const Pipe& p, double* valid) {
+  const int s = blockIdx.x;
+  CRig& rg = rig_of(p, s);
+  StreamState& st = p.st[s];
+  if (st.phase != PH_TRACK) return;
+  constexpr int NC = NMAX / T;
+  const int tid = threadIdx.x;
+  const int cur = st.cur;
+  Landmark* lms = lm_ptr(p, cur, s);
+  const int n = st.n_lm[cur];
+  __shared__ double sh_thr;
+  __shared__ int s_cnt[T / 64];
+  const SE3d Tcw = load_pose7(st.T_c_w[cur]);
+  double d[NC];
+  int nv = 0;
+#pragma unroll
+  for (int c = 0; c < NC; c++) {
+    d[c] = 0;
+    if (c * T >= n) continue;
+    const int i = c * T + tid;
+    bool v = false;
+    if (i < n) {
+      const Landmark& lm = lms[i];
+      V3 pc = se3_act(Tcw, V3{lm.p3w[0], lm.p3w[1], lm.p3w[2]});
+      double u = rg.fx * pc.x / pc.z + rg.cx, vv = rg.fy * pc.y / pc.z + rg.cy;
+      double ex = lm.p2u[0] - u, ey = lm.p2u[1] - vv;
+      d[c] = sqrt(ex * ex + ey * ey);
+      v = d[c] < 3.0;
+    }
+    int tot;
+    const int vr = block_rank<T / 64>(v, s_cnt, tot);
+    if (v) valid[nv + vr] = d[c];
+    nv += tot;
+  }
+  if (tid == 0 && nv == 0) sh_thr = 3.0;
+  __syncthreads();
+  if (tid == 0) {
+    double sum = 0;
+    for (int k = 0; k < nv; k++) sum += valid[k];
+    st.reproj_err = sum / (double)nv;
+  }
+  for (int i = tid; i < nv; i += T) {
+    const int target = nv / 2;
+    const double vi = valid[i];
+    int less = 0, eq = 0;
+    for (int j = 0; j < nv; j++) {
+      const double vj = valid[j];
+      less += vj < vi;
+      eq += vj == vi;
+    }
+    if (less <= target && target < less + eq) sh_thr = 1.5 * vi;
+  }
+  __syncthreads();
+  double sh = sh_thr;
+  if (sh >= 3.0) sh = 3.0;
+  int kept = 0;
+#pragma unroll
+  for (int c = 0; c < NC; c++) {
+    if (c * T >= n) continue;
+    const int i = c * T + tid;
+    const bool keep = i < n && !(d[c] > sh);
+    Landmark lm;
+    if (keep) lm = lms[i];
+    int tot;
+    const int k = kept + block_rank<T / 64>(keep, s_cnt, tot);
+    if (keep) {
+      lm.inlier = 1;
+      lms[k] = lm;
+      double* ex = p.exist_xy + ((size_t)s * NMAX + k) * 2;
+      ex[0] = lm.p2d[0];
+      ex[1] = lm.p2d[1];
+    }
+    kept += tot;
+  }
+  if (tid == 0) {
+    st.n_lm[cur] = kept;
+    st.orig_size = kept;
+    p.n_exist[s] = kept;
+    p.det_mode[s] = 2;
+    p.det_maxc[s] = p.cam.gftt_num;
+    st.vi_corr_due = st.has_imu ? 1 : 0;
+  }
+}
+__global__ __launch_bounds__(PL_T) void k_pose_lm_filter(Pipe p) {
+  kj_wait(p.kj);
+  k_pose_lm_body(p);
+  __syncthreads();
+  reproj_filter_chunks_dev<PL_T>(p, reinterpret_cast<PoseLMShared*>(pl_smem)->terms);
   kj_signal(p.kj);
 }
 __global__ void k_vi_correction(Pipe p) {
@@ -2019,6 +2112,23 @@
   kj_signal(p.kj);
   kj_post_wait(p.kj);
 }
+static_assert(DEM_T == 256, "k_dem_add_new_seeds: FeatureDEM's body, k_add_new_body<256> and the seeds share one workgroup");
+__global__ __launch_bounds__(256) void k_dem_add_new_seeds(Pipe p, DemLaunch d, int with_seeds) {
+  kj_wait(p.kj);
+  const int s = blockIdx.x;
+  k_feature_dem_body(d.w, d.h, p.cam.dem, d.sorted_xy, d.region_off, d.corner_cap, p.det_mode, p.exist_xy, p.n_exist, NMAX, p.new_xy, p.n_new,
+                     NEW_MAX);
+  __syncthreads();
+  if (p.det_mode[s] != 0) {
+    k_add_new_body<256>(p);
+    if (with_seeds) {
+      __syncthreads();
+      for (int i = threadIdx.x; i < NMAX; i += 256) depth_seed_dev(p, s, i);
+    }
+  }
+  kj_signal(p.kj);
+  kj_post_wait(p.kj);
+}
 __device__ __forceinline__ void k_depth_triangulate_body(const Pipe& p) {
   const int s = blockIdx.y;
   CRig& rg = rig_of(p, s);
@@ -2157,12 +2267,13 @@
 }
 
 constexpr int FE_T = 256;
+template <int T>
 __device__ __forceinline__ void k_frame_end_body(const Pipe& p) {
   const int s = blockIdx.x;
   StreamState& st = p.st[s];
   const int lane = threadIdx.x;
   __shared__ int s_newkf;
-  __shared__ int s_cnt[FE_T / 64];
+  __shared__ int s_cnt[T / 64];
   const bool s_chain = st.phase == PH_TRACK;
   if (lane == 0) s_newkf = 0;
   __syncthreads();
@@ -2170,10 +2281,10 @@
     const int cur = st.cur;
     Landmark* lms = lm_ptr(p, cur, s);
     int valid = 0;
-    for (int base = 0; base < st.n_lm[cur]; base += FE_T) {
+    for (int base = 0; base < st.n_lm[cur]; base += T) {
       const int i = base + lane;
       int tot;
-      block_rank<FE_T / 64>(i < st.n_lm[cur] && lms[i].has3d && lms[i].inlier, s_cnt, tot);
+      block_rank<T / 64>(i < st.n_lm[cur] && lms[i].has3d && lms[i].inlier, s_cnt, tot);
       valid += tot;
     }
     if (lane == 0) {
@@ -2239,71 +2350,79 @@
       s_tail = tl;
     }
     __syncthreads();
-    if (s_full) return;
-    KeyFrameDev& kf = p.kfq[(size_t)s * KFQ + (s_tail % KFQ)];
-    Landmark* lms = lm_ptr(p, cur, s);
-    const int n = st.n_lm[cur];
-    int cnt = 0;
-    unsigned hsum = 0u;
-    for (int base = 0; base < n; base += FE_T) {
-      int i = base + lane;
-      bool sel = i < n && lms[i].has3d && lms[i].inlier;
-      int tot;
-      const int rk = block_rank<FE_T / 64>(sel, s_cnt, tot);
-      if (sel) {
-        int k = cnt + rk;
-        if (k < KF_MAXLM) {
-          kf.lm_id[k] = lms[i].id;
-          kf.lm_2d[k][0] = lms[i].p2u[0];
-          kf.lm_2d[k][1] = lms[i].p2u[1];
-          kf.lm_3d[k][0] = lms[i].p3w[0];
-          kf.lm_3d[k][1] = lms[i].p3w[1];
-          kf.lm_3d[k][2] = lms[i].p3w[2];
-          if (p.kf_check) hsum += kf_entry_hash(k, lms[i].id, lms[i].p2u, lms[i].p3w);
-        }
-      }
-      cnt += tot;
-    }
-    if (p.kf_check) {
-      if (hsum) atomicAdd(&s_hash, hsum);
+    if (!s_full) {
+      KeyFrameDev& kf = p.kfq[(size_t)s * KFQ + (s_tail % KFQ)];
+      Landmark* lms = lm_ptr(p, cur, s);
+      const int n = st.n_lm[cur];
+      int cnt = 0;
+      unsigned hsum = 0u;
+      for (int base = 0; base < n; base += T) {
+        int i = base + lane;
+        bool sel = i < n && lms[i].has3d && lms[i].inlier;
+        int tot;
+        const int rk = block_rank<T / 64>(sel, s_cnt, tot);
+        if (sel) {
+          int k = cnt + rk;
+          if (k < KF_MAXLM) {
+            kf.lm_id[k] = lms[i].id;
+            kf.lm_2d[k][0] = lms[i].p2u[0];
+            kf.lm_2d[k][1] = lms[i].p2u[1];
+            kf.lm_3d[k][0] = lms[i].p3w[0];
+            kf.lm_3d[k][1] = lms[i].p3w[1];
+            kf.lm_3d[k][2] = lms[i].p3w[2];
+            if (p.kf_check) hsum += kf_entry_hash(k, lms[i].id, lms[i].p2u, lms[i].p3w);
+          }
+        }
+        cnt += tot;
+      }
+      if (p.kf_check) {
+        if (hsum) atomicAdd(&s_hash, hsum);
+        __syncthreads();
+      }
+      if (lane == 0) {
+        kf.frame_id = st.frame_id[cur];
+        kf.stamp = st.frame_time[cur];
+        kf.lm_count = cnt < KF_MAXLM ? cnt : KF_MAXLM;
+        for (int j = 0; j < 7; j++) kf.T_c_w[j] = st.T_c_w[cur][j];
+        for (int j = 0; j < 4; j++) kf.imu_dq[j] = st.kf_dq[j];
+        kf.imu_dt = st.kf_dt;
+        kf.imu_valid = (s_chain && st.kf_dt > 0) ? 1 : 0;
+        kf.imu_pad = p.kf_check ? (int)s_hash : 0;
+        for (int j = 0; j < 3; j++) {
+          kf.imu_dp[j] = st.kf_dp[j];
+          kf.imu_va[j] = st.kf_va[j];
+          st.kf_dp[j] = st.kf_dv[j] = 0.0;
+        }
+        {
+          const bool have = st.has_imu && st.vi_count > 0;
+          const MotionState& mb = p.vi[(size_t)s * VI_QUEUE + (st.vi_head + (st.vi_count > 0 ? st.vi_count - 1 : 0)) % VI_QUEUE];
+          for (int j = 0; j < 3; j++) st.kf_va[j] = have ? mb.vel[j] : 0.0;
+        }
+        st.kf_dq[0] = 1.0, st.kf_dq[1] = st.kf_dq[2] = st.kf_dq[3] = 0.0;
+        st.kf_dt = 0;
+        {
+          CRig& rg = rig_of(p, s);
+          kf.rig_K[0] = rg.fx, kf.rig_K[1] = rg.fy, kf.rig_K[2] = rg.cx, kf.rig_K[3] = rg.cy;
+          for (int j = 0; j < 7; j++) kf.rig_T_c_i[j] = rg.T_c_i[j];
+        }
+        kf.valid = KFQ_KEYFRAME;
+        p.kfq_kf[s] = s_tail + 1u;
+      }
       __syncthreads();
-    }
-    if (lane == 0) {
-      kf.frame_id = st.frame_id[cur];
-      kf.stamp = st.frame_time[cur];
-      kf.lm_count = cnt < KF_MAXLM ? cnt : KF_MAXLM;
-      for (int j = 0; j < 7; j++) kf.T_c_w[j] = st.T_c_w[cur][j];
-      for (int j = 0; j < 4; j++) kf.imu_dq[j] = st.kf_dq[j];
-      kf.imu_dt = st.kf_dt;
-      kf.imu_valid = (s_chain && st.kf_dt > 0) ? 1 : 0;
-      kf.imu_pad = p.kf_check ? (int)s_hash : 0;
-      for (int j = 0; j < 3; j++) {
-        kf.imu_dp[j] = st.kf_dp[j];
-        kf.imu_va[j] = st.kf_va[j];
-        st.kf_dp[j] = st.kf_dv[j] = 0.0;
-      }
-      {
-        const bool have = st.has_imu && st.vi_count > 0;
-        const MotionState& mb = p.vi[(size_t)s * VI_QUEUE + (st.vi_head + (st.vi_count > 0 ? st.vi_count - 1 : 0)) % VI_QUEUE];
-        for (int j = 0; j < 3; j++) st.kf_va[j] = have ? mb.vel[j] : 0.0;
-      }
-      st.kf_dq[0] = 1.0, st.kf_dq[1] = st.kf_dq[2] = st.kf_dq[3] = 0.0;
-      st.kf_dt = 0;
-      {
-        CRig& rg = rig_of(p, s);
-        kf.rig_K[0] = rg.fx, kf.rig_K[1] = rg.fy, kf.rig_K[2] = rg.cx, kf.rig_K[3] = rg.cy;
-        for (int j = 0; j < 7; j++) kf.rig_T_c_i[j] = rg.T_c_i[j];
-      }
-      kf.valid = KFQ_KEYFRAME;
-      p.kfq_kf[s] = s_tail + 1u;
-    }
-    __syncthreads();
-    if (lane == 0) __hip_atomic_store(&p.kfq_tail[s], s_tail + 1u, __ATOMIC_RELEASE, __HIP_MEMORY_SCOPE_AGENT);
+      if (lane == 0) __hip_atomic_store(&p.kfq_tail[s], s_tail + 1u, __ATOMIC_RELEASE, __HIP_MEMORY_SCOPE_AGENT);
+    }
   }
 }
 __global__ __launch_bounds__(FE_T) void k_frame_end(Pipe p) {
   kj_wait(p.kj);
-  if (stream_present(p, blockIdx.x)) k_frame_end_body(p);
+  if (stream_present(p, blockIdx.x)) k_frame_end_body<FE_T>(p);
+  kj_signal(p.kj);
+}
+__global__ __launch_bounds__(NMAX) void k_depth_innovate_end(Pipe p) {
+  kj_wait(p.kj);
+  k_depth_innovate_body(p);
+  __syncthreads();
+  k_frame_end_body<NMAX>(p);
   kj_signal(p.kj);
 }
 
@@ -2491,6 +2610,9 @@
   return hipSuccess;
 }
 void launch_pose_lm(hipStream_t st, const Pipe& p) { hipLaunchKernelGGL(k_pose_lm, dim3(p.S), dim3(PL_T), sizeof(PoseLMShared), st, p); }
+void launch_pose_lm_filter(hipStream_t st, const Pipe& p) {
+  hipLaunchKernelGGL(k_pose_lm_filter, dim3(p.S), dim3(PL_T), sizeof(PoseLMShared), st, p);
+}
 static hipError_t pnp_tables_init() {
   static bool done[64] = {};
   int dev = 0;
@@ -2554,6 +2676,10 @@
     const hipError_t e = pnp_tables_init();
     if (e != hipSuccess) return e;
   }
+  {
+    const hipError_t e = hipFuncSetAttribute((const void*)k_pose_lm_filter, hipFuncAttributeMaxDynamicSharedMemorySize, (int)sizeof(PoseLMShared));
+    if (e != hipSuccess) return e;
+  }
   return hipFuncSetAttribute((const void*)k_pose_lm, hipFuncAttributeMaxDynamicSharedMemorySize, (int)sizeof(PoseLMShared));
 }
 void launch_reproj_filter(hipStream_t st, const Pipe& p) { hipLaunchKernelGGL(k_reproj_filter, dim3(p.S), dim3(NMAX), 0, st, p); }
@@ -2563,6 +2689,9 @@
   hipLaunchKernelGGL(k_depth_seeds, dim3(NMAX / 256, p.S), dim3(256), 0, st, p);
 }
 void launch_add_new_seeds(hipStream_t st, const Pipe& p) { hipLaunchKernelGGL(k_add_new_seeds, dim3(p.S), dim3(256), 0, st, p); }
+void launch_dem_add_new_seeds(hipStream_t st, const Pipe& p, const DemLaunch& d, bool with_seeds) {
+  hipLaunchKernelGGL(k_dem_add_new_seeds, dim3(p.S), dim3(256), dem_body_lds(d.corner_cap), st, p, d, with_seeds ? 1 : 0);
+}
 void launch_depth_triangulate(hipStream_t st, const Pipe& p) {
   hipLaunchKernelGGL(k_depth_triangulate, dim3(NMAX / 256, p.S), dim3(256), 0, st, p);
 }
@@ -2570,5 +2699,8 @@
 void launch_frame_end(hipStream_t st, const Pipe& p) {
   hipLaunchKernelGGL(k_frame_end, dim3(p.S), dim3(FE_T), 0, st, p);
 }
-
-}
+void launch_depth_innovate_end(hipStream_t st, const Pipe& p) {
+  hipLaunchKernelGGL(k_depth_innovate_end, dim3(p.S), dim3(NMAX), 0, st, p);
+}
+
+}
diff --git a/flvis_amd/csrc/track_kernels.hpp b/flvis_amd/csrc/track_kernels.hpp
--- a/flvis_amd/csrc/track_kernels.hpp
+++ b/flvis_amd/csrc/track_kernels.hpp
@@ -128,13 +128,22 @@
 void launch_track_post(hipStream_t st, const Pipe& p);
 void launch_pose_lm(hipStream_t st, const Pipe& p);
 void launch_reproj_filter(hipStream_t st, const Pipe& p);
+void launch_pose_lm_filter(hipStream_t st, const Pipe& p);
 void launch_vi_correction(hipStream_t st, const Pipe& p);
 void launch_add_new(hipStream_t st, const Pipe& p);
 void launch_depth_seeds(hipStream_t st, const Pipe& p);
 void launch_add_new_seeds(hipStream_t st, const Pipe& p);
+struct DemLaunch {
+  int w, h;
+  const float* sorted_xy;
+  const int* region_off;
+  int corner_cap;
+};
+void launch_dem_add_new_seeds(hipStream_t st, const Pipe& p, const DemLaunch& d, bool with_seeds);
 void launch_depth_triangulate(hipStream_t st, const Pipe& p);
 void launch_depth_innovate(hipStream_t st, const Pipe& p);
 void launch_frame_end(hipStream_t st, const Pipe& p);
+void launch_depth_innovate_end(hipStream_t st, const Pipe& p);
 constexpr int RESET_LIST = 64;
 enum { RS_TRACKER = 1, RS_CMD = 2, RS_SKIP = 4, RS_CREATE = 8 };
 struct ResetList {
```
